# refresh-bio/colord

Measured on AMD Instinct MI355X. Metric: input Gbases/s + archive size vs ref, ONT 50 Gb at 1/2/4/8 MI355X, higher is better.
Workload: dtype u64

## Files before the change

### colord_amd/csrc/common.hpp

```cpp
#pragma once
#ifdef CL_HOST_DEBUG
#define CL_DEV __host__ __device__
#else
#define CL_DEV __device__
#endif
#include <hip/hip_runtime.h>
#include <cstdint>
#include <cstdio>
#include <cstring>
#include <string>
#include <vector>
#include <algorithm>
#include <map>
#include <deque>
#include <mutex>
#include <atomic>
#include <condition_variable>
#include <thread>
#include <chrono>
#include "../../include/colord_hip.h"

#define CL_WAVE 64

struct KernelTime { double ms = 0; uint32_t launches = 0; double bytes = 0, cells = 0; };
// ... 364 lines not shown
	}
	~KernelTimer()
	{
		if (cl_sync_debug())
		{
			fprintf(stderr, "[sync] > %s\n", name);
			const hipError_t e = hipStreamSynchronize(cl_launch_stream(c));
			fprintf(stderr, "[sync] < %s%s%s\n", name, e == hipSuccess ? "" : ": ", e == hipSuccess ? "" : hipGetErrorString(e));
		}
		if (!c->timing) return;
		(void)hipEventRecord(b, cl_launch_stream(c));
		c->pending.push_back({ name, { a, b } });
		c->pending_bytes.push_back(c->next_bytes); c->next_bytes = 0;
		c->pending_cells.push_back(c->next_cells); c->next_cells = 0;
	}
};
#define LAUNCH(ctx, kernel, grid, block, ...) do { KernelTimer _kt((ctx), #kernel); \
	hipLaunchKernelGGL(kernel, dim3(grid), dim3(block), 0, cl_launch_stream(ctx), __VA_ARGS__); } while (0)
#define LAUNCHB_NAMED(ctx, name, bytes, kernel, grid, block, ...) do { (ctx)->next_bytes = (double)(bytes); KernelTimer _kt((ctx), (name)); \
	hipLaunchKernelGGL(kernel, dim3(grid), dim3(block), 0, cl_launch_stream(ctx), __VA_ARGS__); } while (0)
#define LAUNCH_NAMED(ctx, name, kernel, grid, block, ...) LAUNCHB_NAMED(ctx, name, 0.0, kernel, grid, block, __VA_ARGS__)
#define LAUNCHB(ctx, bytes, kernel, grid, block, ...) do { (ctx)->next_bytes = (double)(bytes); LAUNCH(ctx, kernel, grid, block, __VA_ARGS__); } while (0)
#define LAUNCHB_SHM(ctx, bytes, kernel, grid, block, shm, ...) do { (ctx)->next_bytes = (double)(bytes); KernelTimer _kt((ctx), #kernel); \
	hipLaunchKernelGGL(kernel, dim3(grid), dim3(block), (shm), cl_launch_stream(ctx), __VA_ARGS__); } while (0)
enum { CL_ROLE_MAIN = 0, CL_ROLE_QUAL = 1, CL_ROLE_LANE = 2, CL_ROLE_PREP = 3, CL_ROLE_CODER = 4, CL_N_ROLES = 5 };
struct CuMaskCfg { bool any = false; bool on[CL_N_ROLES] = { false, false, false, false, false }; uint32_t lo[CL_N_ROLES] = { 0, 0, 0, 0, 0 }, hi[CL_N_ROLES] = { 0, 0, 0, 0, 0 }; };
inline const CuMaskCfg& cl_cu_mask_cfg()
{
	static const CuMaskCfg cfg = []() {
		CuMaskCfg c;
		const char* e = getenv("COLORD_HIP_CU_MASK");
		if (!e) return c;
		static const char* names[CL_N_ROLES] = { "main", "qual", "lane", "prep", "coder" };
		std::string s(e); size_t p = 0;
		while (p < s.size())
		{
			size_t q = s.find(',', p); if (q == std::string::npos) q = s.size();
			const std::string item = s.substr(p, q - p); p = q + 1;
			const size_t colon = item.find(':'), dash = item.find('-');
			if (colon == std::string::npos || dash == std::string::npos || dash < colon) continue;
			for (int r = 0; r < CL_N_ROLES; ++r) if (item.substr(0, colon) == names[r])
			{
				c.lo[r] = (uint32_t)atoi(item.substr(colon + 1, dash - colon - 1).c_str()); c.hi[r] = (uint32_t)atoi(item.substr(dash + 1).c_str());
				if (c.hi[r] >= c.lo[r] && c.hi[r] < 1024) { c.on[r] = true; c.any = true; }
			}
		}
		return c;
	}();
	return cfg;
}
static inline int cl_role_level(int role, int dflt)
{
	static const struct Cfg { bool on[CL_N_ROLES] = {}; int level[CL_N_ROLES] = {}; Cfg() {
		const char* e = getenv("COLORD_HIP_ROLE_PRIO"); if (!e) return;
		static const char* names[CL_N_ROLES] = { "main", "qual", "lane", "prep", "coder" };
		std::string t(e); size_t p = 0;
		while (p < t.size()) { size_t q = t.find(',', p); if (q == std::string::npos) q = t.size(); const std::string item = t.substr(p, q - p); const size_t c = item.find(':');
			if (c != std::string::npos) for (int r = 0; r < CL_N_ROLES; ++r) if (item.substr(0, c) == names[r]) { on[r] = true; level[r] = atoi(item.c_str() + c + 1); }
			p = q + 1; }
	} } cfg;
	return role >= 0 && role < CL_N_ROLES && cfg.on[role] ? cfg.level[role] : dflt;
}
static inline int cl_level_to_prio(int level)
{
	int least = 0, greatest = 0;
	if (hipDeviceGetStreamPriorityRange(&least, &greatest) != hipSuccess) { (void)hipGetLastError(); return 0; }
	return level > 0 ? greatest : level < 0 ? least : 0;
}
static inline hipError_t cl_stream_create_role(int role, int prio, hipStream_t* s)
{
	const CuMaskCfg& m = cl_cu_mask_cfg();
	if (role >= 0 && role < CL_N_ROLES && m.on[role])
	{
		uint32_t bits[32] = { 0 };
		for (uint32_t b = m.lo[role]; b <= m.hi[role]; ++b) bits[b >> 5] |= 1u << (b & 31);
		return hipExtStreamCreateWithCUMask(s, (m.hi[role] >> 5) + 1, bits);
	}
	return prio ? hipStreamCreateWithPriority(s, hipStreamNonBlocking, prio) : hipStreamCreateWithFlags(s, hipStreamNonBlocking);
}
static inline hipError_t cl_stream_create(cl_ctx* c, hipStream_t* s) { return cl_stream_create_role(c->role, c->prio, s); }
static inline hipError_t cl_side_stream(cl_ctx* c, std::atomic<hipStream_t>& slot)
{
	if (slot.load(std::memory_order_acquire)) return hipSuccess;
	hipStream_t s = nullptr;
	const hipError_t e = cl_stream_create(c, &s);
	if (e == hipSuccess) slot.store(s, std::memory_order_release);
	return e;
}
static inline void cl_timing_begin(cl_ctx*) {}
static inline void cl_timing_collect(cl_ctx* c, bool wait = false)
{
	if (!c->timing) return;
	size_t keep = 0;
	for (size_t i = 0; i < c->pending.size(); ++i)
	{
		auto& p = c->pending[i];
		bool done = true;
		if (wait) (void)hipEventSynchronize(p.second.second);
		else if (hipEventQuery(p.second.second) != hipSuccess) { (void)hipGetLastError(); done = false; }
		if (!done)
		{
			if (keep != i) { c->pending[keep] = std::move(p); c->pending_bytes[keep] = c->pending_bytes[i]; c->pending_cells[keep] = c->pending_cells[i]; }
			++keep;
			continue;
		}
		float ms = 0; (void)hipEventElapsedTime(&ms, p.second.first, p.second.second);
		std::string nm = p.first;
		if (!nm.empty() && nm.front() == '(' && nm.back() == ')') nm = nm.substr(1, nm.size() - 2);
		auto& t = c->times[nm]; t.ms += ms; t.launches += 1; t.bytes += c->pending_bytes[i]; t.cells += c->pending_cells[i];
		c->ev_pool.push_back(p.second.first); c->ev_pool.push_back(p.second.second);
	}
	c->pending.resize(keep); c->pending_bytes.resize(keep); c->pending_cells.resize(keep);
}

__host__ __device__ static inline uint64_t hash_mm(uint64_t x)
{
	x ^= x >> 33; x *= 0xff51afd7ed558ccdULL;
	x ^= x >> 33; x *= 0xc4ceb9fe1a85ec53ULL;
	x ^= x >> 33;
	return x;
}

struct ModTest { uint64_t low_mask, dinv, lim; uint32_t s; };
static inline ModTest make_modtest(uint32_t f)
{
	ModTest m; uint32_t s = 0; uint64_t d = f;
	while ((d & 1) == 0) { d >>= 1; ++s; }
	uint64_t inv = d;
	for (int i = 0; i < 6; ++i) inv *= 2 - d * inv;
	m.s = s; m.low_mask = (s ? ((1ULL << s) - 1) : 0); m.dinv = inv; m.lim = ~0ULL / d;
	return m;
}
__device__ static inline bool mod_is_zero(uint64_t h, const ModTest& m)
{
	return ((h & m.low_mask) == 0) && (((h >> m.s) * m.dinv) <= m.lim);
}

__device__ static inline uint32_t lane_id() { return threadIdx.x & 63; }
__device__ static inline uint64_t lanemask_lt() { return (1ULL << lane_id()) - 1; }

__device__ static inline uint32_t wave_incl_scan(uint32_t v)
{
#pragma unroll
	for (int d = 1; d < 64; d <<= 1) { uint32_t t = __shfl_up(v, d, 64); if ((int)lane_id() >= d) v += t; }
	return v;
}
__device__ static inline uint32_t wave_sum(uint32_t v)
{
#pragma unroll
	for (int d = 32; d > 0; d >>= 1) v += __shfl_xor(v, d, 64);
	return v;
}

__device__ static inline uint32_t block_excl_scan_256(uint32_t v, uint32_t* sh, uint32_t* total)
{
	uint32_t incl = wave_incl_scan(v);
	uint32_t w = threadIdx.x >> 6;
	__syncthreads();
	if (lane_id() == 63) sh[w] = incl;
	__syncthreads();
	uint32_t base = 0, tot = 0;
#pragma unroll
	for (uint32_t i = 0; i < 4; ++i) { uint32_t s = sh[i]; if (i < w) base += s; tot += s; }
	*total = tot;
	return base + incl - v;
}

cl_status dev_exclusive_scan_u32(cl_ctx* ctx, uint32_t* d_data, uint64_t n, uint64_t* h_total);
cl_status dev_exclusive_scan_u64(cl_ctx* ctx, const uint32_t* d_in, uint64_t* d_out, uint64_t n, uint64_t* h_total);
cl_status dev_run_starts_u32(cl_ctx* ctx, const uint32_t* d_keys, uint64_t n, uint32_t shift, uint32_t* d_seg, uint64_t seg_cap, uint64_t* h_n_runs);
cl_status dev_run_starts_u64(cl_ctx* ctx, const uint64_t* d_keys, uint64_t n, uint32_t shift, uint32_t* d_seg, uint64_t seg_cap, uint64_t* h_n_runs);
cl_status dev_sort_pairs(cl_ctx* ctx, uint64_t* d_keys, uint32_t* d_vals, uint64_t n, uint32_t begin_bit, uint32_t end_bit);
cl_status dev_sort_pairs_swap(cl_ctx* ctx, DevBuf<uint64_t>& keys, DevBuf<uint32_t>& vals, uint64_t n, uint32_t begin_bit, uint32_t end_bit);
cl_status dev_sort_keys32_pairs(cl_ctx* ctx, uint32_t* d_keys, uint32_t* d_vals, uint64_t n, uint32_t begin_bit, uint32_t end_bit);
cl_status dev_sort_keys32_pairs_swap(cl_ctx* ctx, DevBuf<uint32_t>& keys, DevBuf<uint32_t>& vals, uint64_t n, uint32_t begin_bit, uint32_t end_bit);

static inline uint32_t grid_for(uint64_t n, uint32_t per_block) { return (uint32_t)((n + per_block - 1) / per_block); }
```

### colord_amd/csrc/dna.hip

```cpp
#include "common.hpp"
#include <functional>
#include "objects.hpp"
#include "rc_dev.hpp"
#include <algorithm>
#include <deque>
#include <thread>
#include <chrono>

namespace {
enum { T_INS = 0, T_DEL, T_MATCH, T_SUBST, T_ANCHOR, T_SKIP, T_ALT_ID, T_MAIN_REF, T_PLAIN, T_START_PLAIN, T_START_ES, T_START_PLAIN_N, T_NONE };
enum { F_READ_TYPE = 0, F_REV_COMP, F_SEEN, F_LEN_BITS, F_LEN_DATA, F_SYMBOLS, F_SYMBOLS_N, F_READ_ID, F_READ_ID_SHORT,
       F_ANCHOR_LEN, F_SKIP_LOCAL, F_SKIP_DISTANT, F_TUPLE_TYPE, N_FAM };
constexpr uint32_t MAX_ALT = 64;

struct FamTab {
	uint32_t n_sym[N_FAM], max_total[N_FAM], adder[N_FAM];
	uint32_t ctx_base[N_FAM + 1];
	uint64_t state_base[N_FAM + 1];
	uint32_t n_ctx[N_FAM];
	int32_t level, T, S;
	uint32_t sym_B;
	uint32_t max_alt;
	uint32_t long_run;
	uint32_t walk_chunk, walk_warm;
};

struct RefStore { const uint64_t* packed; const uint64_t* word_off; const uint32_t* lens; uint32_t n; };
__device__ inline uint32_t ref_at(const RefStore& R, uint32_t id, bool rev, int64_t pos)
{
	if (id >= R.n) return 255;
	const uint32_t len = R.lens[id];
	if (pos < 0 || pos >= (int64_t)len) return 255;
	const uint32_t p = rev ? (len - 1 - (uint32_t)pos) : (uint32_t)pos;
	const uint32_t b = (uint32_t)(R.packed[R.word_off[id] + (p >> 5)] >> (62 - 2 * (p & 31))) & 3u;
	return rev ? 3u - b : b;
}
struct RefCur {
	uint32_t id = 0xffffffffu, len = 0, widx = 0xffffffffu; bool rev = false, ok = false; uint64_t wo = 0, word = 0;
	__device__ inline void set(const RefStore& R, uint32_t nid, bool nrev)
	{
		rev = nrev;
		if (nid == id) return;
		id = nid; widx = 0xffffffffu; ok = nid < R.n;
		if (ok) { len = R.lens[nid]; wo = R.word_off[nid]; }
	}
	__device__ inline uint32_t at(const RefStore& R, int64_t pos)
	{
		if (!ok || pos < 0 || pos >= (int64_t)len) return 255;
		const uint32_t p = rev ? (len - 1 - (uint32_t)pos) : (uint32_t)pos;
		if ((p >> 5) != widx) { widx = p >> 5; word = R.packed[wo + widx]; }
		const uint32_t b = (uint32_t)(word >> (62 - 2 * (p & 31))) & 3u;
		return rev ? 3u - b : b;
	}
};
__device__ inline uint32_t ilog2_(uint64_t x) { return x ? 64u - (uint32_t)__clzll((long long)x) : 0u; }
__device__ inline uint32_t no_bytes_(uint64_t x) { uint32_t r = 1; x >>= 8; for (; x; ++r) x >>= 8; return r; }

template<typename K> struct KeyFmt {
	static __host__ __device__ inline K make(uint32_t gctx, uint32_t payload) { return ((K)gctx << 8) | (K)payload; }
	static __host__ __device__ inline uint32_t ctx(K k) { return (uint32_t)(k >> 8); }
	static __host__ __device__ inline uint32_t payload(K k) { return (uint32_t)k & 0xffu; }
};
__device__ inline uint32_t key_payload(int fam, uint32_t sym, int e1, int e2)
{
	if (fam == F_TUPLE_TYPE)
	{
		const uint32_t x = e1 == 15 ? 0u : e2 == 15 ? (e1 == T_ANCHOR ? 1u : 2u) : e1 == T_ANCHOR ? 3u : e1 == T_DEL ? 4u : 5u;
		return (x << 3) | sym;
	}
	if (fam == F_SYMBOLS) return ((e1 == 15 ? 0u : (uint32_t)e1 + 1u) << 2) | sym;
	return sym;
}
__device__ inline void key_decode(uint32_t fam, uint32_t p, uint32_t& sym, uint32_t& e1, uint32_t& e2)
{
	if (fam == F_TUPLE_TYPE)
	{
		const uint32_t x = p >> 3; sym = p & 7u;
		e1 = x == 0 ? 15u : (x == 1 || x == 3) ? (uint32_t)T_ANCHOR : x == 2 ? (uint32_t)T_SKIP : x == 4 ? (uint32_t)T_DEL : (uint32_t)T_ALT_ID;
		e2 = x == 3 ? (uint32_t)T_MATCH : x == 4 ? (uint32_t)T_SKIP : x == 5 ? (uint32_t)T_MAIN_REF : 15u;
	}
	else if (fam == F_SYMBOLS) { const uint32_t x = p >> 2; sym = p & 3u; e1 = x ? x - 1u : 15u; e2 = 15u; }
	else { sym = p; e1 = e2 = 15u; }
}
__device__ inline uint32_t key_sym_mask(uint32_t fam) { return fam == F_TUPLE_TYPE ? 7u : fam == F_SYMBOLS ? 3u : 0xffu; }

template<typename K>
struct Emitter {
	static constexpr uint32_t SLOTS = 64 / sizeof(K);
	bool write; K* key; uint64_t off; uint32_t count; const FamTab* ft;
	K* stage = nullptr; uint64_t first = 0; bool any = false;
	__device__ inline void put(K k)
	{
		const uint64_t g = off + count;
		if (!stage) { key[g] = k; return; }
		if (!any) { first = g; any = true; }
		stage[g & (SLOTS - 1)] = k;
		if ((g & (SLOTS - 1)) != SLOTS - 1) return;
		const uint64_t base = g & ~(uint64_t)(SLOTS - 1);
		if (first <= base)
		{
			uint4* dst = (uint4*)(key + base); const uint32_t* sw = (const uint32_t*)stage;
#pragma unroll
			for (int q = 0; q < 4; ++q) dst[q] = make_uint4(sw[4 * q], sw[4 * q + 1], sw[4 * q + 2], sw[4 * q + 3]);
		}
		else for (uint64_t x = first; x <= g; ++x) key[x] = stage[x & (SLOTS - 1)];
	}
	__device__ inline void finish()
	{
		if (!stage || !any) return;
		const uint64_t g = off + count, base = g & ~(uint64_t)(SLOTS - 1);
		for (uint64_t x = first > base ? first : base; x < g; ++x) key[x] = stage[x & (SLOTS - 1)];
	}
	__device__ inline void operator()(int fam, uint32_t ctx, uint32_t sym, int e1 = 15, int e2 = 15)
	{
		if (write)
		{
			put(KeyFmt<K>::make(ft->ctx_base[fam] + ctx, key_payload(fam, sym, e1, e2)));
		}
		++count;
	}
};

struct EsReader {
	const uint8_t* p; const uint8_t* e;
	uint64_t w0 = 0, w1 = 0; uint32_t have = 0;
	__device__ inline void refill()
	{
		const uint64_t a = (uint64_t)(size_t)p; const uint32_t sh = (uint32_t)(a & 7);
		const uint64_t* q = (const uint64_t*)(a & ~7ull);
		const uint64_t* lim = (const uint64_t*)(((uint64_t)(size_t)e + 7) & ~7ull);
		const uint64_t x0 = q[0], x1 = q + 1 < lim ? q[1] : 0ull, x2 = q + 2 < lim ? q[2] : 0ull;
		w0 = sh ? (x0 >> (8 * sh)) | (x1 << (64 - 8 * sh)) : x0;
		w1 = sh ? (x1 >> (8 * sh)) | (x2 << (64 - 8 * sh)) : x1;
		have = 16;
	}
	__device__ inline void drop(uint32_t n) { p += n; have -= n; w0 = (w0 >> (8 * n)) | (w1 << (64 - 8 * n)); w1 >>= 8 * n; }
	__device__ inline bool next(uint32_t& type, uint32_t& v1, uint32_t& v2)
	{
		if (p >= e) return false;
		if (have < 5) refill();
		const uint32_t b0 = (uint32_t)(w0 & 0xff), t = b0 >> 4; type = t;
		switch (t)
		{
		case T_INS: case T_SUBST: case T_PLAIN: v1 = b0 & 0xf; drop(1); break;
		case T_ANCHOR: case T_SKIP: v2 = ((b0 & 0xf) << 24) | ((uint32_t)((w0 >> 8) & 0xff) << 16) | ((uint32_t)((w0 >> 16) & 0xff) << 8) | (uint32_t)((w0 >> 24) & 0xff); drop(4); break;
		case T_ALT_ID: case T_START_ES: v2 = b0 & 0xf; v1 = ((uint32_t)((w0 >> 8) & 0xff) << 24) | ((uint32_t)((w0 >> 16) & 0xff) << 16) | ((uint32_t)((w0 >> 24) & 0xff) << 8) | (uint32_t)((w0 >> 32) & 0xff); drop(5); break;
		default: drop(1);
		}
		return true;
	}
};

template<typename K> __device__ inline void emit_read_len(Emitter<K>& em, uint32_t len)
{
	int nb = (int)ilog2_(len);
	em(F_LEN_BITS, 0, (uint32_t)nb);
// ... 190 lines not shown
					rd.p += 8; rd.have -= 8; rd.w0 = rd.w1; rd.w1 = 0;
					t_idx += 8;
					continue;
				}
			}
		}
		if (!rd.next(type, v1, v2)) break;
		++t_idx;
		const uint32_t ref_symbol = !track ? 0u : is_main ? mainc.at(R, ref_pos) : altc.at(R, alt_pos);
		{
			uint32_t cls = delta < -10 ? 1u : delta < -1 ? 2u : delta > 10 ? 3u : delta > 1 ? 4u : 0u;
			uint32_t c = (uint32_t)ctx_tuple | ((uint32_t)(ctx_symbol & 0xf) << s3);
			if (ref_symbol <= 3) c |= (ref_symbol << (s3 + 4)) | (cls << (s3 + 6));
			else c = (1u << (s3 + 9)) + (c | (cls << (s3 + 4)));
			int e1 = 15, e2 = 15;
			if (!first)
				switch (last_flag)
				{
				case T_MATCH: e1 = T_ANCHOR; break;
				case T_DEL: e1 = T_SKIP; break;
				case T_ANCHOR: e1 = T_ANCHOR; e2 = T_MATCH; break;
				case T_SKIP: e1 = T_DEL; e2 = T_SKIP; break;
				case T_MAIN_REF: case T_ALT_ID: e1 = T_ALT_ID; e2 = T_MAIN_REF; break;
				default: break;
				}
			em(F_TUPLE_TYPE, c, type, e1, e2);
			ctx_tuple = ((ctx_tuple << 3) + type) & mask_tuple;
		}
		first = false; last_flag = type;
		switch (type)
		{
		case T_ALT_ID:
		{
			if (!is_main && alt_slot >= 0) alt_pos_of[alt_slot] = (int32_t)alt_pos;
			bool is_new = false; int32_t slot = -1;
			if (n_alt == 0) { emit_read_id(em, v1, cur_read_id); alt_ids[0] = (int32_t)v1; alt_pos_of[0] = 0; n_alt = 1; slot = 0; is_new = true; }
			else
			{
				const uint32_t seen = n_alt;
				for (uint32_t i = 0; i < n_alt; ++i) if (alt_ids[i] == (int32_t)v1) slot = (int32_t)i;
				const int32_t short_id = slot;
				if (slot < 0)
				{
					if (n_alt >= MAX_ALT) { if (err) atomicOr(err, 1u); em.finish(); return; }
					slot = (int32_t)n_alt; alt_ids[n_alt] = (int32_t)v1; alt_pos_of[n_alt] = 0; ++n_alt; is_new = true;
				}
				em(F_SEEN, seen, short_id >= 0 ? 1u : 0u);
				if (short_id < 0) emit_read_id(em, v1, cur_read_id);
				else em(F_READ_ID_SHORT, seen, (uint32_t)short_id);
			}
			if (is_new) alt_rev_of[slot] = (uint8_t)v2;
			rev_comp_flag(v1, v2 != 0);
			alt_id = v1; alt_slot = slot; alt_rev = alt_rev_of[slot] != 0;
			altc.set(R, alt_id, alt_rev);
			alt_pos = 0; is_main = false; delta = 0;
			break;
		}
		case T_ANCHOR:
			emit_anchor_len(em, v2);
			if (is_main) ref_pos += v2; else alt_pos += v2;
			if (track)
			{
				for (int i = ft.S; i > 0; --i)
					ctx_symbol = (ctx_symbol << 2) + (is_main ? mainc.at(R, ref_pos - i) : altc.at(R, alt_pos - i));
				ctx_symbol &= mask_symbol;
				known = (uint32_t)ft.S;
			}
			delta = 0;
			break;
		case T_MATCH:
			ctx_symbol = ((ctx_symbol << 2) + ref_symbol) & mask_symbol; ++known;
			if (is_main) ++ref_pos; else ++alt_pos;
			break;
		case T_INS:
		{
			uint32_t shift = 2, c = 2;
			if (ft.level == 1) { c += (uint32_t)(ctx_symbol & 0xff) << shift; shift += 8; }
			else if (ft.level == 2) { c += (uint32_t)(ctx_symbol & 0x3ff) << shift; shift += 10; }
			else { c += (uint32_t)(ctx_symbol & 0x3ff) << shift; shift += 10; c += (uint32_t)(((ctx_symbol >> 10) & 3) == ((ctx_symbol >> 8) & 3)) << shift; ++shift; }
			const bool guard = ref_symbol > 3;
			c += (guard ? 0u : ref_symbol) << shift; shift += 2;
			c += (uint32_t)(ctx_tuple & 0777) << shift;
			if (guard) c += 1u << ft.sym_B;
			em(F_SYMBOLS, c, v1);
			ctx_symbol = ((ctx_symbol << 2) + v1) & mask_symbol; ++known;
			++delta;
			break;
		}
		case T_DEL:
			if (is_main) ++ref_pos; else ++alt_pos;
			--delta;
			break;
		case T_SUBST:
		{
			const uint32_t rs = ref_symbol & 3;
			const uint32_t sym = (rs == 0) ? (v1 == 0 ? 1u : v1 == 1 ? 2u : 3u) : (rs == 1) ? (v1 == 0 ? 0u : v1 == 1 ? 2u : 3u)
			                   : (rs == 2) ? (v1 == 0 ? 0u : v1 == 1 ? 1u : 3u) : (v1 == 0 ? 0u : v1 == 1 ? 1u : 2u);
			uint32_t shift = 2, c = 1;
			c += (uint32_t)(ctx_symbol & 0x3f) << shift; shift += 6;
			if (ft.level == 3) { c += (uint32_t)(((ctx_symbol >> 6) & 3) == ((ctx_symbol >> 4) & 3)) << shift; ++shift; }
			c += rs << shift; shift += 2;
			c += (uint32_t)(ctx_tuple & 07777) << shift;
			em(F_SYMBOLS, c, sym, (int)rs);
			ctx_symbol = ((ctx_symbol << 2) + sym) & mask_symbol; ++known;
			if (is_main) ++ref_pos; else ++alt_pos;
			break;
		}
		case T_SKIP:
		{
			const int32_t skip_len = (int32_t)v2;
			delta -= skip_len;
			if (!is_main && last_type == T_ALT_ID)
			{
				const int32_t mod = skip_len - (alt_slot >= 0 ? alt_pos_of[alt_slot] : 0);
				if (mod > 0) emit_skip_len(em, (uint32_t)mod, false);
				else { emit_skip_len(em, 0, false); emit_skip_len(em, (uint32_t)(-mod), false); }
			}
			else emit_skip_len(em, (uint32_t)skip_len, last_type != T_ALT_ID && last_type != T_NONE);
			if (is_main) ref_pos += v2; else alt_pos += v2;
			break;
		}
		case T_MAIN_REF:
			is_main = true;
			if (alt_slot >= 0) alt_pos_of[alt_slot] = (int32_t)alt_pos;
			delta = 0;
			break;
		default: break;
		}
		last_type = type;
	}
	em.finish();
	if (!WRITE)
	{
		hdr_counts[r] = em.count; counts[r] = em.count;
		if (t_idx != ntup - 1 && err) atomicOr(err, 2u);
	}
}

__global__ void k_read_flags(const uint8_t* __restrict__ es, const uint64_t* __restrict__ es_off, uint32_t r0, uint32_t r1, uint8_t* __restrict__ flag)
{
	uint32_t r = r0 + blockIdx.x * blockDim.x + threadIdx.x;
	if (r >= r1) return;
	uint32_t t = es[es_off[r]] >> 4;
	flag[r - r0] = t == T_START_PLAIN ? 0 : t == T_START_PLAIN_N ? 1 : 2;
}

__global__ __launch_bounds__(256) void k_fill_sidx(const uint64_t* __restrict__ sym_off, uint64_t s0, uint32_t r0, uint32_t r1, TripLayoutDev lay, uint32_t* __restrict__ sidx)
{
	const uint32_t r = r0 + blockIdx.x * 4 + (threadIdx.x >> 6);
	if (r >= r1) return;
	const uint32_t lane = threadIdx.x & 63;
	const uint64_t a = sym_off[r] - s0, b = sym_off[r + 1] - s0;
	if (a == b) return;
	const uint32_t part = part_of_read(lay, r), pl = lay.rank ? lay.rank[part] : part;
	const uint64_t gb = lay.group_base[pl >> 6], p0 = lay.part_sym_start[part];
	for (uint64_t i = a + lane; i < b; i += 64) sidx[i] = (uint32_t)trip_slot(gb, pl & 63, i - p0);
}
template<typename K>
__global__ __launch_bounds__(256) void k_dna_plain(const FamTab* __restrict__ ftp, const uint8_t* __restrict__ es, const uint64_t* __restrict__ es_off,
                                                  const uint32_t* __restrict__ es_ntup, const uint8_t* __restrict__ read_flag, const uint32_t* __restrict__ hdr_counts,
                                                  const uint64_t* __restrict__ sym_off, uint32_t r0, uint32_t r1, K* __restrict__ key)
{
	const uint32_t r = r0 + blockIdx.x * 4 + (threadIdx.x >> 6);
	if (r >= r1) return;
	const uint32_t fl = read_flag[r - r0];
	if (fl == 2) return;
	const FamTab& ft = *ftp;
	const uint32_t lane = threadIdx.x & 63;
	const uint8_t* b = es + es_off[r] + 1;
	const uint32_t len = es_ntup[r] - 1;
	const uint64_t off = sym_off[r - r0] + hdr_counts[r - r0];
	const uint32_t S2 = 2 * ft.S; const uint32_t mask = (1u << S2) - 1;
	const uint32_t fam = fl == 0 ? F_SYMBOLS : F_SYMBOLS_N;
	const uint32_t cbase = ft.ctx_base[fam];
	for (uint32_t i = lane; i < len; i += 64)
	{
		uint32_t ctx = mask;
		if (fl == 0)
		{
			const uint32_t n = i < (uint32_t)ft.S ? i : (uint32_t)ft.S;
			for (uint32_t t = n; t >= 1; --t) ctx = ((ctx << 2) + (b[i - t] & 3u)) & mask;
			ctx <<= 2;
		}
		else
		{
			const uint32_t n = i < 4 ? i : 4;
			for (uint32_t t = n; t >= 1; --t) ctx = ((ctx << 4) + (b[i - t] & 0xfu)) & mask;
		}
		key[off + i] = KeyFmt<K>::make(cbase + ctx, b[i] & 0xfu);
	}
}


constexpr uint32_t LONG_RUN = 1u << 19;
struct LongRun { uint32_t s, e, fam, gctx; uint64_t step0, group0, epoch0; uint32_t epoch_cap, pad; };
template<int NS> struct EpochRec { uint32_t start, tot; uint32_t st[NS]; uint32_t cnt0[NS]; };
__device__ inline uint32_t find_run(const LongRun* runs, uint32_t n_runs, uint64_t step)
{
	uint32_t lo = 0, hi = n_runs;
	while (hi - lo > 1) { const uint32_t mid = (lo + hi) >> 1; if (runs[mid].step0 <= step) lo = mid; else hi = mid; }
	return lo;
}
template<typename K>
__global__ void k_long_find(const uint32_t* __restrict__ seg_start, uint32_t n_seg, const K* __restrict__ skey, const FamTab* __restrict__ ftp, LongRun* __restrict__ runs , uint32_t cap, uint32_t* __restrict__ n_runs )
{
	const uint32_t sg = blockIdx.x * blockDim.x + threadIdx.x;
	if (sg >= n_seg) return;
	const uint32_t s = seg_start[sg], e = seg_start[sg + 1];
	const FamTab& ft = *ftp;
	if (e - s < ft.long_run) return;
	const uint32_t gctx = KeyFmt<K>::ctx(skey[s]);
	uint32_t fam = 0;
	for (uint32_t f = 1; f < N_FAM; ++f) if (gctx >= ft.ctx_base[f]) fam = f;
	if (ft.n_sym[fam] > 32) return;
	const uint32_t which = ft.n_sym[fam] > 8 ? 1u : 0u;
	const uint32_t i = atomicAdd(n_runs + which, 1u);
	if (i < cap) { LongRun r; r.s = s; r.e = e; r.fam = fam; r.gctx = gctx; r.step0 = r.group0 = r.epoch0 = 0; r.epoch_cap = 0; r.pad = 0; runs[which * cap + i] = r; }
}
template<int NS, typename K>
__global__ __launch_bounds__(256) void k_long_hist(const LongRun* __restrict__ runs, uint32_t n_runs, uint64_t n_groups, const K* __restrict__ skey,
                                                  uint32_t* __restrict__ step_pfx, uint32_t* __restrict__ group_tot)
{
	const uint64_t g = ((uint64_t)blockIdx.x * blockDim.x + threadIdx.x) >> 6; const uint32_t lane = threadIdx.x & 63;
	if (g >= n_groups) return;
	uint32_t lo = 0, hi = n_runs;
	while (hi - lo > 1) { const uint32_t mid = (lo + hi) >> 1; if (runs[mid].group0 <= g) lo = mid; else hi = mid; }
	const LongRun R = runs[lo];
	const uint64_t gl = g - R.group0;
	const uint32_t smask = key_sym_mask(R.fam);
	uint32_t c[NS];
#pragma unroll
	for (int a = 0; a < NS; ++a) c[a] = 0;
	for (uint32_t k = 0; k < 64; ++k)
	{
		const uint64_t j = (uint64_t)R.s + (gl * 64 + k) * 64 + lane;
		const bool valid = j < R.e;
		const uint32_t sym = valid ? (uint32_t)skey[j] & smask : 0xffu;
#pragma unroll
		for (uint32_t a = 0; a < NS; ++a) { const uint32_t n = (uint32_t)__popcll(__ballot(sym == a)); if (lane == k) c[a] = n; }
	}
	const uint64_t n_steps = ((uint64_t)(R.e - R.s) + 63) / 64;
	const uint64_t step = R.step0 + gl * 64 + lane;
#pragma unroll
	for (uint32_t a = 0; a < NS; ++a)
	{
		const uint32_t incl = wave_incl_scan(c[a]);
		if (gl * 64 + lane < n_steps) step_pfx[step * NS + a] = incl - c[a];
		if (lane == 63) group_tot[g * NS + a] = incl;
	}
}
template<int NS>
__global__ __launch_bounds__(64) void k_long_groups(const LongRun* __restrict__ runs, uint32_t n_runs, uint32_t* __restrict__ group_tot )
{
	const uint32_t r = blockIdx.x, lane = threadIdx.x;
	if (r >= n_runs) return;
	const LongRun R = runs[r];
	const uint64_t n_steps = ((uint64_t)(R.e - R.s) + 63) / 64, n_groups = (n_steps + 63) / 64;
	uint32_t carry[NS];
#pragma unroll
	for (int a = 0; a < NS; ++a) carry[a] = 0;
	for (uint64_t g0 = 0; g0 < n_groups; g0 += 64)
	{
		const uint64_t g = g0 + lane; const bool valid = g < n_groups;
#pragma unroll
		for (uint32_t a = 0; a < NS; ++a)
		{
			const uint32_t v = valid ? group_tot[(R.group0 + g) * NS + a] : 0u;
			const uint32_t incl = wave_incl_scan(v);
			if (valid) group_tot[(R.group0 + g) * NS + a] = carry[a] + incl - v;
			carry[a] += __shfl(incl, 63);
		}
	}
}
template<int NS, typename K>
__device__ inline uint32_t long_prefix(const LongRun& R, const K* skey, const uint32_t* step_pfx, const uint32_t* group_pfx, uint32_t x, uint32_t lane)
{
	const uint32_t smask = key_sym_mask(R.fam);
	const uint64_t step = x >> 6; const uint32_t off = x & 63;
	const uint32_t a = lane & (NS - 1);
	uint32_t v = group_pfx[(R.group0 + (step >> 6)) * NS + a] + (step * 64 < (uint64_t)(R.e - R.s) || off ? step_pfx[(R.step0 + step) * NS + a] : 0u);
	if (x == R.e - R.s && off == 0)
	{
		const uint64_t last = step - 1;
		const uint64_t j = (uint64_t)R.s + last * 64 + lane; const uint32_t sym = j < R.e ? (uint32_t)skey[j] & smask : 0xffu;
		uint32_t mine = 0;
#pragma unroll
		for (uint32_t b = 0; b < NS; ++b) { const uint32_t n = (uint32_t)__popcll(__ballot(sym == b)); if (a == b) mine = n; }
		return group_pfx[(R.group0 + (last >> 6)) * NS + a] + step_pfx[(R.step0 + last) * NS + a] + mine;
	}
	if (off)
	{
		const uint64_t j = (uint64_t)R.s + step * 64 + lane; const uint32_t sym = j < R.e ? (uint32_t)skey[j] & smask : 0xffu;
		const uint64_t below = (1ULL << off) - 1;
		uint32_t mine = 0;
#pragma unroll
		for (uint32_t b = 0; b < NS; ++b) { const uint32_t n = (uint32_t)__popcll(__ballot(sym == b) & below); if (a == b) mine = n; }
		v += mine;
	}
	return v;
}
template<int NS, typename K>
__global__ __launch_bounds__(64) void k_long_epochs(const FamTab* __restrict__ ftp, const LongRun* __restrict__ runs, uint32_t n_runs, const K* __restrict__ skey,
                                                   const uint32_t* __restrict__ step_pfx, const uint32_t* __restrict__ group_pfx, uint32_t* __restrict__ state,
                                                   EpochRec<NS>* __restrict__ epochs, uint32_t* __restrict__ n_epochs, uint32_t* __restrict__ group_epoch, uint32_t* __restrict__ err)
{
	const uint32_t r = blockIdx.x, lane = threadIdx.x;
	if (r >= n_runs) return;
	const LongRun R = runs[r];
	const FamTab& ft = *ftp;
	const uint32_t n_sym = ft.n_sym[R.fam], max_total = ft.max_total[R.fam], adder = ft.adder[R.fam];
// ... 101 lines not shown
	{
		if (e - s >= ft.long_run) return;
		uint32_t st[8]; uint32_t tot = sp[n_sym];
#pragma unroll
		for (uint32_t a = 0; a < 8; ++a) st[a] = a < n_sym ? sp[a] : 0u;
		for (uint32_t j0 = s; j0 < e; j0 += 64)
		{
			const uint32_t j = j0 + lane; const bool valid = j < e;
			uint32_t sym = 0xffu, e1 = 15u, e2 = 15u;
			if (valid) key_decode(fam, KeyFmt<K>::payload(skey[j]), sym, e1, e2);
			const uint32_t dst = valid ? sval[j] : 0u;
			uint64_t m[8];
#pragma unroll
			for (uint32_t a = 0; a < 8; ++a) m[a] = __ballot(valid && sym == a);
			const uint32_t cnt = (e - j0) < 64 ? (e - j0) : 64;
			uint32_t start = 0;
			while (start < cnt)
			{
				const uint32_t r = (max_total - tot + adder - 1) / adder;
				const uint32_t now = (cnt - start) < r ? (cnt - start) : r;
				const uint64_t win = (now == 64 ? ~0ULL : ((1ULL << now) - 1)) << start;
				if (lane >= start && lane < start + now)
				{
					const uint64_t before = lt & win;
					uint32_t cum = 0, freq = 0, excl = 0;
#pragma unroll
					for (uint32_t a = 0; a < 8; ++a)
					{
						const uint32_t v = st[a] + adder * (uint32_t)__popcll(m[a] & before);
						const bool ex = a == e1 || a == e2;
						if (ex) excl += v;
						if (a < sym && !ex) cum += v;
						if (a == sym) freq = v;
					}
					trip[dst] = pack_triple(cum, freq, tot + adder * (lane - start) - excl);
				}
#pragma unroll
				for (uint32_t a = 0; a < 8; ++a) st[a] += adder * (uint32_t)__popcll(m[a] & win);
				tot += adder * now;
				while (tot >= max_total)
				{
					tot = 0;
#pragma unroll
					for (uint32_t a = 0; a < 8; ++a) { st[a] = (st[a] + 1) / 2; tot += st[a]; }
				}
				start += now;
			}
		}
		if (lane == 0)
		{
			for (uint32_t a = 0; a < n_sym; ++a) sp[a] = st[a];
			sp[n_sym] = tot;
		}
		return;
	}
	if (n_sym <= 32 && e - s >= ft.long_run) return;
	uint32_t* cnt = s_cnt[w]; uint32_t* pre = s_pre[w];
#pragma unroll
	for (uint32_t t = 0; t < 4; ++t) { uint32_t a = lane * 4 + t; cnt[a] = a < n_sym ? sp[a] : 0u; }
	uint32_t tot = sp[n_sym];
	auto rebuild_prefix = [&]() {
		uint32_t v0 = cnt[lane * 4], v1 = cnt[lane * 4 + 1], v2 = cnt[lane * 4 + 2], v3 = cnt[lane * 4 + 3];
		uint32_t sum = v0 + v1 + v2 + v3;
		uint32_t ex = wave_incl_scan(sum) - sum;
		pre[lane * 4] = ex; pre[lane * 4 + 1] = ex + v0; pre[lane * 4 + 2] = ex + v0 + v1; pre[lane * 4 + 3] = ex + v0 + v1 + v2;
		__builtin_amdgcn_wave_barrier();
	};
	__builtin_amdgcn_wave_barrier();
	rebuild_prefix();
	for (uint32_t j0 = s; j0 < e; j0 += 64)
	{
		const uint32_t j = j0 + lane; const bool valid = j < e;
		const uint32_t sym = valid ? KeyFmt<K>::payload(skey[j]) : 0u;
		const uint32_t dst = valid ? sval[j] : 0u;
		const uint32_t n_here = (e - j0) < 64 ? (e - j0) : 64;
		uint32_t start = 0;
		while (start < n_here)
		{
			const uint32_t r = (max_total - tot + adder - 1) / adder;
			const uint32_t now = (n_here - start) < r ? (n_here - start) : r;
			uint32_t less = 0, eq = 0;
			for (uint32_t l = start; l < start + now; ++l)
			{
				const uint32_t o = __builtin_amdgcn_readlane(sym, l);
				if (l < lane) { less += (o < sym) ? 1u : 0u; eq += (o == sym) ? 1u : 0u; }
			}
			const bool mine = lane >= start && lane < start + now;
			if (mine) trip[dst] = pack_triple(pre[sym] + adder * less, cnt[sym] + adder * eq, tot + adder * (lane - start));
			__builtin_amdgcn_wave_barrier();
			if (mine) atomicAdd(&cnt[sym], adder);
			__builtin_amdgcn_wave_barrier();
			tot += adder * now;
			while (tot >= max_total)
			{
				uint32_t sum = 0;
#pragma unroll
				for (uint32_t t = 0; t < 4; ++t) { uint32_t a = lane * 4 + t; if (a < n_sym) { uint32_t v = (cnt[a] + 1) / 2; cnt[a] = v; sum += v; } }
				tot = wave_sum(sum);
			}
			__builtin_amdgcn_wave_barrier();
			rebuild_prefix();
			start += now;
		}
	}
#pragma unroll
	for (uint32_t t = 0; t < 4; ++t) { uint32_t a = lane * 4 + t; if (a < n_sym) sp[a] = cnt[a]; }
	if (lane == 0) sp[n_sym] = tot;
}

__global__ void k_init_fam_state(const FamTab* __restrict__ ftp, uint32_t fam, uint32_t* __restrict__ state)
{
	const FamTab& ft = *ftp;
	const uint32_t ns = ft.n_sym[fam];
	const uint64_t n = (uint64_t)ft.n_ctx[fam] * (ns + 1);
	for (uint64_t i = (uint64_t)blockIdx.x * blockDim.x + threadIdx.x; i < n; i += (uint64_t)gridDim.x * blockDim.x)
		state[ft.state_base[fam] + i] = (i % (ns + 1)) == ns ? ns : 1u;
}
__global__ void k_gather_bytes2(const uint8_t* __restrict__ src, const uint64_t* __restrict__ src_off, const uint64_t* __restrict__ dst_off,
                                const uint64_t* __restrict__ size, uint8_t* __restrict__ dst)
{
	const uint32_t p = blockIdx.x;
	const uint64_t n = size[p]; const uint8_t* s = src + src_off[p]; uint8_t* d = dst + dst_off[p];
	for (uint64_t i = threadIdx.x; i < n; i += blockDim.x) d[i] = s[i];
}
__global__ void k_last_types(const uint8_t* __restrict__ flag, uint32_t n, uint32_t prev, uint32_t* __restrict__ out)
{
	uint32_t v = prev;
	uint32_t start = n > 4 ? n - 4 : 0;
	for (uint32_t i = start; i < n; ++i) v = ((v << 2) + flag[i]) & 0xff;
	*out = v;
}
}

struct DnaGroupPrep {
	uint32_t p0 = 0, p1 = 0, r0 = 0, r1 = 0; uint64_t s0 = 0, n_syms = 0, n_seg = 0, trip_words = 0;
	std::vector<uint32_t> rank, plen_r;
	DevBuf<uint64_t> d_gbase; DevBuf<uint32_t> d_plen;
	DevBuf<uint32_t> sidx, seg;
	struct LongPrep { uint32_t n_runs = 0; uint64_t steps = 0, groups = 0, eps = 0; DevBuf<LongRun> runs; DevBuf<uint32_t> step_pfx, group_pfx; } lp[2];
	bool long_ready = false;
};
struct DnaWalked {
	const uint8_t* d_es = nullptr; uint32_t n_reads = 0;
	uint32_t prev_types_in = 0, cur_read_id_in = 0, prev_types_out = 0;
	DevBuf<uint8_t> rflag; DevBuf<uint32_t> hdr; DevBuf<uint64_t> sym_off, key; DevBuf<uint32_t> key32; bool narrow = false;
	std::vector<uint64_t> h_sym_off;
	bool presorted = false; std::vector<uint32_t> part_bounds; std::vector<std::unique_ptr<DnaGroupPrep>> groups;
};
struct cl_dna_coder {
	cl_ctx* ctx = nullptr;
	FamTab ft;
	DevBuf<FamTab> d_ft;
	DevBuf<uint32_t> state;
	uint32_t ctx_bits = 0; bool narrow = false;
	uint32_t cur_read_id = 0;
	uint32_t prev_types = 0;
	uint32_t next_read_id = 0, next_prev_types = 0; bool next_valid = false;
	std::unique_ptr<DnaWalked> ahead;
	std::function<cl_status()> before_tail;
	std::deque<std::unique_ptr<struct DnaEvolved>> evolved;
	uint32_t ahead_prev_types = 0, ahead_read_id = 0;
	std::vector<hipStream_t> cstreams; uint32_t next_cstream = 0;
	~cl_dna_coder();
};

extern "C" cl_status cl_dna_coder_create(cl_ctx* ctx, uint32_t max_alt_refs, int32_t level, uint32_t start_read_id, cl_dna_coder** out)
{
	if (!ctx || !out) return cl_fail(ctx, CL_E_INVALID, "cl_dna_coder_create: null argument");
	if (level < 1 || level > 3 || max_alt_refs < 1 || max_alt_refs > MAX_ALT) return cl_fail(ctx, CL_E_INVALID, "cl_dna_coder_create: level 1..3, 1 <= max_alt_refs <= 64");
	HIP_TRY(ctx, hipSetDevice(ctx->device));
	cl_dna_coder* D = new cl_dna_coder(); D->ctx = ctx; D->cur_read_id = start_read_id;
	std::unique_ptr<cl_dna_coder> guard(D);
	FamTab& f = D->ft; memset(&f, 0, sizeof(f));
	f.level = level; f.max_alt = max_alt_refs;
	f.T = level == 3 ? 4 : level == 2 ? 3 : 2;
	f.S = level == 3 ? 8 : level == 2 ? 7 : 5;
	f.sym_B = level == 3 ? 24 : level == 2 ? 23 : 22;
	f.long_run = LONG_RUN;
	if (const char* lr = getenv("COLORD_HIP_LONG_RUN")) f.long_run = (uint32_t)std::max(64, atoi(lr));
	f.walk_chunk = WALK_CHUNK; f.walk_warm = WALK_WARM;
	if (const char* v = getenv("COLORD_HIP_WALK_CHUNK")) f.walk_chunk = (uint32_t)std::min(1 << 20, std::max(32, atoi(v)));
	if (const char* v = getenv("COLORD_HIP_WALK_WARM")) f.walk_warm = (uint32_t)std::max(0, atoi(v));
	f.walk_warm = std::min(f.walk_warm, f.walk_chunk / 2);
	auto set = [&](int i, uint32_t ns, uint32_t mt, uint32_t ad, uint32_t nc) { f.n_sym[i] = ns; f.max_total[i] = mt; f.adder[i] = ad; f.n_ctx[i] = nc; };
	set(F_READ_TYPE, 3, 1u << 15, 1, 256);
	set(F_REV_COMP, 2, 1u << 15, 1, 16);
	set(F_SEEN, 2, 1u << 15, 1, MAX_ALT + 1);
	set(F_LEN_BITS, 32, 1u << 18, 8, 1);
	set(F_LEN_DATA, 256, 1u << 18, 8, 512);
	set(F_SYMBOLS, 4, 1u << 10, 1, 1u << (f.sym_B + 1));
	set(F_SYMBOLS_N, 5, 1u << 10, 1, 1u << 16);
	set(F_READ_ID, 256, 1u << 13, 1, 2048);
	set(F_READ_ID_SHORT, max_alt_refs, 1u << 13, 1, MAX_ALT + 1);
	set(F_ANCHOR_LEN, 24, 1u << 15, 1, 1u << 17);
	set(F_SKIP_LOCAL, 256, 1u << 15, 1, 1u << 14);
	set(F_SKIP_DISTANT, 256, 1u << 15, 1, 256);
	set(F_TUPLE_TYPE, 8, 1u << 15, 1, 1u << (3 * f.T + 10));
	uint64_t cb = 0, sb = 0;
	for (int i = 0; i < N_FAM; ++i) { f.ctx_base[i] = (uint32_t)cb; f.state_base[i] = sb; cb += f.n_ctx[i]; sb += (uint64_t)f.n_ctx[i] * (f.n_sym[i] + 1); }
	f.ctx_base[N_FAM] = (uint32_t)cb; f.state_base[N_FAM] = sb;
	if (cb >= (1ull << 32)) return cl_fail(ctx, CL_E_UNSUPPORTED, "cl_dna_coder_create: context space too large");
	D->ctx_bits = 1; while ((1ull << D->ctx_bits) < cb) ++D->ctx_bits;
	D->narrow = D->ctx_bits + 8 <= 32 && !getenv("COLORD_HIP_DNA_WIDE_KEYS");
	DEV_ALLOC(ctx, D->d_ft, 1);
	HIP_TRY(ctx, hipMemcpyAsync(D->d_ft.p, &f, sizeof(f), hipMemcpyHostToDevice, ctx->stream));
	DEV_ALLOC(ctx, D->state, sb);
	for (uint32_t i = 0; i < N_FAM; ++i) LAUNCH(ctx, k_init_fam_state, 2048, 256, (const FamTab*)D->d_ft.p, i, D->state.p);
	HIP_TRY(ctx, hipGetLastError());
	HIP_TRY(ctx, hipStreamSynchronize(ctx->stream));
	*out = guard.release();
	return CL_OK;
}
extern "C" void cl_dna_coder_free(cl_dna_coder* d) { delete d; }

namespace {
struct SideSync { hipStream_t s = nullptr; ~SideSync() { if (s) (void)hipStreamSynchronize(s); } };
struct PendingGroup {
	DevBuf<triple_t> trip; DevBuf<uint64_t> d_gbase, d_out_off, d_size, d_dst_off; DevBuf<uint32_t> d_plen; DevBuf<uint8_t> tmp;
	std::vector<uint64_t> out_off; std::vector<uint32_t> rank; uint32_t p0 = 0, np = 0;
	hipStream_t stream = nullptr;
	SideSync sync;
};
}
struct DnaEvolved {
	const uint8_t* d_es = nullptr; uint32_t n_reads = 0, prev_types_in = 0, read_id_in = 0, prev_types_out = 0;
	std::vector<uint32_t> part_bounds;
	std::vector<std::unique_ptr<PendingGroup>> groups;
};
cl_dna_coder::~cl_dna_coder() { evolved.clear(); for (hipStream_t s : cstreams) (void)hipStreamDestroy(s); }

namespace {
cl_status dna_walk(cl_ctx* ctx, cl_dna_coder* D, const cl_reads* refs, const uint8_t* d_es, const uint64_t* d_es_off, const uint32_t* d_es_ntuples, uint32_t n_reads,
                   uint32_t prev_types, uint32_t cur_read_id, DnaWalked& W)
{
	const FamTab& f = D->ft;
	RefStore R{ refs->packed.p, refs->word_off.p, refs->lens.p, refs->n_reads };
	W.d_es = d_es; W.n_reads = n_reads; W.prev_types_in = prev_types; W.cur_read_id_in = cur_read_id;
	DevBuf<uint8_t>& rflag = W.rflag; DevBuf<uint32_t>& hdr = W.hdr; DevBuf<uint64_t>& sym_off = W.sym_off; std::vector<uint64_t>& h_sym_off = W.h_sym_off;
	W.narrow = D->narrow;
	DEV_ALLOC(ctx, rflag, (uint64_t)n_reads + 1); DEV_ALLOC(ctx, hdr, (uint64_t)n_reads + 1); DEV_ALLOC(ctx, sym_off, (uint64_t)n_reads + 1);
	DevBuf<uint32_t> err; DEV_ALLOC(ctx, err, 1);
	HIP_TRY(ctx, hipMemsetAsync(err.p, 0, 4, ctx->stream));
	h_sym_off.assign((size_t)n_reads + 1, 0);
	if (n_reads)
	{
		uint64_t total_syms = 0, h_eb[2] = { 0, 0 };
		HIP_TRY(ctx, hipMemcpyAsync(&h_eb[0], d_es_off, 8, hipMemcpyDeviceToHost, ctx->stream));
		HIP_TRY(ctx, hipMemcpyAsync(&h_eb[1], d_es_off + n_reads, 8, hipMemcpyDeviceToHost, ctx->stream));
		HIP_TRY(ctx, hipStreamSynchronize(ctx->stream));
		DevBuf<uint64_t> chunk_off; DEV_ALLOC(ctx, chunk_off, (uint64_t)n_reads + 1);
		DevBuf<WalkCk> cks; uint64_t n_chunks = 0;
		{
			DevBuf<uint32_t> counts; DEV_ALLOC(ctx, counts, n_reads);
			LAUNCH(ctx, k_read_flags, grid_for(n_reads, 256), 256, d_es, d_es_off, 0u, n_reads, rflag.p);
			LAUNCH(ctx, k_walk_chunks, grid_for(n_reads, 256), 256, d_es_ntuples, (const uint8_t*)rflag.p, n_reads, f.walk_chunk, counts.p);
			CL_TRY(dev_exclusive_scan_u64(ctx, counts.p, chunk_off.p, n_reads, &n_chunks));
			if (n_chunks >= (1ull << 32)) return cl_fail(ctx, CL_E_UNSUPPORTED, "cl_dna_encode: too many tuples in one call");
			DEV_ALLOC(ctx, cks, n_chunks);
			LAUNCHB_NAMED(ctx, "k_dna_walk<false>", (double)(h_eb[1] - h_eb[0]) + 8.0 * n_reads + (double)n_chunks * sizeof(WalkCk), (k_dna_walk<false, uint32_t>), grid_for(n_reads, WALK_LPW), 64,
				(const FamTab*)D->d_ft.p, R, d_es, d_es_off, d_es_ntuples, (const uint8_t*)rflag.p, n_reads,
				prev_types, cur_read_id, (const uint64_t*)chunk_off.p, cks.p, (uint32_t)n_chunks, counts.p, hdr.p, (const uint64_t*)nullptr, (uint32_t*)nullptr, err.p, 0u);
			HIP_TRY(ctx, hipGetLastError());
			CL_TRY(dev_exclusive_scan_u64(ctx, counts.p, sym_off.p, n_reads, &total_syms));
		}
		HIP_TRY(ctx, hipMemcpy(h_sym_off.data(), sym_off.p, ((uint64_t)n_reads + 1) * 8, hipMemcpyDeviceToHost));
		uint32_t herr0 = 0;
		HIP_TRY(ctx, hipMemcpy(&herr0, err.p, 4, hipMemcpyDeviceToHost));
		if (herr0 & 2) return cl_fail(ctx, CL_E_INVALID, "cl_dna_encode: the tuple count of a read does not match its stream");
		if (herr0) return cl_fail(ctx, CL_E_UNSUPPORTED, "cl_dna_encode: a read uses more than 64 alternative references");
		if (W.narrow)
		{
			DEV_ALLOC(ctx, W.key32, total_syms);
			LAUNCHB_NAMED(ctx, "k_dna_walk<true>", total_syms * 5.0, (k_dna_walk<true, uint32_t>), grid_for(n_chunks, WALK_LPW), 64,
				(const FamTab*)D->d_ft.p, R, d_es, d_es_off, d_es_ntuples, (const uint8_t*)rflag.p, n_reads,
				prev_types, cur_read_id, (const uint64_t*)chunk_off.p, cks.p, (uint32_t)n_chunks, (uint32_t*)nullptr, (uint32_t*)nullptr, (const uint64_t*)sym_off.p, W.key32.p, err.p, 1u);
			LAUNCH_NAMED(ctx, "k_dna_plain", (k_dna_plain<uint32_t>), grid_for(n_reads, 4), 256, (const FamTab*)D->d_ft.p, d_es, d_es_off, d_es_ntuples, (const uint8_t*)rflag.p, (const uint32_t*)hdr.p,
				(const uint64_t*)sym_off.p, 0u, n_reads, W.key32.p);
		}
		else
		{
			DEV_ALLOC(ctx, W.key, total_syms);
			LAUNCHB_NAMED(ctx, "k_dna_walk<true>", total_syms * 9.0, (k_dna_walk<true, uint64_t>), grid_for(n_chunks, WALK_LPW), 64,
				(const FamTab*)D->d_ft.p, R, d_es, d_es_off, d_es_ntuples, (const uint8_t*)rflag.p, n_reads,
				prev_types, cur_read_id, (const uint64_t*)chunk_off.p, cks.p, (uint32_t)n_chunks, (uint32_t*)nullptr, (uint32_t*)nullptr, (const uint64_t*)sym_off.p, W.key.p, err.p, 1u);
			LAUNCH_NAMED(ctx, "k_dna_plain", (k_dna_plain<uint64_t>), grid_for(n_reads, 4), 256, (const FamTab*)D->d_ft.p, d_es, d_es_off, d_es_ntuples, (const uint8_t*)rflag.p, (const uint32_t*)hdr.p,
				(const uint64_t*)sym_off.p, 0u, n_reads, W.key.p);
		}
		HIP_TRY(ctx, hipGetLastError());
	}
	{
		DevBuf<uint32_t> lt; DEV_ALLOC(ctx, lt, 1);
		LAUNCH(ctx, k_last_types, 1, 1, (const uint8_t*)rflag.p, n_reads, prev_types, lt.p);
		HIP_TRY(ctx, hipGetLastError());
		HIP_TRY(ctx, hipMemcpyAsync(&W.prev_types_out, lt.p, 4, hipMemcpyDeviceToHost, ctx->stream));
		HIP_TRY(ctx, hipStreamSynchronize(ctx->stream));
	}
	return CL_OK;
}
}

namespace {
template<typename K>
cl_status dna_long_prepare(cl_ctx* ctx, cl_dna_coder* D, const K* gkey, uint64_t n_syms, DnaGroupPrep& G)
{
	const FamTab& f = D->ft;
	const uint32_t RUN_CAP = (uint32_t)std::max<uint64_t>(4096, n_syms / f.long_run + 2);
	DevBuf<LongRun> runs; DEV_ALLOC(ctx, runs, 2 * RUN_CAP);
	DevBuf<uint32_t> n_runs; DEV_ALLOC(ctx, n_runs, 2);
	HIP_TRY(ctx, hipMemsetAsync(n_runs.p, 0, 8, ctx->stream));
	LAUNCH_NAMED(ctx, "k_long_find", (k_long_find<K>), grid_for(G.n_seg, 256), 256, (const uint32_t*)G.seg.p, (uint32_t)G.n_seg, gkey, (const FamTab*)D->d_ft.p, runs.p, RUN_CAP, n_runs.p);
	uint32_t nlr2[2] = { 0, 0 };
	HIP_TRY(ctx, hipMemcpyAsync(nlr2, n_runs.p, 8, hipMemcpyDeviceToHost, ctx->stream));
	HIP_TRY(ctx, hipStreamSynchronize(ctx->stream));
	if (nlr2[0] > RUN_CAP || nlr2[1] > RUN_CAP) return cl_fail(ctx, CL_E_UNSUPPORTED, "cl_dna_encode: more than 4096 long context runs in one group");
	for (int which = 0; which < 2; ++which)
	{
		DnaGroupPrep::LongPrep& L = G.lp[which];
		const uint32_t nlr = nlr2[which], NS = which ? 32 : 8;
		L.n_runs = nlr; L.steps = L.groups = L.eps = 0;
		if (!nlr) continue;
		std::vector<LongRun> h(nlr);
		HIP_TRY(ctx, hipMemcpy(h.data(), runs.p + (uint64_t)which * RUN_CAP, nlr * sizeof(LongRun), hipMemcpyDeviceToHost));
		std::sort(h.begin(), h.end(), [](const LongRun& a, const LongRun& b) { return a.s < b.s; });
		for (auto& r : h)
		{
			const uint64_t Ln = r.e - r.s, ns = (Ln + 63) / 64, ngp = (ns + 63) / 64;
			const uint64_t half = f.max_total[r.fam] / 2 / f.adder[r.fam];
			r.step0 = L.steps; r.group0 = L.groups; r.epoch0 = L.eps; r.epoch_cap = (uint32_t)(Ln / (half > 80 ? half - 40 : 1) + 8);
			L.steps += ns; L.groups += ngp; L.eps += r.epoch_cap;
		}
		DEV_ALLOC(ctx, L.runs, nlr);
		HIP_TRY(ctx, hipMemcpyAsync(L.runs.p, h.data(), nlr * sizeof(LongRun), hipMemcpyHostToDevice, ctx->stream));
		DEV_ALLOC(ctx, L.step_pfx, (L.steps + 1) * NS); DEV_ALLOC(ctx, L.group_pfx, (L.groups + 1) * NS);
		const LongRun* cr = L.runs.p;
		if (which == 0)
		{
			LAUNCHB_NAMED(ctx, "k_long_hist<8>", L.steps * 64.0 * sizeof(K), (k_long_hist<8, K>), grid_for(L.groups * 64, 256), 256, cr, nlr, L.groups, gkey, L.step_pfx.p, L.group_pfx.p);
			LAUNCH(ctx, (k_long_groups<8>), nlr, 64, cr, nlr, L.group_pfx.p);
		}
		else
		{
			LAUNCHB_NAMED(ctx, "k_long_hist<32>", L.steps * 64.0 * sizeof(K), (k_long_hist<32, K>), grid_for(L.groups * 64, 256), 256, cr, nlr, L.groups, gkey, L.step_pfx.p, L.group_pfx.p);
			LAUNCH(ctx, (k_long_groups<32>), nlr, 64, cr, nlr, L.group_pfx.p);
		}
		HIP_TRY(ctx, hipGetLastError());
		HIP_TRY(ctx, hipStreamSynchronize(ctx->stream));
	}
	G.long_ready = true;
	return CL_OK;
}
}

namespace {
cl_status dna_group_prepare(cl_ctx* ctx, cl_dna_coder* D, DnaWalked& W, uint32_t p0, const uint32_t* h_part_bounds, uint32_t n_parts, DnaGroupPrep& G)
{
	const std::vector<uint64_t>& h_sym_off = W.h_sym_off;
	const uint64_t GROUP_SYMS = 5ull << 28;
	uint32_t p1 = p0; const uint32_t r0 = h_part_bounds[p0];
	while (p1 < n_parts)
	{
		const uint64_t pl = h_sym_off[h_part_bounds[p1 + 1]] - h_sym_off[h_part_bounds[p1]];
		if (pl >= (1ull << 31) - 64) return cl_fail(ctx, CL_E_UNSUPPORTED, "cl_dna_encode: one part has >= 2^31 symbols");
		if (p1 > p0 && h_sym_off[h_part_bounds[p1 + 1]] - h_sym_off[r0] >= GROUP_SYMS) break;
		++p1;
	}
	const uint32_t r1 = h_part_bounds[p1], nr = r1 - r0, np = p1 - p0, ng = (np + 63) / 64;
	const uint64_t s0 = h_sym_off[r0], n_syms = h_sym_off[r1] - s0;
	G.p0 = p0; G.p1 = p1; G.r0 = r0; G.r1 = r1; G.s0 = s0; G.n_syms = n_syms;
	std::vector<uint64_t> sym_start(np + 1);
	std::vector<uint32_t> plen(np), pfirst(np + 1);
	for (uint32_t p = 0; p <= np; ++p) { pfirst[p] = h_part_bounds[p0 + p]; sym_start[p] = h_sym_off[pfirst[p]] - s0; }
	for (uint32_t p = 0; p < np; ++p) plen[p] = (uint32_t)(sym_start[p + 1] - sym_start[p]);
	std::vector<uint32_t> order(np); std::vector<uint32_t>& rank = G.rank; std::vector<uint32_t>& plen_r = G.plen_r;
	rank.resize(np); plen_r.resize(np);
	for (uint32_t p = 0; p < np; ++p) order[p] = p;
	std::stable_sort(order.begin(), order.end(), [&](uint32_t a, uint32_t b) { return plen[a] > plen[b]; });
	for (uint32_t i = 0; i < np; ++i) { rank[order[i]] = i; plen_r[i] = plen[order[i]]; }
	std::vector<uint64_t> gbase(ng + 1, 0);
	for (uint32_t g = 0; g < ng; ++g) gbase[g + 1] = gbase[g] + trip_group_words(plen_r[g * 64]);
	if (gbase[ng] >= (1ull << 32)) return cl_fail(ctx, CL_E_UNSUPPORTED, "cl_dna_encode: group too large for 32-bit triple indices");
	G.trip_words = gbase[ng];
	DevBuf<uint64_t> d_sym_start; DevBuf<uint32_t> d_pfirst, d_rank;
	DEV_ALLOC(ctx, d_rank, np);
	HIP_TRY(ctx, hipMemcpyAsync(d_rank.p, rank.data(), np * 4, hipMemcpyHostToDevice, ctx->stream));
	DEV_ALLOC(ctx, d_sym_start, np + 1); DEV_ALLOC(ctx, G.d_gbase, ng + 1); DEV_ALLOC(ctx, G.d_plen, np); DEV_ALLOC(ctx, d_pfirst, np + 1);
	HIP_TRY(ctx, hipMemcpyAsync(d_sym_start.p, sym_start.data(), (np + 1) * 8, hipMemcpyHostToDevice, ctx->stream));
	HIP_TRY(ctx, hipMemcpyAsync(G.d_gbase.p, gbase.data(), (ng + 1) * 8, hipMemcpyHostToDevice, ctx->stream));
	HIP_TRY(ctx, hipMemcpyAsync(G.d_plen.p, plen_r.data(), np * 4, hipMemcpyHostToDevice, ctx->stream));
	HIP_TRY(ctx, hipMemcpyAsync(d_pfirst.p, pfirst.data(), (np + 1) * 4, hipMemcpyHostToDevice, ctx->stream));
	TripLayoutDev lay{ d_pfirst.p, d_sym_start.p, G.d_gbase.p, np, d_rank.p };
	if (n_syms)
	{
		DEV_ALLOC(ctx, G.sidx, n_syms);
		LAUNCHB(ctx, n_syms * 4.0, k_fill_sidx, grid_for(nr, 4), 256, (const uint64_t*)W.sym_off.p, s0, r0, r1, lay, G.sidx.p);
		HIP_TRY(ctx, hipGetLastError());
		const uint32_t cbits = D->ctx_bits;
		const uint64_t seg_cap = std::min<uint64_t>(n_syms, D->ft.ctx_base[N_FAM]) + 1;
		DEV_ALLOC(ctx, G.seg, seg_cap);
		if (W.narrow)
		{
			if (s0 == 0 && W.key32.n == n_syms) CL_TRY(dev_sort_keys32_pairs_swap(ctx, W.key32, G.sidx, n_syms, 8, 8 + cbits));
			else CL_TRY(dev_sort_keys32_pairs(ctx, W.key32.p + s0, G.sidx.p, n_syms, 8, 8 + cbits));
			CL_TRY(dev_run_starts_u32(ctx, W.key32.p + s0, n_syms, 8, G.seg.p, seg_cap, &G.n_seg));
			CL_TRY(dna_long_prepare<uint32_t>(ctx, D, W.key32.p + s0, n_syms, G));
		}
		else
		{
			if (s0 == 0 && W.key.n == n_syms) CL_TRY(dev_sort_pairs_swap(ctx, W.key, G.sidx, n_syms, 8, 8 + cbits));
			else CL_TRY(dev_sort_pairs(ctx, W.key.p + s0, G.sidx.p, n_syms, 8, 8 + cbits));
			CL_TRY(dev_run_starts_u64(ctx, W.key.p + s0, n_syms, 8, G.seg.p, seg_cap, &G.n_seg));
			CL_TRY(dna_long_prepare<uint64_t>(ctx, D, W.key.p + s0, n_syms, G));
		}
	}
	HIP_TRY(ctx, hipStreamSynchronize(ctx->stream));
	return CL_OK;
}
}

cl_status cl_dna_prepare_batch(cl_ctx* ctx, cl_dna_coder* D, const cl_reads* refs, const uint8_t* d_es, const uint64_t* d_es_off, const uint32_t* d_es_ntuples, uint32_t n_reads,
                               uint32_t prev_types, uint32_t read_id, const uint32_t* h_part_bounds, uint32_t n_parts, DnaWalked** out, uint32_t* prev_types_out)
{
	if (!ctx || !D || !refs || !d_es || !d_es_off || !d_es_ntuples || !n_reads || !out) return CL_E_INVALID;
	HIP_TRY(ctx, hipSetDevice(ctx->device));
	auto W = std::make_unique<DnaWalked>();
	CL_TRY(dna_walk(ctx, D, refs, d_es, d_es_off, d_es_ntuples, n_reads, prev_types, read_id, *W));
	if (h_part_bounds && n_parts && h_part_bounds[0] == 0 && h_part_bounds[n_parts] == n_reads)
	{
		W->part_bounds.assign(h_part_bounds, h_part_bounds + n_parts + 1);
		for (uint32_t p0 = 0; p0 < n_parts; )
		{
			auto G = std::make_unique<DnaGroupPrep>();
			CL_TRY(dna_group_prepare(ctx, D, *W, p0, h_part_bounds, n_parts, *G));
			p0 = G->p1;
			W->groups.push_back(std::move(G));
		}
		W->presorted = true;
	}
	if (prev_types_out) *prev_types_out = W->prev_types_out;
	*out = W.release();
	return CL_OK;
}
namespace {
__global__ void k_batch_types(const uint8_t* __restrict__ es, const uint64_t* __restrict__ es_off, uint32_t n_reads, uint64_t es_bytes, uint32_t prev, unsigned long long* __restrict__ out)
{
	uint32_t v = prev; bool ok = true;
	const uint32_t start = n_reads > 4 ? n_reads - 4 : 0;
	for (uint32_t r = start; r < n_reads; ++r)
	{
		const uint64_t a = es_off[r], b = es_off[r + 1];
		if (a >= b || b > es_bytes) { ok = false; break; }
		const uint32_t t = es[a] >> 4;
		v = ((v << 2) + (t == T_START_PLAIN ? 0u : t == T_START_PLAIN_N ? 1u : 2u)) & 0xff;
	}
	*out = ok ? (unsigned long long)v : ~0ull;
}
}
cl_status cl_dna_batch_types(cl_ctx* ctx, const uint8_t* d_es, const uint64_t* d_es_off, uint32_t n_reads, uint64_t es_bytes, uint32_t prev_types, uint32_t* out)
{
	if (!ctx || !d_es || !d_es_off || !out) return CL_E_INVALID;
	HIP_TRY(ctx, hipSetDevice(ctx->device));
	uint64_t* hs = nullptr; uint64_t* ds = nullptr;
	HIP_TRY(ctx, cl_slot(ctx, 1, &hs, &ds));
	LAUNCH(ctx, k_batch_types, 1, 1, d_es, d_es_off, n_reads, es_bytes, prev_types, (unsigned long long*)ds);
	HIP_TRY(ctx, hipGetLastError());
	HIP_TRY(ctx, hipStreamSynchronize(ctx->stream));
	const uint64_t v = *(volatile uint64_t*)hs;
	if (v == ~0ull) return cl_fail(ctx, CL_E_INVALID, "cl_dna_batch_types: a tuple stream offset of the last reads lies outside the stream");
	*out = (uint32_t)v;
	return CL_OK;
}
void cl_dna_walked_free(DnaWalked* W) { delete W; }
void cl_dna_set_ahead(cl_dna_coder* D, DnaWalked* W) { if (D) D->ahead.reset(W); else delete W; }
void cl_dna_coder_state(const cl_dna_coder* D, uint32_t* prev_types, uint32_t* read_id) { if (prev_types) *prev_types = D->prev_types; if (read_id) *read_id = D->cur_read_id; }

cl_status cl_dna_walk_ahead(cl_ctx* ctx, cl_dna_coder* D, const cl_reads* refs, const uint8_t* d_es, const uint64_t* d_es_off, const uint32_t* d_es_ntuples, uint32_t n_reads)
{
	if (!ctx || !D || !refs || !d_es || !d_es_off || !d_es_ntuples || !n_reads) return CL_E_INVALID;
	if (!D->next_valid) return cl_fail(ctx, CL_E_INVALID, "cl_dna_walk_ahead: only while a batch is being coded");
	auto W = std::make_unique<DnaWalked>();
	CL_TRY(dna_walk(ctx, D, refs, d_es, d_es_off, d_es_ntuples, n_reads, D->next_prev_types, D->next_read_id, *W));
	D->ahead = std::move(W);
	return CL_OK;
}
void cl_dna_set_before_tail(cl_dna_coder* D, std::function<cl_status()> fn) { if (D) D->before_tail = std::move(fn); }

namespace {
cl_status dna_evolve_batch(cl_ctx* ctx, cl_dna_coder* D, const cl_reads* refs, const uint8_t* d_es, const uint64_t* d_es_off, const uint32_t* d_es_ntuples, uint32_t n_reads,
                           const uint32_t* h_part_bounds, uint32_t n_parts, std::unique_ptr<DnaWalked> Wp, uint32_t prev_types, uint32_t read_id, DnaEvolved& E)
{
	const uint64_t* inv_tab = nullptr;
	CL_TRY(cl_inv_table(ctx, &inv_tab));
	if (Wp && Wp->presorted && (Wp->part_bounds.size() != (size_t)n_parts + 1 || memcmp(Wp->part_bounds.data(), h_part_bounds, ((size_t)n_parts + 1) * 4) != 0)) Wp.reset();
	if (!Wp) { Wp = std::make_unique<DnaWalked>(); CL_TRY(dna_walk(ctx, D, refs, d_es, d_es_off, d_es_ntuples, n_reads, prev_types, read_id, *Wp)); }
	DnaWalked& W = *Wp;
	DevBuf<uint32_t> err; DEV_ALLOC(ctx, err, 1);
	HIP_TRY(ctx, hipMemsetAsync(err.p, 0, 4, ctx->stream));
	E.d_es = d_es; E.n_reads = n_reads; E.prev_types_in = prev_types; E.read_id_in = read_id; E.prev_types_out = W.prev_types_out;
	E.part_bounds.assign(h_part_bounds, h_part_bounds + n_parts + 1);
	uint32_t p0 = 0; size_t gi = 0;
	while (p0 < n_parts)
	{
		std::unique_ptr<DnaGroupPrep> GP;
		if (W.presorted) { if (gi >= W.groups.size() || !W.groups[gi] || W.groups[gi]->p0 != p0) return cl_fail(ctx, CL_E_INVALID, "cl_dna_encode: prepared groups do not match"); GP = std::move(W.groups[gi++]); }
		else { GP = std::make_unique<DnaGroupPrep>(); CL_TRY(dna_group_prepare(ctx, D, W, p0, h_part_bounds, n_parts, *GP)); }
		const uint32_t p1 = GP->p1, np = p1 - p0, ng = (np + 63) / 64;
		const uint64_t s0 = GP->s0, n_syms = GP->n_syms;
		const std::vector<uint32_t>& rank = GP->rank; const std::vector<uint32_t>& plen_r = GP->plen_r;
		auto G = std::make_unique<PendingGroup>(); G->p0 = p0; G->np = np; G->rank = rank;
		G->d_gbase = std::move(GP->d_gbase); G->d_plen = std::move(GP->d_plen);
		DevBuf<uint64_t>& d_gbase = G->d_gbase; DevBuf<uint32_t>& d_plen = G->d_plen; DevBuf<triple_t>& trip = G->trip;
		DEV_ALLOC(ctx, trip, GP->trip_words);
		if (n_syms)
		{
			DevBuf<uint32_t>& sidx = GP->sidx; DevBuf<uint32_t>& seg = GP->seg; const uint64_t n_seg = GP->n_seg;
			auto models = [&](auto* gkey) -> cl_status {
				typedef std::remove_cv_t<std::remove_pointer_t<decltype(gkey)>> K;
				LAUNCHB_NAMED(ctx, "k_dna_evolve", n_syms * (12.0 + sizeof(K)), (k_dna_evolve<K>), grid_for(n_seg, 4), 256, (const FamTab*)D->d_ft.p, (const K*)gkey, (const uint32_t*)sidx.p, (const uint32_t*)seg.p,
					(uint32_t)n_seg, D->state.p, trip.p);
				HIP_TRY(ctx, hipGetLastError());
				for (int which = 0; which < 2; ++which)
				{
					DnaGroupPrep::LongPrep& L = GP->lp[which];
					const uint32_t nlr = L.n_runs, NS = which ? 32 : 8;
					if (!nlr) continue;
					DevBuf<uint32_t> d_ne, group_epoch, epochs;
					DEV_ALLOC(ctx, d_ne, nlr); DEV_ALLOC(ctx, group_epoch, L.groups + 1); DEV_ALLOC(ctx, epochs, (L.eps + 1) * (2 + 2 * NS));
					const LongRun* cr = L.runs.p; const uint64_t steps = L.steps;
					if (which == 0)
					{
						LAUNCH_NAMED(ctx, "k_long_epochs<8>", (k_long_epochs<8, K>), nlr, 64, (const FamTab*)D->d_ft.p, cr, nlr, (const K*)gkey, (const uint32_t*)L.step_pfx.p, (const uint32_t*)L.group_pfx.p,
							D->state.p, (EpochRec<8>*)epochs.p, d_ne.p, group_epoch.p, err.p);
						LAUNCHB_NAMED(ctx, "k_long_apply<8>", steps * 64 * (12.0 + sizeof(K)), (k_long_apply<8, K>), grid_for(steps * 64, 256), 256, cr, nlr, steps, (const K*)gkey, (const uint32_t*)sidx.p,
							(const uint32_t*)L.step_pfx.p, (const uint32_t*)L.group_pfx.p, (const EpochRec<8>*)epochs.p, (const uint32_t*)d_ne.p, (const uint32_t*)group_epoch.p, (const FamTab*)D->d_ft.p, trip.p);
					}
					else
					{
						LAUNCH_NAMED(ctx, "k_long_epochs<32>", (k_long_epochs<32, K>), nlr, 64, (const FamTab*)D->d_ft.p, cr, nlr, (const K*)gkey, (const uint32_t*)L.step_pfx.p, (const uint32_t*)L.group_pfx.p,
							D->state.p, (EpochRec<32>*)epochs.p, d_ne.p, group_epoch.p, err.p);
						LAUNCHB_NAMED(ctx, "k_long_apply<32>", steps * 64 * (12.0 + sizeof(K)), (k_long_apply<32, K>), grid_for(steps * 64, 256), 256, cr, nlr, steps, (const K*)gkey, (const uint32_t*)sidx.p,
							(const uint32_t*)L.step_pfx.p, (const uint32_t*)L.group_pfx.p, (const EpochRec<32>*)epochs.p, (const uint32_t*)d_ne.p, (const uint32_t*)group_epoch.p, (const FamTab*)D->d_ft.p, trip.p);
					}
					HIP_TRY(ctx, hipGetLastError());
					HIP_TRY(ctx, hipStreamSynchronize(ctx->stream));
				}
				return CL_OK;
			};
			if (W.narrow) CL_TRY(models((const uint32_t*)(W.key32.p + s0))); else CL_TRY(models((const uint64_t*)(W.key.p + s0)));
			HIP_TRY(ctx, hipStreamSynchronize(ctx->stream));
		}
		uint32_t herr = 0;
		HIP_TRY(ctx, hipMemcpy(&herr, err.p, 4, hipMemcpyDeviceToHost));
		if (herr & 8) return cl_fail(ctx, CL_E_UNSUPPORTED, "cl_dna_encode: epoch table of a long context run too small");
		if (herr) return cl_fail(ctx, CL_E_UNSUPPORTED, "cl_dna_encode: a read uses more than 64 alternative references");
		if (D->cstreams.size() < 4) { hipStream_t ns = nullptr; HIP_TRY(ctx, cl_stream_create_role(CL_ROLE_CODER, cl_level_to_prio(cl_role_level(CL_ROLE_CODER, 0)), &ns)); D->cstreams.push_back(ns); }
		G->stream = D->cstreams[D->next_cstream++ % D->cstreams.size()];
		G->out_off.resize(np + 1);
		G->out_off[0] = 0;
		for (uint32_t p = 0; p < np; ++p) { uint64_t sy = plen_r[p]; G->out_off[p + 1] = G->out_off[p] + ((sy * 18 + 7) / 8 + sy / 16 + 64 + 7) / 8 * 8; }
		DEV_ALLOC(ctx, G->tmp, G->out_off[np]);
		DEV_ALLOC(ctx, G->d_out_off, np + 1); DEV_ALLOC(ctx, G->d_size, np); DEV_ALLOC(ctx, G->d_dst_off, np);
		HIP_TRY(ctx, hipStreamSynchronize(ctx->stream));
// ... 98 lines not shown
```

### colord_amd/csrc/qual.hip

```cpp
#include "common.hpp"
#include <functional>
#include <deque>
#include <thread>
#include <chrono>
#include "objects.hpp"
#include "rc_dev.hpp"
#include <algorithm>

namespace {

enum { QM_ORIGINAL = 0, QM_QUINARY_AVG, QM_QUAD_AVG, QM_BINARY_AVG, QM_QUINARY_THR, QM_QUAD_THR, QM_BINARY_THR, QM_AVERAGE, QM_NONE };

struct QualCfg {
	int32_t mode, level;
	uint32_t bits_per_sym, n_ctx_sym, ctx_bits;
	uint32_t base_bits;
	uint32_t n_sym, sym_bits;
	uint32_t n_bins, navg;
	uint32_t max_total, adder;
	uint32_t n_ctx;
	uint32_t is_avg, is_thr;
	uint32_t hist_radix, n_hist;
	uint32_t dense_bits;
	uint8_t map_fwd[96], quant[96];
};

__host__ __device__ inline uint32_t qual_hist_radix(const QualCfg& c) { return c.mode == QM_ORIGINAL ? 1u << c.bits_per_sym : c.n_sym + 1; }
__host__ __device__ inline uint32_t qual_hist_add(uint32_t hist, uint32_t place, uint32_t field) { return hist + place * field; }
__host__ __device__ inline uint32_t qual_ctx_id(const QualCfg& c, uint32_t hist, uint32_t bctx, uint32_t fl)
{
	return hist + c.n_hist * (bctx | (fl << c.base_bits));
}

}

struct QualGroupPrep {
	uint32_t p0 = 0, p1 = 0, np = 0, ng = 0; uint64_t n_base = 0, n_syms = 0, n_byte = 0, trip_words = 0;
	std::vector<uint32_t> rank, plen_r;
	DevBuf<uint64_t> d_gbase; DevBuf<uint32_t> d_plen;
	DevBuf<uint32_t> key, sidx, bkey, bsidx, bss, bse;
};
struct QualPrepared {
	const cl_reads* R = nullptr; const uint8_t* d_quals = nullptr; std::vector<uint32_t> part_bounds;
	std::vector<std::unique_ptr<QualGroupPrep>> groups;
};
struct cl_qual_coder {
	cl_ctx* ctx = nullptr;
	QualCfg cfg;
	DevBuf<QualCfg> d_cfg;
	DevBuf<uint32_t> state;
	DevBuf<uint32_t> bstate;
	uint64_t symbols_coded = 0;
	std::unique_ptr<QualPrepared> ahead;
	std::deque<std::unique_ptr<struct QualEvolved>> evolved;
	std::function<cl_status()> before_tail;
	std::vector<hipStream_t> cstreams; uint32_t next_cstream = 0;
	~cl_qual_coder();
};
struct QualPending {
	DevBuf<triple_t> trip; DevBuf<uint64_t> d_gbase, d_out_off, d_size, d_dst_off; DevBuf<uint32_t> d_plen; DevBuf<uint8_t> tmp;
	std::vector<uint32_t> rank; uint32_t p0 = 0, np = 0; uint64_t n_syms = 0;
	hipStream_t stream = nullptr;
	~QualPending() { if (stream) (void)hipStreamSynchronize(stream); }
};
struct QualEvolved {
	const cl_reads* R = nullptr; const uint8_t* d_quals = nullptr; std::vector<uint32_t> part_bounds;
	std::vector<std::unique_ptr<QualPending>> groups;
};
cl_qual_coder::~cl_qual_coder() { evolved.clear(); for (hipStream_t s : cstreams) (void)hipStreamDestroy(s); }

namespace {
constexpr uint32_t BYTE_CTX = 5 * 128 + 256;

__device__ inline uint32_t arena_base(const uint64_t* __restrict__ packed, uint64_t wb, uint32_t p)
{
	return (uint32_t)(packed[wb + (p >> 5)] >> (62 - 2 * (p & 31))) & 3u;
}

__global__ __launch_bounds__(256) void k_qual_symbols(const QualCfg* __restrict__ cfgp, const uint64_t* __restrict__ packed,
                                                     const uint64_t* __restrict__ word_off, const uint8_t* __restrict__ quals,
                                                     const uint64_t* __restrict__ qoff, const uint8_t* __restrict__ flags,
                                                     uint32_t r0, uint32_t r1, uint64_t q0, TripLayoutDev lay,
                                                     uint32_t* __restrict__ key, uint32_t* __restrict__ sidx_out,
                                                     uint32_t* __restrict__ bkey, uint32_t* __restrict__ bsidx, uint32_t* __restrict__ bad)
{
	__shared__ QualCfg cfg;
	for (uint32_t i = threadIdx.x; i < sizeof(QualCfg) / 4; i += blockDim.x) ((uint32_t*)&cfg)[i] = ((const uint32_t*)cfgp)[i];
	__syncthreads();
	const uint32_t r = r0 + blockIdx.x * 4 + (threadIdx.x >> 6);
	if (r >= r1) return;
	const uint32_t lane = threadIdx.x & 63;
	const uint64_t qb = qoff[r]; const uint32_t len = (uint32_t)(qoff[r + 1] - qb);
	const uint64_t wb = word_off[r];
	const uint32_t navg = cfg.navg;
	const bool per_base = !(cfg.mode == QM_AVERAGE || cfg.mode == QM_NONE);
	const uint64_t s_read = (per_base ? (qb - q0) : 0) + (uint64_t)(r - r0) * navg;
	const uint64_t k_read = qb - q0;
	const uint32_t part = part_of_read(lay, r);
	bool out_of_range = false;

	if (navg)
	{
		uint32_t sum[5] = { 0, 0, 0, 0, 0 }, cnt[5] = { 0, 0, 0, 0, 0 };
		for (uint32_t i = lane; i < len; i += 64)
		{
			uint32_t q = quals[qb + i] - 33u;
			out_of_range |= q > 95u;
			uint32_t b = cfg.mode == QM_AVERAGE ? 0u : cfg.map_fwd[q > 95u ? 0u : q];
#pragma unroll
			for (uint32_t t = 0; t < 5; ++t) if (b == t) { sum[t] += q; cnt[t] += 1; }
		}
#pragma unroll
		for (uint32_t t = 0; t < 5; ++t) { sum[t] = wave_sum(sum[t]); cnt[t] = wave_sum(cnt[t]); }
		if (lane == 0)
		{
			const uint64_t bo = (uint64_t)(r - r0) * navg;
			if (cfg.mode == QM_AVERAGE)
			{
				double avg = (double)sum[0] / (double)len;
				uint32_t a = (uint32_t)(avg * 256), a1 = a >> 8, a2 = a & 0xff;
				bkey[bo] = (0u << 8) | a1; bsidx[bo] = trip_index(lay, part, s_read);
				bkey[bo + 1] = ((640u + a1) << 8) | a2; bsidx[bo + 1] = trip_index(lay, part, s_read + 1);
			}
			else
			{
				uint32_t ctx_p = 0;
				for (uint32_t t = 0; t < cfg.n_bins; ++t)
				{
					double avg = cnt[t] ? (double)sum[t] / (double)cnt[t] : 0.0;
					uint32_t a = (uint32_t)(avg * 256), a1 = a >> 8, a2 = a & 0xff;
					bkey[bo + 2 * t] = ((t * 128u + ctx_p) << 8) | a1; bsidx[bo + 2 * t] = trip_index(lay, part, s_read + 2 * t);
					bkey[bo + 2 * t + 1] = ((640u + a1) << 8) | a2; bsidx[bo + 2 * t + 1] = trip_index(lay, part, s_read + 2 * t + 1);
					ctx_p = (uint32_t)avg;
				}
			}
		}
	}
	if (cfg.mode == QM_AVERAGE || cfg.mode == QM_NONE) { if (__ballot(out_of_range) && lane == 0) atomicOr(bad, 1u); return; }

	const uint32_t radix = cfg.hist_radix, missing = radix - 1;
	for (uint32_t i = lane; i < len; i += 64)
	{
		uint32_t qv = quals[qb + i] - 33u;
		if (qv > 95u) { out_of_range = true; qv = 0; }
		uint32_t sym = cfg.map_fwd[qv];
		uint32_t hist = 0, place = 1;
		for (uint32_t t = 1; t <= cfg.n_ctx_sym; ++t, place *= radix)
		{
			uint32_t v = missing;
			if (i >= t)
			{
				const uint32_t qp = quals[qb + i - t] - 33u;
				uint32_t s = cfg.map_fwd[qp > 95u ? 0u : qp];
				v = cfg.mode == QM_ORIGINAL ? (cfg.quant[s] & missing) : s;
			}
			hist = qual_hist_add(hist, place, v);
		}
		uint32_t b0 = arena_base(packed, wb, i);
		uint32_t bm1 = i > 0 ? arena_base(packed, wb, i - 1) : 0;
		uint32_t bm2 = i > 1 ? arena_base(packed, wb, i - 2) : 0;
		uint32_t bp1 = i + 1 < len ? arena_base(packed, wb, i + 1) : 0;
		uint32_t bctx;
		if (cfg.is_avg) bctx = (bm2 << 6) | (bm1 << 4) | (b0 << 2) | bp1;
		else if (cfg.is_thr) bctx = b0 | (bm1 << 2) | (bm2 << 4) | (bp1 << 6);
		else if (cfg.level == 3) bctx = b0 | (bm1 << 2) | (bm2 << 4) | (bp1 << 6);
		else bctx = b0 | (bm1 << 2) | ((uint32_t)(i > 1 && bm2 == bm1) << 4) | (bp1 << 5);
		uint32_t fl = 0;
		if (cfg.level > 1 && flags) { uint8_t c = flags[qb + i]; fl = (c == 'M' ? 1u : 0u) | (c == 'A' ? 2u : 0u); }
		key[k_read + i] = (qual_ctx_id(cfg, hist, bctx, fl) << cfg.sym_bits) | sym;
		sidx_out[k_read + i] = trip_index(lay, part, s_read + navg + i);
	}
	if (__ballot(out_of_range) && lane == 0) atomicOr(bad, 1u);
}

__global__ void k_seg_bounds(const uint32_t* __restrict__ skey, uint64_t n, uint32_t shift, uint32_t* __restrict__ seg_start, uint32_t* __restrict__ seg_end)
{
	uint64_t j = (uint64_t)blockIdx.x * blockDim.x + threadIdx.x;
	if (j >= n) return;
	uint32_t c = skey[j] >> shift;
	if (j == 0 || (skey[j - 1] >> shift) != c) seg_start[c] = (uint32_t)j;
	if (j + 1 == n || (skey[j + 1] >> shift) != c) seg_end[c] = (uint32_t)j + 1;
}

__device__ inline uint32_t wave_ctx_lower_bound(const uint32_t* __restrict__ skey, uint32_t lo, uint32_t n, uint32_t shift, uint32_t c, uint32_t lane)
{
	uint32_t hi = n;
	while (hi > lo)
	{
		const uint32_t step = (hi - lo) / 64 + 1;
		const uint64_t p = (uint64_t)lo + (uint64_t)(lane + 1) * step - 1;
		const bool ge = p < hi ? (skey[p] >> shift) >= c : true;
		const uint32_t f = (uint32_t)__builtin_ctzll(__ballot(ge));
		const uint64_t nhi = (uint64_t)lo + (uint64_t)(f + 1) * step - 1;
		lo += f * step;
		if (nhi < hi) hi = (uint32_t)nhi;
	}
	return lo;
}

template<uint32_t A>
__global__ __launch_bounds__(256) void k_evolve_small(const uint32_t* __restrict__ skey, const uint32_t* __restrict__ sval, uint32_t n,
                                                     uint32_t n_ctx, uint32_t sym_bits, uint32_t max_total, uint32_t adder,
                                                     uint32_t* __restrict__ state, triple_t* __restrict__ trip)
{
	const uint32_t c = blockIdx.x * 4 + (threadIdx.x >> 6);
	if (c >= n_ctx) return;
	const uint32_t lane = threadIdx.x & 63;
	const uint32_t s = wave_ctx_lower_bound(skey, 0, n, sym_bits, c, lane);
	if (s >= n || (skey[s] >> sym_bits) != c) return;
	const uint32_t e = wave_ctx_lower_bound(skey, s + 1, n, sym_bits, c + 1, lane);
	const uint64_t lt = (1ULL << lane) - 1;
	uint32_t st[A]; uint32_t tot;
#pragma unroll
	for (uint32_t a = 0; a < A; ++a) st[a] = state[(uint64_t)c * (A + 1) + a];
	tot = state[(uint64_t)c * (A + 1) + A];
	const uint32_t smask = (1u << sym_bits) - 1;
	uint32_t nkey = s + lane < e ? skey[s + lane] : 0u, nval = s + lane < e ? sval[s + lane] : 0u;
	for (uint32_t j0 = s; j0 < e; j0 += 64)
	{
		const uint32_t j = j0 + lane;
		const bool valid = j < e;
		const uint32_t sym = valid ? (nkey & smask) : 0xffu;
		const uint32_t dst = valid ? nval : 0u;
		{ const uint32_t jn = j + 64; const bool vn = jn < e; nkey = vn ? skey[jn] : 0u; nval = vn ? sval[jn] : 0u; }
		uint64_t m[A];
#pragma unroll
		for (uint32_t a = 0; a < A; ++a) m[a] = __ballot(valid && sym == a);
		const uint32_t cnt = (e - j0) < 64 ? (e - j0) : 64;
		uint32_t start = 0;
		while (start < cnt)
		{
			uint32_t r = (max_total - tot + adder - 1) / adder;
			uint32_t now = (cnt - start) < r ? (cnt - start) : r;
			uint64_t win = (now == 64 ? ~0ULL : ((1ULL << now) - 1)) << start;
			if (lane >= start && lane < start + now)
			{
				uint64_t before = lt & win;
				uint32_t cum = 0, freq = 0;
#pragma unroll
				for (uint32_t a = 0; a < A; ++a)
				{
					uint32_t v = st[a] + adder * (uint32_t)__popcll(m[a] & before);
					if (a < sym) cum += v;
					if (a == sym) freq = v;
				}
				trip[dst] = pack_triple(cum, freq, tot + adder * (lane - start));
			}
#pragma unroll
			for (uint32_t a = 0; a < A; ++a) st[a] += adder * (uint32_t)__popcll(m[a] & win);
			tot += adder * now;
			while (tot >= max_total)
			{
				tot = 0;
#pragma unroll
				for (uint32_t a = 0; a < A; ++a) { st[a] = (st[a] + 1) / 2; tot += st[a]; }
			}
			start += now;
		}
	}
	if (lane == 0)
	{
#pragma unroll
		for (uint32_t a = 0; a < A; ++a) state[(uint64_t)c * (A + 1) + a] = st[a];
		state[(uint64_t)c * (A + 1) + A] = tot;
	}
}

__global__ __launch_bounds__(256) void k_evolve_large(const uint32_t* __restrict__ skey, const uint32_t* __restrict__ sval,
                                                     const uint32_t* __restrict__ seg_start, const uint32_t* __restrict__ seg_end, uint32_t n,
                                                     uint32_t n_ctx, uint32_t n_sym, uint32_t sym_bits, uint32_t max_total, uint32_t adder,
                                                     uint32_t* __restrict__ state, triple_t* __restrict__ trip)
{
	__shared__ uint32_t s_cnt[4][256];
	__shared__ uint32_t s_pre[4][256];
	const uint32_t w = threadIdx.x >> 6;
	const uint32_t c = blockIdx.x * 4 + w;
	if (c >= n_ctx) return;
	const uint32_t lane = threadIdx.x & 63;
	uint32_t s, e;
	if (seg_start) { s = seg_start[c]; e = seg_end[c]; }
	else
	{
		s = wave_ctx_lower_bound(skey, 0, n, sym_bits, c, lane);
		e = s < n && (skey[s] >> sym_bits) == c ? wave_ctx_lower_bound(skey, s + 1, n, sym_bits, c + 1, lane) : s;
	}
	if (e <= s) return;
	uint32_t* sp = state + (uint64_t)c * (n_sym + 1);
	uint32_t* cnt = s_cnt[w]; uint32_t* pre = s_pre[w];
#pragma unroll
	for (uint32_t t = 0; t < 4; ++t) { uint32_t a = lane * 4 + t; cnt[a] = a < n_sym ? sp[a] : 0u; }
	uint32_t tot = sp[n_sym];
	auto rebuild_prefix = [&]() {
		uint32_t v0 = cnt[lane * 4], v1 = cnt[lane * 4 + 1], v2 = cnt[lane * 4 + 2], v3 = cnt[lane * 4 + 3];
		uint32_t sum = v0 + v1 + v2 + v3;
		uint32_t ex = wave_incl_scan(sum) - sum;
		pre[lane * 4] = ex; pre[lane * 4 + 1] = ex + v0; pre[lane * 4 + 2] = ex + v0 + v1; pre[lane * 4 + 3] = ex + v0 + v1 + v2;
		__builtin_amdgcn_wave_barrier();
	};
	__builtin_amdgcn_wave_barrier();
	rebuild_prefix();
	const uint32_t smask = (1u << sym_bits) - 1;
	for (uint32_t j0 = s; j0 < e; j0 += 64)
	{
		const uint32_t j = j0 + lane;
		const bool valid = j < e;
		const uint32_t sym = valid ? (skey[j] & smask) : 0u;
		const uint32_t dst = valid ? sval[j] : 0u;
		const uint32_t n_here = (e - j0) < 64 ? (e - j0) : 64;
		uint32_t start = 0;
		while (start < n_here)
		{
			const uint32_t r = (max_total - tot + adder - 1) / adder;
			const uint32_t now = (n_here - start) < r ? (n_here - start) : r;
			uint32_t less = 0, eq = 0;
			for (uint32_t l = start; l < start + now; ++l)
			{
				const uint32_t o = __builtin_amdgcn_readlane(sym, l);
				if (l < lane) { less += (o < sym) ? 1u : 0u; eq += (o == sym) ? 1u : 0u; }
			}
			const bool mine = lane >= start && lane < start + now;
			if (mine) trip[dst] = pack_triple(pre[sym] + adder * less, cnt[sym] + adder * eq, tot + adder * (lane - start));
			__builtin_amdgcn_wave_barrier();
			if (mine) atomicAdd(&cnt[sym], adder);
			__builtin_amdgcn_wave_barrier();
			tot += adder * now;
			while (tot >= max_total)
			{
				uint32_t sum = 0;
#pragma unroll
				for (uint32_t t = 0; t < 4; ++t) { uint32_t a = lane * 4 + t; if (a < n_sym) { uint32_t v = (cnt[a] + 1) / 2; cnt[a] = v; sum += v; } }
				tot = wave_sum(sum);
			}
			__builtin_amdgcn_wave_barrier();
			rebuild_prefix();
			start += now;
		}
	}
#pragma unroll
	for (uint32_t t = 0; t < 4; ++t) { uint32_t a = lane * 4 + t; if (a < n_sym) sp[a] = cnt[a]; }
	if (lane == 0) sp[n_sym] = tot;
}

__global__ void k_gather_u64(const uint64_t* __restrict__ src, const uint32_t* __restrict__ idx, uint64_t n, uint64_t* __restrict__ dst)
{ uint64_t i = (uint64_t)blockIdx.x * blockDim.x + threadIdx.x; if (i < n) dst[i] = src[idx[i]]; }
__global__ void k_fill_u32(uint32_t* v, uint64_t n, uint32_t x) { uint64_t i = (uint64_t)blockIdx.x * blockDim.x + threadIdx.x; if (i < n) v[i] = x; }
__global__ void k_init_state(uint32_t* st, uint64_t n_ctx, uint32_t n_sym)
{
	uint64_t i = (uint64_t)blockIdx.x * blockDim.x + threadIdx.x;
	if (i >= n_ctx * (n_sym + 1)) return;
	st[i] = (i % (n_sym + 1)) == n_sym ? n_sym : 1u;
}
__global__ void k_gather_bytes(const uint8_t* __restrict__ src, const uint64_t* __restrict__ src_off, const uint64_t* __restrict__ dst_off,
                               const uint64_t* __restrict__ size, uint8_t* __restrict__ dst)
{
	const uint32_t p = blockIdx.x;
	const uint64_t n = size[p]; const uint8_t* s = src + src_off[p]; uint8_t* d = dst + dst_off[p];
	for (uint64_t i = threadIdx.x; i < n; i += blockDim.x) d[i] = s[i];
}

void fill_range(uint8_t* a, int lo, int hi, uint8_t v) { for (int i = lo; i < hi; ++i) a[i] = v; }
}

extern "C" cl_status cl_qual_coder_create(cl_ctx* ctx, const cl_qual_params* prm, cl_qual_coder** out)
{
	if (!ctx || !prm || !out) return cl_fail(ctx, CL_E_INVALID, "cl_qual_coder_create: null argument");
	if (prm->mode < 0 || prm->mode > QM_NONE || prm->source < 0 || prm->source > 2 || prm->level < 1 || prm->level > 3)
		return cl_fail(ctx, CL_E_INVALID, "cl_qual_coder_create: mode 0..8, source 0..2, level 1..3");
	HIP_TRY(ctx, hipSetDevice(ctx->device));
	cl_qual_coder* Q = new cl_qual_coder(); Q->ctx = ctx;
	std::unique_ptr<cl_qual_coder> guard(Q);
	QualCfg& c = Q->cfg; memset(&c, 0, sizeof(c));
	c.mode = prm->mode; c.level = prm->level;
	c.max_total = 1u << 18; c.adder = 8;
	auto bins = [&](uint32_t n) -> cl_status {
		if (prm->n_fwd != n - 1) return cl_fail(ctx, CL_E_INVALID, "cl_qual_coder_create: need " + std::to_string(n - 1) + " thresholds");
		for (uint32_t i = 0; i + 1 < n - 1; ++i) if (prm->fwd[i] > prm->fwd[i + 1]) return cl_fail(ctx, CL_E_INVALID, "thresholds must ascend");
		if (prm->fwd[n - 2] > 96) return cl_fail(ctx, CL_E_INVALID, "threshold > 96");
		fill_range(c.map_fwd, 0, (int)prm->fwd[0], 0);
		for (uint32_t b = 1; b + 1 < n; ++b) fill_range(c.map_fwd, (int)prm->fwd[b - 1], (int)prm->fwd[b], (uint8_t)b);
		fill_range(c.map_fwd, (int)prm->fwd[n - 2], 96, (uint8_t)(n - 1));
		c.n_bins = n; c.n_sym = n;
		return CL_OK;
	};
	switch (prm->mode)
	{
	case QM_ORIGINAL:
	{
		for (int i = 0; i < 96; ++i) c.map_fwd[i] = (uint8_t)i;
		static const int ont3[] = { 0, 1, 2, 4, 7, 11, 16, 22, 29, 37, 46, 56, 67, 79, 90, 96 };
		static const int ont12[] = { 0, 1, 2, 5, 10, 15, 20, 25, 35, 50, 70, 96 };
		static const int pb3[] = { 0, 1, 10, 20, 30, 39, 45, 51, 57, 63, 69, 75, 81, 87, 93, 94 };
		static const int pb12[] = { 0, 1, 15, 29, 41, 53, 63, 72, 80, 87, 93, 94 };
		const int* t; int n;
		if (prm->source == 0) { if (prm->level == 3) { t = ont3; n = 15; } else { t = ont12; n = 11; } }
		else { if (prm->level == 3) { t = pb3; n = 15; } else { t = pb12; n = 11; } }
		for (int b = 0; b < n; ++b) fill_range(c.quant, t[b], t[b + 1], (uint8_t)b);
		if (prm->source == 2) { for (int i = 0; i < 93; ++i) c.quant[i] += 1; c.quant[93] = 0; }
		c.bits_per_sym = 4; c.n_ctx_sym = 2; c.n_sym = 96; c.max_total = 1u << 20; c.adder = 32;
		c.base_bits = prm->level == 3 ? 8 : 7;
		break;
	}
	case QM_QUINARY_AVG: CL_TRY(bins(5)); c.bits_per_sym = 3; c.n_ctx_sym = 3; c.is_avg = 1; c.navg = 10; c.base_bits = 8; break;
	case QM_QUAD_AVG: CL_TRY(bins(4)); c.bits_per_sym = 3; c.n_ctx_sym = 3; c.is_avg = 1; c.navg = 8; c.base_bits = 8; break;
	case QM_BINARY_AVG: CL_TRY(bins(2)); c.bits_per_sym = 2; c.n_ctx_sym = 6; c.is_avg = 1; c.navg = 4; c.base_bits = 8; break;
	case QM_QUINARY_THR: CL_TRY(bins(5)); c.bits_per_sym = 3; c.n_ctx_sym = 3; c.is_thr = 1; c.base_bits = 8; break;
	case QM_QUAD_THR: CL_TRY(bins(4)); c.bits_per_sym = 3; c.n_ctx_sym = 3; c.is_thr = 1; c.base_bits = 8; break;
	case QM_BINARY_THR: CL_TRY(bins(2)); c.bits_per_sym = 2; c.n_ctx_sym = 6; c.is_thr = 1; c.base_bits = 8; break;
	case QM_AVERAGE: c.navg = 2; c.n_sym = 2; break;
	case QM_NONE: c.n_sym = 2; break;
	}
	c.ctx_bits = c.bits_per_sym * c.n_ctx_sym;
	c.sym_bits = 1; while ((1u << c.sym_bits) < c.n_sym) ++c.sym_bits;
	c.hist_radix = qual_hist_radix(c); c.n_hist = 1;
	for (uint32_t t = 0; t < c.n_ctx_sym; ++t) c.n_hist *= c.hist_radix;
	const uint64_t n_ctx64 = (uint64_t)c.n_hist << (c.base_bits + (c.level > 1 ? 2 : 0));
	if (n_ctx64 > (1ull << 30)) return cl_fail(ctx, CL_E_UNSUPPORTED, "cl_qual_coder_create: context does not fit 32-bit keys");
	c.n_ctx = (c.mode == QM_AVERAGE || c.mode == QM_NONE) ? 1u : (uint32_t)n_ctx64;
	c.dense_bits = 0; while ((1ull << c.dense_bits) < c.n_ctx) ++c.dense_bits;
	if (c.dense_bits + c.sym_bits > 32 || (c.n_ctx > 1 && qual_ctx_id(c, c.n_hist - 1, (1u << c.base_bits) - 1, c.level > 1 ? 3u : 0u) != c.n_ctx - 1))
		return cl_fail(ctx, CL_E_UNSUPPORTED, "cl_qual_coder_create: context ids do not fit the bits the sort is asked for");
	DEV_ALLOC(ctx, Q->d_cfg, 1);
	HIP_TRY(ctx, hipMemcpyAsync(Q->d_cfg.p, &c, sizeof(c), hipMemcpyHostToDevice, ctx->stream));
	DEV_ALLOC(ctx, Q->state, (uint64_t)c.n_ctx * (c.n_sym + 1));
	LAUNCH(ctx, k_init_state, grid_for((uint64_t)c.n_ctx * (c.n_sym + 1), 256), 256, Q->state.p, (uint64_t)c.n_ctx, c.n_sym);
	DEV_ALLOC(ctx, Q->bstate, (uint64_t)BYTE_CTX * 257);
	LAUNCH(ctx, k_init_state, grid_for((uint64_t)BYTE_CTX * 257, 256), 256, Q->bstate.p, (uint64_t)BYTE_CTX, 256u);
	HIP_TRY(ctx, hipGetLastError());
	HIP_TRY(ctx, hipStreamSynchronize(ctx->stream));
	*out = guard.release();
	return CL_OK;
}
extern "C" cl_ctx* cl_qual_coder_ctx(const cl_qual_coder* q) { return q ? q->ctx : nullptr; }
extern "C" void cl_qual_coder_free(cl_qual_coder* q) { delete q; }

namespace {
cl_status qual_prepare(cl_ctx* ctx, cl_qual_coder* Q, const cl_reads* R, const uint8_t* d_quals, const uint64_t* d_qual_off,
                       const uint8_t* d_flags, const uint32_t* h_part_bounds, uint32_t n_parts, QualPrepared& P)
{
	const QualCfg& c = Q->cfg;
	P.R = R; P.d_quals = d_quals; P.part_bounds.assign(h_part_bounds, h_part_bounds + n_parts + 1);
	std::vector<uint64_t> qo(n_parts + 1);
	{
		DevBuf<uint32_t> d_pb; DEV_ALLOC(ctx, d_pb, (uint64_t)n_parts + 1);
		DevBuf<uint64_t> d_qo; DEV_ALLOC(ctx, d_qo, (uint64_t)n_parts + 1);
		HIP_TRY(ctx, hipMemcpyAsync(d_pb.p, h_part_bounds, ((uint64_t)n_parts + 1) * 4, hipMemcpyHostToDevice, ctx->stream));
		LAUNCH(ctx, k_gather_u64, grid_for((uint64_t)n_parts + 1, 256), 256, d_qual_off, (const uint32_t*)d_pb.p, (uint64_t)n_parts + 1, d_qo.p);
		HIP_TRY(ctx, hipMemcpyAsync(qo.data(), d_qo.p, ((uint64_t)n_parts + 1) * 8, hipMemcpyDeviceToHost, ctx->stream));
		HIP_TRY(ctx, hipStreamSynchronize(ctx->stream));
	}
	DevBuf<uint32_t> bad; DEV_ALLOC(ctx, bad, 1);
	HIP_TRY(ctx, hipMemsetAsync(bad.p, 0, 4, ctx->stream));
	auto refuse_bad = [&]() -> cl_status {
		uint32_t h_bad = 0;
		HIP_TRY(ctx, hipMemcpyAsync(&h_bad, bad.p, 4, hipMemcpyDeviceToHost, ctx->stream));
		HIP_TRY(ctx, hipStreamSynchronize(ctx->stream));
		if (h_bad) return cl_fail(ctx, CL_E_INVALID, "cl_qual_encode: quality byte outside '!'..'~'+1 (Phred+33 values 0..95)");
		return CL_OK;
	};
	const uint64_t GROUP_SYMS = (1ull << 31) - (1ull << 24);
	uint32_t p0 = 0;
	while (p0 < n_parts)
	{
		auto Gp = std::make_unique<QualGroupPrep>(); QualGroupPrep& G = *Gp;
		uint32_t p1 = p0 + 1;
		const bool per_base = !(c.mode == QM_AVERAGE);
		auto syms_of = [&](uint32_t a, uint32_t b) { return (per_base ? (qo[b] - qo[a]) : 0) + (uint64_t)(h_part_bounds[b] - h_part_bounds[a]) * c.navg; };
		while (p1 < n_parts && syms_of(p0, p1 + 1) <= GROUP_SYMS) ++p1;
		const uint32_t r0 = h_part_bounds[p0], r1 = h_part_bounds[p1];
		const uint64_t n_base = qo[p1] - qo[p0], n_syms = syms_of(p0, p1), n_byte = (uint64_t)(r1 - r0) * c.navg;
		if (n_syms >= (1ull << 32)) return cl_fail(ctx, CL_E_UNSUPPORTED, "cl_qual_encode: a single part has >= 2^32 symbols");
		const uint32_t np = p1 - p0;
		const uint32_t ng = (np + 63) / 64;
		G.p0 = p0; G.p1 = p1; G.np = np; G.ng = ng; G.n_base = per_base ? n_base : 0; G.n_syms = n_syms; G.n_byte = n_byte;
		std::vector<uint64_t> sym_start(np + 1), gbase(ng + 1);
		std::vector<uint32_t> plen(np), pfirst(np + 1);
		sym_start[0] = 0;
		for (uint32_t p = 0; p < np; ++p)
		{
			uint64_t sl = syms_of(p0 + p, p0 + p + 1);
			if (sl >= (1ull << 31)) return cl_fail(ctx, CL_E_UNSUPPORTED, "cl_qual_encode: a part has >= 2^31 symbols");
			plen[p] = (uint32_t)sl; sym_start[p + 1] = sym_start[p] + sl; pfirst[p] = h_part_bounds[p0 + p];
		}
		pfirst[np] = h_part_bounds[p1];
		std::vector<uint32_t> order(np); std::vector<uint32_t>& rank = G.rank; std::vector<uint32_t>& plen_r = G.plen_r;
		rank.resize(np); plen_r.resize(np);
		for (uint32_t p = 0; p < np; ++p) order[p] = p;
		std::stable_sort(order.begin(), order.end(), [&](uint32_t a, uint32_t b) { return plen[a] > plen[b]; });
		for (uint32_t i = 0; i < np; ++i) { rank[order[i]] = i; plen_r[i] = plen[order[i]]; }
		gbase[0] = 0;
		for (uint32_t g = 0; g < ng; ++g) gbase[g + 1] = gbase[g] + trip_group_words(plen_r[g * 64]);
		if (gbase[ng] >= (1ull << 32)) return cl_fail(ctx, CL_E_UNSUPPORTED, "cl_qual_encode: group too large for 32-bit triple indices");
		G.trip_words = gbase[ng];
		DevBuf<uint64_t> d_sym_start; DevBuf<uint32_t> d_pfirst, d_rank;
		DEV_ALLOC(ctx, d_sym_start, np + 1); DEV_ALLOC(ctx, G.d_gbase, ng + 1); DEV_ALLOC(ctx, G.d_plen, np); DEV_ALLOC(ctx, d_pfirst, np + 1); DEV_ALLOC(ctx, d_rank, np);
		HIP_TRY(ctx, hipMemcpyAsync(d_rank.p, rank.data(), np * 4, hipMemcpyHostToDevice, ctx->stream));
		HIP_TRY(ctx, hipMemcpyAsync(d_sym_start.p, sym_start.data(), (np + 1) * 8, hipMemcpyHostToDevice, ctx->stream));
		HIP_TRY(ctx, hipMemcpyAsync(G.d_gbase.p, gbase.data(), (ng + 1) * 8, hipMemcpyHostToDevice, ctx->stream));
		HIP_TRY(ctx, hipMemcpyAsync(G.d_plen.p, plen_r.data(), np * 4, hipMemcpyHostToDevice, ctx->stream));
		HIP_TRY(ctx, hipMemcpyAsync(d_pfirst.p, pfirst.data(), (np + 1) * 4, hipMemcpyHostToDevice, ctx->stream));
		TripLayoutDev lay{ d_pfirst.p, d_sym_start.p, G.d_gbase.p, np, d_rank.p };
		DevBuf<uint32_t>& key = G.key; DevBuf<uint32_t>& sidx = G.sidx; DevBuf<uint32_t>& bkey = G.bkey; DevBuf<uint32_t>& bsidx = G.bsidx;
		DEV_ALLOC(ctx, key, per_base ? n_base : 0); DEV_ALLOC(ctx, sidx, per_base ? n_base : 0);
		DEV_ALLOC(ctx, bkey, n_byte); DEV_ALLOC(ctx, bsidx, n_byte);
		if (r1 > r0)
			LAUNCHB(ctx, n_base * (1.0 + 0.25 + 8.0) + n_byte * 8.0, k_qual_symbols, grid_for(r1 - r0, 4), 256, (const QualCfg*)Q->d_cfg.p, (const uint64_t*)R->packed.p, (const uint64_t*)R->word_off.p,
				d_quals, d_qual_off, d_flags, r0, r1, qo[p0], lay, key.p, sidx.p, bkey.p, bsidx.p, bad.p);
		HIP_TRY(ctx, hipGetLastError());
		if (per_base && n_base) CL_TRY(dev_sort_keys32_pairs(ctx, key.p, sidx.p, n_base, c.sym_bits, c.sym_bits + c.dense_bits));
		if (n_byte)
		{
			CL_TRY(dev_sort_keys32_pairs(ctx, bkey.p, bsidx.p, n_byte, 8, 8 + 10));
			DEV_ALLOC(ctx, G.bss, BYTE_CTX); DEV_ALLOC(ctx, G.bse, BYTE_CTX);
			HIP_TRY(ctx, hipMemsetAsync(G.bss.p, 0, BYTE_CTX * 4, ctx->stream));
			HIP_TRY(ctx, hipMemsetAsync(G.bse.p, 0, BYTE_CTX * 4, ctx->stream));
			LAUNCH(ctx, k_seg_bounds, grid_for(n_byte, 256), 256, (const uint32_t*)bkey.p, n_byte, 8u, G.bss.p, G.bse.p);
			HIP_TRY(ctx, hipGetLastError());
		}
		CL_TRY(refuse_bad());
		P.groups.push_back(std::move(Gp));
		p0 = p1;
	}
	return CL_OK;
}
}
cl_status cl_qual_prepare_batch(cl_ctx* ctx, cl_qual_coder* Q, const cl_reads* R, const uint8_t* d_quals, const uint64_t* d_qual_off,
                                const uint8_t* d_flags, const uint32_t* h_part_bounds, uint32_t n_parts, QualPrepared** out)
{
	if (!ctx || !Q || !R || !d_qual_off || !h_part_bounds || !n_parts || !out || Q->cfg.mode == QM_NONE) return CL_E_INVALID;
	HIP_TRY(ctx, hipSetDevice(ctx->device));
	for (uint32_t p = 0; p < n_parts; ++p) if (h_part_bounds[p] > h_part_bounds[p + 1]) return CL_E_INVALID;
	if (h_part_bounds[n_parts] > R->n_reads) return CL_E_INVALID;
	auto P = std::make_unique<QualPrepared>();
	CL_TRY(qual_prepare(ctx, Q, R, d_quals, d_qual_off, d_flags, h_part_bounds, n_parts, *P));
	*out = P.release();
	return CL_OK;
}
void cl_qual_prepared_free(QualPrepared* P) { delete P; }
void cl_qual_set_ahead(cl_qual_coder* Q, QualPrepared* P) { if (Q) Q->ahead.reset(P); else delete P; }

namespace {
cl_status qual_evolve_batch(cl_ctx* ctx, cl_qual_coder* Q, const cl_reads* R, const uint8_t* d_quals, const uint64_t* d_qual_off, const uint8_t* d_flags,
                            const uint32_t* h_part_bounds, uint32_t n_parts, std::unique_ptr<QualPrepared> Pp, QualEvolved& E)
{
	const QualCfg& c = Q->cfg;
	if (Pp && !(Pp->R == R && Pp->d_quals == d_quals && Pp->part_bounds.size() == (size_t)n_parts + 1 && memcmp(Pp->part_bounds.data(), h_part_bounds, ((size_t)n_parts + 1) * 4) == 0)) Pp.reset();
	if (!Pp) { Pp = std::make_unique<QualPrepared>(); CL_TRY(qual_prepare(ctx, Q, R, d_quals, d_qual_off, d_flags, h_part_bounds, n_parts, *Pp)); }
	E.R = R; E.d_quals = d_quals; E.part_bounds.assign(h_part_bounds, h_part_bounds + n_parts + 1);
	const uint32_t bits_max = c.max_total == (1u << 20) ? 20 : 18;
	const uint64_t* inv_tab = nullptr;
	CL_TRY(cl_inv_table(ctx, &inv_tab));
	for (auto& Gp : Pp->groups)
	{
		QualGroupPrep& G = *Gp;
		const uint32_t np = G.np, ng = G.ng;
		const uint64_t n_base = G.n_base, n_syms = G.n_syms, n_byte = G.n_byte;
		auto Pn = std::make_unique<QualPending>(); QualPending& PG = *Pn;
		PG.p0 = G.p0; PG.np = np; PG.rank = G.rank; PG.n_syms = n_syms;
		PG.d_gbase = std::move(G.d_gbase); PG.d_plen = std::move(G.d_plen);
		DevBuf<triple_t>& trip = PG.trip; DEV_ALLOC(ctx, trip, G.trip_words);
		if (n_base)
		{
			const uint32_t g = grid_for(c.n_ctx, 4);
			switch (c.n_sym)
			{
			case 2: LAUNCHB(ctx, n_base * 16.0, (k_evolve_small<2>), g, 256, (const uint32_t*)G.key.p, (const uint32_t*)G.sidx.p, (uint32_t)n_base, c.n_ctx, c.sym_bits, c.max_total, c.adder, Q->state.p, trip.p); break;
			case 4: LAUNCHB(ctx, n_base * 16.0, (k_evolve_small<4>), g, 256, (const uint32_t*)G.key.p, (const uint32_t*)G.sidx.p, (uint32_t)n_base, c.n_ctx, c.sym_bits, c.max_total, c.adder, Q->state.p, trip.p); break;
			case 5: LAUNCHB(ctx, n_base * 16.0, (k_evolve_small<5>), g, 256, (const uint32_t*)G.key.p, (const uint32_t*)G.sidx.p, (uint32_t)n_base, c.n_ctx, c.sym_bits, c.max_total, c.adder, Q->state.p, trip.p); break;
			default: LAUNCHB(ctx, n_base * 16.0, k_evolve_large, g, 256, (const uint32_t*)G.key.p, (const uint32_t*)G.sidx.p, (const uint32_t*)nullptr, (const uint32_t*)nullptr, (uint32_t)n_base, c.n_ctx, c.n_sym, c.sym_bits, c.max_total, c.adder, Q->state.p, trip.p); break;
			}
			HIP_TRY(ctx, hipGetLastError());
		}
		if (n_byte)
		{
			LAUNCH(ctx, k_evolve_large, grid_for(BYTE_CTX, 4), 256, (const uint32_t*)G.bkey.p, (const uint32_t*)G.bsidx.p, (const uint32_t*)G.bss.p, (const uint32_t*)G.bse.p, (uint32_t)n_byte,
				BYTE_CTX, 256u, 8u, 1u << 18, 8u, Q->bstate.p, trip.p);
			HIP_TRY(ctx, hipGetLastError());
		}
		std::vector<uint64_t> out_off(np + 1);
		out_off[0] = 0;
		for (uint32_t p = 0; p < np; ++p)
		{
			uint64_t s = G.plen_r[p];
			out_off[p + 1] = out_off[p] + ((s * bits_max + 7) / 8 + s / 16 + 64 + 7) / 8 * 8;
		}
		DEV_ALLOC(ctx, PG.tmp, out_off[np]);
		DEV_ALLOC(ctx, PG.d_out_off, np + 1); DEV_ALLOC(ctx, PG.d_size, np); DEV_ALLOC(ctx, PG.d_dst_off, np);
		HIP_TRY(ctx, hipMemcpyAsync(PG.d_out_off.p, out_off.data(), (np + 1) * 8, hipMemcpyHostToDevice, ctx->stream));
		HIP_TRY(ctx, hipStreamSynchronize(ctx->stream));
		G.key.release(); G.sidx.release(); G.bkey.release(); G.bsidx.release();
		if (Q->cstreams.size() < 4) { hipStream_t ns = nullptr; HIP_TRY(ctx, cl_stream_create_role(CL_ROLE_CODER, cl_level_to_prio(cl_role_level(CL_ROLE_CODER, 0)), &ns)); Q->cstreams.push_back(ns); }
		PG.stream = Q->cstreams[Q->next_cstream++ % Q->cstreams.size()];
		{
			LaunchOn on(ctx, PG.stream);
			LAUNCH_RANGE_CODE(ctx, n_syms * 8.0, ng, (const triple_t*)trip.p, (const uint64_t*)PG.d_gbase.p, (const uint32_t*)PG.d_plen.p, np, PG.tmp.p, (const uint64_t*)PG.d_out_off.p, PG.d_size.p, inv_tab);
			hipError_t e2 = hipGetLastError();
			HIP_TRY(ctx, e2);
		}
		E.groups.push_back(std::move(Pn));
	}
	return CL_OK;
}
}
cl_status cl_qual_evolve_ahead(cl_ctx* ctx, cl_qual_coder* Q, const cl_reads* R, const uint8_t* d_quals, const uint64_t* d_qual_off, const uint32_t* h_part_bounds, uint32_t n_parts, QualPrepared* P)
{
	std::unique_ptr<QualPrepared> Pp(P);
	if (!ctx || !Q || !R || !h_part_bounds || !n_parts || Q->evolved.size() >= 4 || Q->cfg.mode == QM_NONE) return CL_E_INVALID;
	auto E = std::make_unique<QualEvolved>();
	CL_TRY(qual_evolve_batch(ctx, Q, R, d_quals, d_qual_off, nullptr, h_part_bounds, n_parts, std::move(Pp), *E));
	Q->evolved.push_back(std::move(E));
	return CL_OK;
}
void cl_qual_set_before_tail(cl_qual_coder* Q, std::function<cl_status()> fn) { if (Q) Q->before_tail = std::move(fn); }

extern "C" cl_status cl_qual_encode(cl_ctx* ctx, cl_qual_coder* Q, const cl_reads* R, const uint8_t* d_quals, const uint64_t* d_qual_off,
                                    const uint8_t* d_flags, const uint32_t* h_part_bounds, uint32_t n_parts,
                                    uint8_t* d_out, uint64_t cap, uint64_t* h_part_sizes, uint64_t* n_out)
{
	if (!ctx || !Q || !R || !d_qual_off || !h_part_bounds || !h_part_sizes || !n_out) return cl_fail(ctx, CL_E_INVALID, "cl_qual_encode: null argument");
	HIP_TRY(ctx, hipSetDevice(ctx->device));
	const QualCfg& c = Q->cfg;
	for (uint32_t p = 0; p < n_parts; ++p) if (h_part_bounds[p] > h_part_bounds[p + 1]) return cl_fail(ctx, CL_E_INVALID, "cl_qual_encode: part bounds must ascend");
	if (n_parts && h_part_bounds[n_parts] > R->n_reads) return cl_fail(ctx, CL_E_INVALID, "cl_qual_encode: part bound beyond the arena");
	*n_out = 0;
	std::unique_ptr<QualPrepared> Pp = std::move(Q->ahead);
	std::unique_ptr<QualEvolved> Ep;
	if (!Q->evolved.empty()) { Ep = std::move(Q->evolved.front()); Q->evolved.pop_front(); }
	if (!n_parts) return Ep ? cl_fail(ctx, CL_E_INVALID, "cl_qual_encode: the batch evolved ahead is not the one encoded next") : CL_OK;
	if (c.mode == QM_NONE)
	{
		if (cap < 8ull * n_parts) { *n_out = 8ull * n_parts; return cl_fail(ctx, CL_E_CAPACITY, "cl_qual_encode: output capacity"); }
		HIP_TRY(ctx, hipMemsetAsync(d_out, 0, 8ull * n_parts, ctx->stream));
		HIP_TRY(ctx, hipStreamSynchronize(ctx->stream));
		for (uint32_t p = 0; p < n_parts; ++p) h_part_sizes[p] = 8;
		*n_out = 8ull * n_parts;
		return CL_OK;
	}
	if (Ep)
	{
		if (!(Ep->R == R && Ep->d_quals == d_quals && Ep->part_bounds.size() == (size_t)n_parts + 1 && memcmp(Ep->part_bounds.data(), h_part_bounds, ((size_t)n_parts + 1) * 4) == 0))
			return cl_fail(ctx, CL_E_INVALID, "cl_qual_encode: the batch evolved ahead is not the one encoded next");
	}
	else { Ep = std::make_unique<QualEvolved>(); CL_TRY(qual_evolve_batch(ctx, Q, R, d_quals, d_qual_off, d_flags, h_part_bounds, n_parts, std::move(Pp), *Ep)); }
	if (Q->before_tail)
		for (;;)
		{
			const cl_status hs = Q->before_tail();
			if (hs == CL_OK) break;
			if (hs != CL_HOOK_RETRY) return hs;
			bool running = false;
			for (auto& g : Ep->groups) if (hipStreamQuery(g->stream) == hipErrorNotReady) running = true;
			(void)hipGetLastError();
			if (!running) break;
			std::this_thread::sleep_for(std::chrono::milliseconds(1));
		}
	uint64_t written = 0;
	for (auto& Pn : Ep->groups)
	{
		QualPending& PG = *Pn;
		const uint32_t p0 = PG.p0, np = PG.np;
		HIP_TRY(ctx, hipStreamSynchronize(PG.stream));
		std::vector<uint64_t> size_r(np);
// ... 22 lines not shown
```

### colord_amd/csrc/rc_dev.hpp

```cpp
#pragma once
#include "common.hpp"
#include <type_traits>

typedef uint64_t triple_t;
__device__ inline triple_t pack_triple(uint32_t cum, uint32_t freq, uint32_t tot)
{
	return ((uint64_t)cum << 42) | ((uint64_t)freq << 21) | tot;
}
constexpr uint32_t INV_TABLE_SIZE = 1u << 21;
static __global__ void k_fill_inv_table(uint64_t* __restrict__ tab)
{
	const uint32_t i = blockIdx.x * blockDim.x + threadIdx.x;
	if (i < INV_TABLE_SIZE) tab[i] = i ? ~0ULL / (uint64_t)i : ~0ULL;
}
static inline cl_status cl_inv_table(cl_ctx* ctx, const uint64_t** out)
{
	if (!ctx->inv_tab)
	{
		HIP_TRY(ctx, hipMalloc((void**)&ctx->inv_tab, (uint64_t)INV_TABLE_SIZE * 8));
		hipLaunchKernelGGL(k_fill_inv_table, dim3(INV_TABLE_SIZE / 256), dim3(256), 0, ctx->stream, ctx->inv_tab);
		HIP_TRY(ctx, hipGetLastError());
		HIP_TRY(ctx, hipStreamSynchronize(ctx->stream));
	}
	*out = ctx->inv_tab;
	return CL_OK;
}

#ifndef CL_TRIP_RUN
#define CL_TRIP_RUN 1
#endif
constexpr uint32_t TRIP_RUN = CL_TRIP_RUN;
__host__ __device__ inline uint64_t trip_slot(uint64_t group_base, uint32_t place, uint64_t pos) { return group_base + (pos / TRIP_RUN) * (64ull * TRIP_RUN) + (uint64_t)place * TRIP_RUN + pos % TRIP_RUN; }
__host__ __device__ inline uint64_t trip_group_words(uint64_t longest_part) { return (longest_part + TRIP_RUN - 1) / TRIP_RUN * TRIP_RUN * 64; }
struct TripLayoutDev {
	const uint32_t* part_first_read;
	const uint64_t* part_sym_start;
	const uint64_t* group_base;
	uint32_t np;
	const uint32_t* rank = nullptr;
};
__device__ inline uint32_t part_of_read(const TripLayoutDev& L, uint32_t r)
{
	uint32_t lo = 0, hi = L.np;
	while (hi - lo > 1) { uint32_t mid = (lo + hi) >> 1; if (L.part_first_read[mid] <= r) lo = mid; else hi = mid; }
	return lo;
}
__device__ inline uint32_t trip_index(const TripLayoutDev& L, uint32_t part, uint64_t stream_pos)
{
	const uint32_t pl = L.rank ? L.rank[part] : part;
	return (uint32_t)trip_slot(L.group_base[pl >> 6], pl & 63, stream_pos - L.part_sym_start[part]);
}

struct __attribute__((packed)) unaligned_u64 { uint64_t v; };
__device__ inline void store_be64(uint8_t* p, uint64_t v) { ((unaligned_u64*)p)->v = __builtin_bswap64(v); }

constexpr uint32_t RING = 256, RING_UNIT = 128, RING_STRIDE = 8 + RING + 8 + 4;
typedef uint64_t __attribute__((may_alias, aligned(1))) u64_any;
typedef uint32_t __attribute__((may_alias, aligned(1))) u32_any;
__device__ inline void lds_store_be64(uint8_t* p, uint64_t v) { *(u64_any*)p = __builtin_bswap64(v); }

static __global__ __launch_bounds__(64) void k_range_code(const triple_t* __restrict__ trip, const uint64_t* __restrict__ group_base,
                                                         const uint32_t* __restrict__ part_len, uint32_t n_parts,
                                                         uint8_t* __restrict__ out, const uint64_t* __restrict__ part_out_off, uint64_t* __restrict__ part_size,
                                                         const uint64_t* __restrict__ inv_tab)
{
	__builtin_amdgcn_s_setprio(3);
	const uint32_t p = blockIdx.x * 64 + threadIdx.x;
	const bool live = p < n_parts;
	const uint64_t MASK = 0xff00000000000000ULL;
	uint64_t low = 0, range = MASK;
	const uint64_t out_off = live ? part_out_off[p] : 0;
	uint8_t* outp = out + out_off;
	const uint64_t cap = live ? part_out_off[p + 1] - part_out_off[p] : 0;
	uint32_t n_out = 0; bool overflow = cap < 8 || cap > 0xfffffff0ull;
	__shared__ __attribute__((aligned(16))) uint8_t s_ring[64 * RING_STRIDE];
	uint8_t* const ring = s_ring + threadIdx.x * RING_STRIDE + 8;
	const uint32_t room = overflow ? 0u : (uint32_t)cap;
	uint32_t flushed = 0;
	auto drain = [&]()
	{
		static_assert(RING_UNIT - 1 + 8 * 8 + 8 <= RING, "a round's bytes must fit behind an incomplete unit");
		uint64_t m;
		while ((m = __ballot(n_out - flushed >= RING_UNIT)) != 0)
		{
			const int L = __builtin_ctzll(m);
			const uint32_t fl = __builtin_amdgcn_readlane(flushed, L), rm = __builtin_amdgcn_readlane(room, L);
			const uint64_t o = ((uint64_t)(uint32_t)__builtin_amdgcn_readlane((uint32_t)(out_off >> 32), L) << 32) | (uint32_t)__builtin_amdgcn_readlane((uint32_t)out_off, L);
			if (fl + RING_UNIT <= rm && threadIdx.x < RING_UNIT / 4)
			{
				const uint32_t w = *(const u32_any*)(s_ring + L * RING_STRIDE + 8 + (fl & (RING - 1)) + threadIdx.x * 4);
				*(u32_any*)(out + o + fl + threadIdx.x * 4) = w;
			}
			if ((int)threadIdx.x == L) flushed += RING_UNIT;
		}
	};
	const uint32_t len = live ? part_len[p] : 0;
	uint32_t lmax = len;
#pragma unroll
	for (int d = 32; d > 0; d >>= 1) { uint32_t t = __shfl_xor(lmax, d, 64); lmax = t > lmax ? t : lmax; }
	if (lmax == 0) { if (live) { if (!overflow) store_be64(outp, 0); part_size[p] = overflow ? ~0ULL : 8; } return; }
	const triple_t* src = trip + group_base[blockIdx.x] + threadIdx.x * TRIP_RUN;
	auto at = [](uint32_t q) -> uint64_t { return (uint64_t)(q / TRIP_RUN) * (64 * TRIP_RUN) + q % TRIP_RUN; };
	constexpr uint32_t U = 8;
	static_assert(U % TRIP_RUN == 0, "a round of the coder takes whole runs of a lane's triples");
	triple_t A[U], B[U], C[U]; uint64_t iA[U], iB[U], iC[U];
	const uint64_t NEUTRAL_X = (1ULL << 21) | 1ULL, NEUTRAL_Y = ~0ULL;
	const uint32_t last = lmax - 1;
#pragma unroll
	for (uint32_t u = 0; u < U; ++u) { A[u] = src[at(u < last ? u : last)]; B[u] = src[at(U + u < last ? U + u : last)]; }
#pragma unroll
	for (uint32_t u = 0; u < U; ++u) iA[u] = inv_tab[A[u] & 0x1fffff];
	auto round = [&](auto all_active, uint32_t pos, const triple_t (&cur)[U], const uint64_t (&icur)[U], const triple_t (&nxt)[U], uint64_t (&inxt)[U], triple_t (&far)[U])
	{
		{
			const uint32_t q0 = pos + 2 * U;
			if (TRIP_RUN == U && q0 + U - 1 <= last)
			{
				const ulonglong2* v = (const ulonglong2*)(src + at(q0));
#pragma unroll
				for (uint32_t u = 0; u < U; u += 2) { const ulonglong2 w = v[u / 2]; far[u] = w.x; far[u + 1] = w.y; }
			}
			else
			{
#pragma unroll
				for (uint32_t u = 0; u < U; ++u) { const uint32_t q = q0 + u; far[u] = src[at(q < last ? q : last)]; }
			}
		}
#pragma unroll
		for (uint32_t u = 0; u < U; ++u) inxt[u] = inv_tab[nxt[u] & 0x1fffff];
#pragma unroll
		for (uint32_t u = 0; u < U; ++u)
		{
			const bool act = decltype(all_active)::value || pos + u < len;
			const uint64_t tx = act ? cur[u] : NEUTRAL_X, inv = act ? icur[u] : NEUTRAL_Y;
			const uint32_t tot = (uint32_t)(tx & 0x1fffff), freq = (uint32_t)((tx >> 21) & 0x1fffff), cum = (uint32_t)(tx >> 42);
			uint64_t q = __umul64hi(range, inv);
			const uint32_t r = (uint32_t)range - (uint32_t)q * tot;
			q += (uint32_t)(r >= tot);
			low += q * cum;
			range = q * freq;
			const uint64_t low0 = low;
			uint32_t nb = 0;
			uint32_t rh = (uint32_t)(range >> 32), rl = (uint32_t)range, lh = (uint32_t)(low >> 32), ll = (uint32_t)low;
			asm volatile("" : "+v"(rh), "+v"(rl), "+v"(lh), "+v"(ll));
			auto step = [&]()
			{
				const bool need = rh < 0x00010000u;
				const uint32_t sh = lh + rh + (uint32_t)(rl > ~ll);
				const bool straddle = (lh ^ sh) > 0x00ffffffu;
				const uint32_t fh = straddle ? (~lh & 0x0000ffffu) : rh, fl = straddle ? ~ll : rl;
				rh = need ? __builtin_amdgcn_alignbit(fh, fl, 24) : rh; rl = need ? fl << 8 : rl;
				lh = need ? __builtin_amdgcn_alignbit(lh, ll, 24) : lh; ll = need ? ll << 8 : ll;
				nb += need ? 1u : 0u;
			};
			step();
			if (__any(rh < 0x00010000u))
			{
#pragma unroll 1
				for (uint32_t it = 1; it < 8; ++it) { step(); if (!__any(rh < 0x00010000u)) break; }
			}
			range = ((uint64_t)rh << 32) | rl; low = ((uint64_t)lh << 32) | ll;
			if (nb) { const uint32_t rp = n_out & (RING - 1); lds_store_be64(ring + rp, low0); if (rp > RING - 8) lds_store_be64(ring + rp - RING, low0); }
			n_out += nb;
		}
		drain();
	};
	uint32_t lmin = live ? len : 0u;
#pragma unroll
	for (int d = 32; d > 0; d >>= 1) { uint32_t t = __shfl_xor(lmin, d, 64); lmin = t < lmin ? t : lmin; }
	const std::true_type ALL{}; const std::false_type SOME{};
	uint32_t pos = 0;
	for (; pos + 3 * U <= lmin; pos += 3 * U)
	{
		round(ALL, pos, A, iA, B, iB, C);
		round(ALL, pos + U, B, iB, C, iC, A);
		round(ALL, pos + 2 * U, C, iC, A, iA, B);
	}
	for (; pos < lmax; pos += 3 * U)
	{
		round(SOME, pos, A, iA, B, iB, C);
		if (pos + U >= lmax) break;
		round(SOME, pos + U, B, iB, C, iC, A);
		if (pos + 2 * U >= lmax) break;
		round(SOME, pos + 2 * U, C, iC, A, iA, B);
	}
	{
		{ const uint32_t rp = n_out & (RING - 1); lds_store_be64(ring + rp, low); if (rp > RING - 8) lds_store_be64(ring + rp - RING, low); }
		n_out += 8;
		if (!live || n_out > room || (uint32_t)(range >> 32) < 0x00010000u) overflow = true;
		drain();
		const uint32_t rem = overflow ? 0u : n_out - flushed;
		for (int L = 0; L < 64; ++L)
		{
			const uint32_t n = __builtin_amdgcn_readlane(rem, L), fl = __builtin_amdgcn_readlane(flushed, L);
			if (n == 0) continue;
			const uint64_t o = ((uint64_t)(uint32_t)__builtin_amdgcn_readlane((uint32_t)(out_off >> 32), L) << 32) | (uint32_t)__builtin_amdgcn_readlane((uint32_t)out_off, L);
			for (uint32_t b = threadIdx.x; b < n; b += 64) out[o + fl + b] = s_ring[L * RING_STRIDE + 8 + ((fl + b) & (RING - 1))];
		}
		if (live) part_size[p] = overflow ? ~0ULL : n_out;
	}
}

#define LAUNCH_RANGE_CODE(ctx, bytes, ng, ...) LAUNCHB_NAMED(ctx, "k_range_code", bytes, k_range_code, ng, 64, __VA_ARGS__)
```

### colord_amd/csrc/sort.hip

```cpp
#include "common.hpp"
#include <string>

namespace {
constexpr uint32_t ST = 256;
constexpr uint32_t SI = 16;
constexpr uint32_t STILE = ST * SI;

template<typename K, uint32_t DB, uint32_t G>
__global__ __launch_bounds__(ST) void k_sort_hist(const K* __restrict__ keys, uint64_t n, uint32_t shift, uint32_t dmask,
                                                  uint32_t* __restrict__ hist, uint32_t nb)
{
	constexpr uint32_t ND = 1u << DB;
	constexpr uint32_t ROW = G > 1 ? ND + 1 : ND;
	__shared__ uint32_t h[G * ROW];
	for (uint32_t i = threadIdx.x; i < G * ROW; i += ST) h[i] = 0;
	__syncthreads();
	const uint32_t tile0 = blockIdx.x * G;
	for (uint32_t g = 0; g < G && tile0 + g < nb; ++g)
	{
		const uint64_t base = (uint64_t)(tile0 + g) * STILE;
#pragma unroll
		for (uint32_t i = 0; i < SI; ++i)
		{
			uint64_t idx = base + (uint64_t)i * ST + threadIdx.x;
			if (idx < n) atomicAdd(&h[g * ROW + ((uint32_t)(keys[idx] >> shift) & dmask)], 1u);
		}
	}
	__syncthreads();
	for (uint32_t i = threadIdx.x; i < G * ND; i += ST)
	{
		const uint32_t g = i % G, d = i / G;
		if (tile0 + g < nb) hist[(uint64_t)d * nb + tile0 + g] = h[g * ROW + d];
	}
}

template<typename K, bool HAS_V, uint32_t DB>
__global__ __launch_bounds__(ST) void k_sort_scatter(const K* __restrict__ kin, const uint32_t* __restrict__ vin,
                                                     K* __restrict__ kout, uint32_t* __restrict__ vout,
                                                     uint64_t n, uint32_t shift, uint32_t dmask, const uint32_t* __restrict__ offs, uint32_t nb)
{
	constexpr uint32_t ND = 1u << DB, PER = ND / ST;
	__shared__ uint32_t wh[4][ND];
	__shared__ uint32_t lstart[ND + 1];
	__shared__ uint32_t gdelta[ND];
	__shared__ uint32_t wtot[4];
	__shared__ K skey[STILE];
	__shared__ uint32_t sval[HAS_V ? STILE : 1];
	const uint32_t w = threadIdx.x >> 6, lane = threadIdx.x & 63;
	for (uint32_t i = threadIdx.x; i < 4 * ND; i += ST) (&wh[0][0])[i] = 0;
	__syncthreads();

	const uint64_t tbase = (uint64_t)blockIdx.x * STILE, wbase = tbase + (uint64_t)w * (64 * SI);
	K key[SI]; uint32_t rank[SI]; uint32_t val[HAS_V ? SI : 1];
	const uint64_t lt = (1ULL << lane) - 1;
	uint32_t goff[PER];
#pragma unroll
	for (uint32_t k = 0; k < PER; ++k) goff[k] = offs[(uint64_t)(threadIdx.x * PER + k) * nb + blockIdx.x];
#pragma unroll
	for (uint32_t r = 0; r < SI; ++r)
	{
		uint64_t idx = wbase + (uint64_t)r * 64 + lane;
		key[r] = idx < n ? kin[idx] : (K)0;
		if (HAS_V) val[r] = idx < n ? vin[idx] : 0u;
	}
#pragma unroll
	for (uint32_t r = 0; r < SI; ++r)
	{
		uint64_t idx = wbase + (uint64_t)r * 64 + lane;
		bool valid = idx < n;
		uint32_t d = (uint32_t)(key[r] >> shift) & dmask;
		uint64_t peers = __ballot(valid);
#pragma unroll
		for (uint32_t b = 0; b < DB; ++b)
		{
			bool bit = (d >> b) & 1u;
			uint64_t m = __ballot(valid && bit);
			peers &= bit ? m : ~m;
		}
		uint32_t prior = valid ? wh[w][d] : 0u;
		rank[r] = prior + (uint32_t)__popcll(peers & lt);
		__builtin_amdgcn_wave_barrier();
		if (valid && (peers & lt) == 0) wh[w][d] = prior + (uint32_t)__popcll(peers);
		__builtin_amdgcn_wave_barrier();
	}
	__syncthreads();
	{
		uint32_t c[PER][4], tot[PER], mine = 0;
#pragma unroll
		for (uint32_t k = 0; k < PER; ++k)
		{
			const uint32_t d = threadIdx.x * PER + k;
			c[k][0] = wh[0][d]; c[k][1] = wh[1][d]; c[k][2] = wh[2][d]; c[k][3] = wh[3][d];
			tot[k] = c[k][0] + c[k][1] + c[k][2] + c[k][3]; mine += tot[k];
		}
		uint32_t incl = mine;
#pragma unroll
		for (uint32_t o = 1; o < 64; o <<= 1) { const uint32_t t = __shfl_up(incl, o, 64); if (lane >= o) incl += t; }
		if (lane == 63) wtot[w] = incl;
		__syncthreads();
		uint32_t ls = incl - mine;
		for (uint32_t i = 0; i < w; ++i) ls += wtot[i];
#pragma unroll
		for (uint32_t k = 0; k < PER; ++k)
		{
			const uint32_t d = threadIdx.x * PER + k;
			lstart[d] = ls;
			if (d == ND - 1) lstart[ND] = ls + tot[k];
			gdelta[d] = goff[k] - ls;
			wh[0][d] = ls; wh[1][d] = ls + c[k][0]; wh[2][d] = ls + c[k][0] + c[k][1]; wh[3][d] = ls + c[k][0] + c[k][1] + c[k][2];
			ls += tot[k];
		}
	}
	__syncthreads();
#pragma unroll
	for (uint32_t r = 0; r < SI; ++r)
	{
		uint64_t idx = wbase + (uint64_t)r * 64 + lane;
		if (idx < n)
		{
			uint32_t d = (uint32_t)(key[r] >> shift) & dmask;
			uint32_t lp = wh[w][d] + rank[r];
			skey[lp] = key[r];
			if (HAS_V) sval[lp] = val[r];
		}
	}
	__syncthreads();
	const uint32_t tile_n = lstart[ND];
	for (uint32_t j = threadIdx.x; j < tile_n; j += ST)
	{
		const K k = skey[j];
		const uint32_t pos = gdelta[(uint32_t)(k >> shift) & dmask] + j;
		kout[pos] = k;
		if (HAS_V) vout[pos] = sval[j];
	}
}

template<typename K, uint32_t DB>
cl_status sort_pass(cl_ctx* ctx, const K* kin, const uint32_t* vin, K* kout, uint32_t* vout, uint64_t n, uint32_t shift, uint32_t dmask, uint32_t* hist, uint32_t nb)
{
	static const std::string kt = sizeof(K) == 8 ? "unsigned long" : "unsigned int", db = std::to_string(DB) + "u";
	constexpr uint32_t G = DB == 8 ? 16 : 4; const bool grouped = nb >= 4096;
	static const std::string n_hist1 = "k_sort_hist<" + kt + ", " + db + ", 1u>", n_histg = "k_sort_hist<" + kt + ", " + db + ", " + std::to_string(G) + "u>", n_sv = "k_sort_scatter<" + kt + ", true, " + db + ">", n_sk = "k_sort_scatter<" + kt + ", false, " + db + ">";
	if (grouped) LAUNCHB_NAMED(ctx, n_histg.c_str(), n * sizeof(K), (k_sort_hist<K, DB, G>), (nb + G - 1) / G, ST, kin, n, shift, dmask, hist, nb);
	else LAUNCHB_NAMED(ctx, n_hist1.c_str(), n * sizeof(K), (k_sort_hist<K, DB, 1>), nb, ST, kin, n, shift, dmask, hist, nb);
	HIP_TRY(ctx, hipGetLastError());
	CL_TRY(dev_exclusive_scan_u32(ctx, hist, (uint64_t)(1u << DB) * nb, nullptr));
	if (vin) LAUNCHB_NAMED(ctx, n_sv.c_str(), n * (2 * sizeof(K) + 8), (k_sort_scatter<K, true, DB>), nb, ST, kin, vin, kout, vout, n, shift, dmask, (const uint32_t*)hist, nb);
	else LAUNCHB_NAMED(ctx, n_sk.c_str(), n * 2 * sizeof(K), (k_sort_scatter<K, false, DB>), nb, ST, kin, (const uint32_t*)nullptr, kout, (uint32_t*)nullptr, n, shift, dmask, (const uint32_t*)hist, nb);
	HIP_TRY(ctx, hipGetLastError());
	return CL_OK;
}

template<typename K>
cl_status sort_impl(cl_ctx* ctx, K* d_keys, uint32_t* d_vals, uint64_t n, uint32_t begin_bit, uint32_t end_bit, DevBuf<K>* swap_k = nullptr, DevBuf<uint32_t>* swap_v = nullptr)
{
	if (n <= 1 || end_bit <= begin_bit) return CL_OK;
	if (n >= (1ULL << 32)) return cl_fail(ctx, CL_E_UNSUPPORTED, "radix sort: n must be < 2^32 per call");
	const uint32_t nb = grid_for(n, STILE);
	const uint32_t bits = end_bit - begin_bit;
	const uint32_t n_pass_real = (bits + 7) / 8 == (bits + 9) / 10 ? (bits + 7) / 8 : (bits + 9) / 10;
	const uint32_t db_hi = (bits + n_pass_real - 1) / n_pass_real;
	const bool third = (n_pass_real & 1) && n_pass_real > 1 && n * (sizeof(K) + (d_vals ? 4 : 0)) <= (2ull << 30);
	const uint32_t n_pass = third ? n_pass_real : (n_pass_real + 1) & ~1u;
	DevBuf<K> ktmp, ktmp2; DEV_ALLOC(ctx, ktmp, n);
	DevBuf<uint32_t> vtmp, vtmp2; if (d_vals) DEV_ALLOC(ctx, vtmp, n);
	if (n_pass & 1) { DEV_ALLOC(ctx, ktmp2, n); if (d_vals) DEV_ALLOC(ctx, vtmp2, n); }
	DevBuf<uint32_t> hist; DEV_ALLOC(ctx, hist, (uint64_t)(1u << std::max(8u, db_hi)) * nb);
	K* kin = d_keys; uint32_t* vin = d_vals;
	uint32_t pass = 0;
	for (uint32_t shift = begin_bit; shift < end_bit; ++pass)
	{
		K* kout; uint32_t* vout;
		if (n_pass & 1) { kout = pass == 0 ? ktmp2.p : (pass & 1) ? ktmp.p : d_keys; vout = pass == 0 ? vtmp2.p : (pass & 1) ? vtmp.p : d_vals; }
		else { kout = (pass & 1) ? d_keys : ktmp.p; vout = (pass & 1) ? d_vals : vtmp.p; }
		const uint32_t left = end_bit - shift, passes_left = n_pass_real - pass;
		const uint32_t db = std::max(8u, (left + passes_left - 1) / passes_left);
		const uint32_t use = std::min(db, 10u);
		const uint32_t dmask = (1u << std::min(use, left)) - 1;
		if (use == 10) CL_TRY((sort_pass<K, 10>(ctx, kin, vin, kout, vout, n, shift, dmask, hist.p, nb)));
		else if (use == 9) CL_TRY((sort_pass<K, 9>(ctx, kin, vin, kout, vout, n, shift, dmask, hist.p, nb)));
		else CL_TRY((sort_pass<K, 8>(ctx, kin, vin, kout, vout, n, shift, dmask, hist.p, nb)));
		shift += use;
		kin = kout; vin = vout;
	}
	if (kin != d_keys && swap_k && kin == ktmp.p && (!d_vals || (swap_v && vin == vtmp.p)))
	{
		std::swap(*swap_k, ktmp);
		if (d_vals) std::swap(*swap_v, vtmp);
	}
	else if (kin != d_keys)
	{
		HIP_TRY(ctx, hipMemcpyAsync(d_keys, kin, n * sizeof(K), hipMemcpyDeviceToDevice, cl_launch_stream(ctx)));
		if (d_vals) HIP_TRY(ctx, hipMemcpyAsync(d_vals, vin, n * 4, hipMemcpyDeviceToDevice, cl_launch_stream(ctx)));
	}
	HIP_TRY(ctx, hipStreamSynchronize(cl_launch_stream(ctx)));
	return CL_OK;
}
}

cl_status dev_sort_pairs(cl_ctx* ctx, uint64_t* d_keys, uint32_t* d_vals, uint64_t n, uint32_t begin_bit, uint32_t end_bit)
{
	return sort_impl<uint64_t>(ctx, d_keys, d_vals, n, begin_bit, end_bit);
}
cl_status dev_sort_pairs_swap(cl_ctx* ctx, DevBuf<uint64_t>& keys, DevBuf<uint32_t>& vals, uint64_t n, uint32_t begin_bit, uint32_t end_bit)
{
	if (keys.n != n || vals.n != n) return sort_impl<uint64_t>(ctx, keys.p, vals.p, n, begin_bit, end_bit);
	return sort_impl<uint64_t>(ctx, keys.p, vals.p, n, begin_bit, end_bit, &keys, &vals);
}
cl_status dev_sort_keys32_pairs(cl_ctx* ctx, uint32_t* d_keys, uint32_t* d_vals, uint64_t n, uint32_t begin_bit, uint32_t end_bit)
{
	return sort_impl<uint32_t>(ctx, d_keys, d_vals, n, begin_bit, end_bit);
}
cl_status dev_sort_keys32_pairs_swap(cl_ctx* ctx, DevBuf<uint32_t>& keys, DevBuf<uint32_t>& vals, uint64_t n, uint32_t begin_bit, uint32_t end_bit)
{
	if (keys.n != n || vals.n != n) return sort_impl<uint32_t>(ctx, keys.p, vals.p, n, begin_bit, end_bit);
	return sort_impl<uint32_t>(ctx, keys.p, vals.p, n, begin_bit, end_bit, &keys, &vals);
}
```

Baseline: 2.905.

## Fuse slot-index and qual key generation into first radix sort pass

Adds generic source objects so the first radix-sort pass computes its (key, value) pairs on the fly instead of reading them from buffers that a separate kernel filled. For DNA, the trip-slot index is derived inside the histogram and scatter kernels using wave-cooperative binary searches over partition starts, which removes k_fill_sidx and its write and read of the sidx array. For quality, key and slot computation is factored out so it can run inside the sort's first pass. This trades a pass of memory traffic for extra searches and per-element compute, and the histogram kernel may have to recompute the keys as well.

```diff
diff --git a/colord_amd/csrc/common.hpp b/colord_amd/csrc/common.hpp
--- a/colord_amd/csrc/common.hpp
+++ b/colord_amd/csrc/common.hpp
@@ -540,6 +540,28 @@
 	return v;
 }
 
+template<typename T>
+__device__ static inline uint32_t last_le(const T* __restrict__ a, uint32_t lo, uint32_t hi, T x)
+{
+	while (hi - lo > 1) { const uint32_t mid = lo + ((hi - lo) >> 1); if (a[mid] <= x) lo = mid; else hi = mid; }
+	return lo;
+}
+template<typename T>
+__device__ static inline uint32_t wave_last_le(const T* __restrict__ a, uint32_t lo, uint32_t hi, T x)
+{
+	while (hi - lo > 1)
+	{
+		const uint32_t step = (hi - lo - 1) / 64 + 1;
+		const uint64_t p = (uint64_t)lo + (uint64_t)(lane_id() + 1) * step;
+		const bool gt = p < hi ? a[p] > x : true;
+		const uint32_t f = (uint32_t)__builtin_ctzll(__ballot(gt));
+		const uint64_t nhi = (uint64_t)lo + (uint64_t)(f + 1) * step;
+		lo += f * step;
+		if (nhi < hi) hi = (uint32_t)nhi;
+	}
+	return lo;
+}
+
 __device__ static inline uint32_t block_excl_scan_256(uint32_t v, uint32_t* sh, uint32_t* total)
 {
 	uint32_t incl = wave_incl_scan(v);
diff --git a/colord_amd/csrc/dna.hip b/colord_amd/csrc/dna.hip
--- a/colord_amd/csrc/dna.hip
+++ b/colord_amd/csrc/dna.hip
@@ -2,6 +2,7 @@
 #include <functional>
 #include "objects.hpp"
 #include "rc_dev.hpp"
+#include "sort_dev.hpp"
 #include <algorithm>
 #include <deque>
 #include <thread>
@@ -498,10 +499,45 @@
 	const uint32_t lane = threadIdx.x & 63;
 	const uint64_t a = sym_off[r] - s0, b = sym_off[r + 1] - s0;
 	if (a == b) return;
-	const uint32_t part = part_of_read(lay, r), pl = lay.rank ? lay.rank[part] : part;
-	const uint64_t gb = lay.group_base[pl >> 6], p0 = lay.part_sym_start[part];
-	for (uint64_t i = a + lane; i < b; i += 64) sidx[i] = (uint32_t)trip_slot(gb, pl & 63, i - p0);
-}
+	const TripPart tp = trip_part(lay, part_of_read(lay, r));
+	for (uint64_t i = a + lane; i < b; i += 64) sidx[i] = trip_index(tp, i);
+}
+template<typename K>
+struct SlotSource {
+	const K* __restrict__ kin; TripLayoutDev lay;
+	struct Cursor {
+		uint32_t p_lo, p_hi;
+		uint32_t a, len; TripPart tp;
+	};
+	template<bool PAIRS> __device__ Cursor begin(uint64_t first, uint64_t end) const
+	{
+		Cursor c; c.p_lo = c.p_hi = 0; c.a = 0; c.len = 0; c.tp = TripPart{ 0, 0, 0 };
+		if (!PAIRS || first >= end) return c;
+		const uint64_t* __restrict__ ps = lay.part_sym_start;
+		const uint32_t lo = wave_last_le(ps, 0u, lay.np, first);
+		const uint32_t j = lo + 1 + lane_id() < lay.np ? lo + 1 + lane_id() : lay.np;
+		const uint64_t m = __ballot(ps[j] > end - 1);
+		const uint32_t hi = m ? lo + (uint32_t)__builtin_ctzll(m) : wave_last_le(ps, lo + 64, lay.np, end - 1);
+		c.p_lo = __builtin_amdgcn_readfirstlane(lo); c.p_hi = __builtin_amdgcn_readfirstlane(hi);
+		return c;
+	}
+	__device__ K key(Cursor&, uint64_t idx) const { return kin[idx]; }
+	template<bool HAS_V> __device__ void pair(Cursor& c, uint64_t idx, K& k, uint32_t& v) const
+	{
+		k = kin[idx];
+		if ((uint32_t)idx - c.a >= c.len)
+		{
+			const uint32_t p = last_le(lay.part_sym_start, c.p_lo, c.p_hi + 1, idx);
+			c.a = (uint32_t)lay.part_sym_start[p]; c.len = (uint32_t)(lay.part_sym_start[p + 1] - lay.part_sym_start[p]);
+			c.tp = trip_part(lay, p);
+		}
+		v = trip_index(c.tp, idx);
+	}
+	static const char* suffix() { return "SlotSource"; }
+	static constexpr bool KEYS_ONLY = false;
+	double hist_bytes() const { return sizeof(K); }
+	double pair_bytes(bool) const { return sizeof(K); }
+};
 template<typename K>
 __global__ __launch_bounds__(256) void k_dna_plain(const FamTab* __restrict__ ftp, const uint8_t* __restrict__ es, const uint64_t* __restrict__ es_off,
                                                   const uint32_t* __restrict__ es_ntup, const uint8_t* __restrict__ read_flag, const uint32_t* __restrict__ hdr_counts,
@@ -909,6 +945,7 @@
 	FamTab ft;
 	DevBuf<FamTab> d_ft;
 	DevBuf<uint32_t> state;
+	bool slot_unfused = false;
 	uint32_t ctx_bits = 0; bool narrow = false;
 	uint32_t cur_read_id = 0;
 	uint32_t prev_types = 0;
@@ -958,6 +995,7 @@
 	f.ctx_base[N_FAM] = (uint32_t)cb; f.state_base[N_FAM] = sb;
 	if (cb >= (1ull << 32)) return cl_fail(ctx, CL_E_UNSUPPORTED, "cl_dna_coder_create: context space too large");
 	D->ctx_bits = 1; while ((1ull << D->ctx_bits) < cb) ++D->ctx_bits;
+	D->slot_unfused = getenv("COLORD_HIP_DNA_SLOT_UNFUSED") != nullptr;
 	D->narrow = D->ctx_bits + 8 <= 32 && !getenv("COLORD_HIP_DNA_WIDE_KEYS");
 	DEV_ALLOC(ctx, D->d_ft, 1);
 	HIP_TRY(ctx, hipMemcpyAsync(D->d_ft.p, &f, sizeof(f), hipMemcpyHostToDevice, ctx->stream));
@@ -1149,21 +1187,28 @@
 	if (n_syms)
 	{
 		DEV_ALLOC(ctx, G.sidx, n_syms);
-		LAUNCHB(ctx, n_syms * 4.0, k_fill_sidx, grid_for(nr, 4), 256, (const uint64_t*)W.sym_off.p, s0, r0, r1, lay, G.sidx.p);
+		const bool fused = !D->slot_unfused;
+		if (!fused) LAUNCHB(ctx, n_syms * 4.0, k_fill_sidx, grid_for(nr, 4), 256, (const uint64_t*)W.sym_off.p, s0, r0, r1, lay, G.sidx.p);
 		HIP_TRY(ctx, hipGetLastError());
 		const uint32_t cbits = D->ctx_bits;
 		const uint64_t seg_cap = std::min<uint64_t>(n_syms, D->ft.ctx_base[N_FAM]) + 1;
 		DEV_ALLOC(ctx, G.seg, seg_cap);
 		if (W.narrow)
 		{
-			if (s0 == 0 && W.key32.n == n_syms) CL_TRY(dev_sort_keys32_pairs_swap(ctx, W.key32, G.sidx, n_syms, 8, 8 + cbits));
+			const bool whole = s0 == 0 && W.key32.n == n_syms;
+			const SlotSource<uint32_t> src{ W.key32.p + s0, lay };
+			if (fused) CL_TRY((sort_impl<uint32_t, SlotSource<uint32_t>>(ctx, W.key32.p + s0, G.sidx.p, n_syms, 8, 8 + cbits, whole ? &W.key32 : nullptr, whole ? &G.sidx : nullptr, &src)));
+			else if (whole) CL_TRY(dev_sort_keys32_pairs_swap(ctx, W.key32, G.sidx, n_syms, 8, 8 + cbits));
 			else CL_TRY(dev_sort_keys32_pairs(ctx, W.key32.p + s0, G.sidx.p, n_syms, 8, 8 + cbits));
 			CL_TRY(dev_run_starts_u32(ctx, W.key32.p + s0, n_syms, 8, G.seg.p, seg_cap, &G.n_seg));
 			CL_TRY(dna_long_prepare<uint32_t>(ctx, D, W.key32.p + s0, n_syms, G));
 		}
 		else
 		{
-			if (s0 == 0 && W.key.n == n_syms) CL_TRY(dev_sort_pairs_swap(ctx, W.key, G.sidx, n_syms, 8, 8 + cbits));
+			const bool whole = s0 == 0 && W.key.n == n_syms;
+			const SlotSource<uint64_t> src{ W.key.p + s0, lay };
+			if (fused) CL_TRY((sort_impl<uint64_t, SlotSource<uint64_t>>(ctx, W.key.p + s0, G.sidx.p, n_syms, 8, 8 + cbits, whole ? &W.key : nullptr, whole ? &G.sidx : nullptr, &src)));
+			else if (whole) CL_TRY(dev_sort_pairs_swap(ctx, W.key, G.sidx, n_syms, 8, 8 + cbits));
 			else CL_TRY(dev_sort_pairs(ctx, W.key.p + s0, G.sidx.p, n_syms, 8, 8 + cbits));
 			CL_TRY(dev_run_starts_u64(ctx, W.key.p + s0, n_syms, 8, G.seg.p, seg_cap, &G.n_seg));
 			CL_TRY(dna_long_prepare<uint64_t>(ctx, D, W.key.p + s0, n_syms, G));
diff --git a/colord_amd/csrc/qual.hip b/colord_amd/csrc/qual.hip
--- a/colord_amd/csrc/qual.hip
+++ b/colord_amd/csrc/qual.hip
@@ -5,6 +5,7 @@
 #include <chrono>
 #include "objects.hpp"
 #include "rc_dev.hpp"
+#include "sort_dev.hpp"
 #include <algorithm>
 
 namespace {
@@ -54,6 +55,7 @@
 	std::unique_ptr<QualPrepared> ahead;
 	std::deque<std::unique_ptr<struct QualEvolved>> evolved;
 	std::function<cl_status()> before_tail;
+	bool unfused = false;
 	std::vector<hipStream_t> cstreams; uint32_t next_cstream = 0;
 	~cl_qual_coder();
 };
@@ -77,6 +79,89 @@
 	return (uint32_t)(packed[wb + (p >> 5)] >> (62 - 2 * (p & 31))) & 3u;
 }
 
+
+__device__ inline uint32_t qual_key_at(const QualCfg& cfg, const uint64_t* __restrict__ packed, const uint8_t* __restrict__ quals, const uint8_t* __restrict__ flags,
+                                       uint64_t qb, uint64_t wb, uint32_t len, uint32_t i, bool& out_of_range)
+{
+	const uint8_t* q = quals + qb + i;
+	uint32_t w0, w1 = 0;
+	if (i >= 3) w0 = *(const u32_any*)(q - 3);
+	else { w0 = (uint32_t)q[0] << 24; if (i >= 1) w0 |= (uint32_t)q[-1] << 16; if (i >= 2) w0 |= (uint32_t)q[-2] << 8; }
+	if (cfg.n_ctx_sym > 3)
+	{
+		if (i >= 7) w1 = *(const u32_any*)(q - 7);
+		else for (uint32_t t = 4; t <= i; ++t) w1 |= (uint32_t)q[-(int32_t)t] << (24 - 8 * (t - 4));
+	}
+	auto back = [&](uint32_t t) { return ((t < 4 ? w0 >> (24 - 8 * t) : w1 >> (24 - 8 * (t - 4))) & 0xffu) - 33u; };
+	uint32_t qv = back(0);
+	if (qv > 95u) { out_of_range = true; qv = 0; }
+	const uint32_t sym = cfg.map_fwd[qv];
+	const uint32_t radix = cfg.hist_radix, missing = radix - 1;
+	uint32_t hist = 0, place = 1;
+	for (uint32_t t = 1; t <= cfg.n_ctx_sym; ++t, place *= radix)
+	{
+		uint32_t v = missing;
+		if (i >= t)
+		{
+			const uint32_t qp = back(t);
+			uint32_t s = cfg.map_fwd[qp > 95u ? 0u : qp];
+			v = cfg.mode == QM_ORIGINAL ? (cfg.quant[s] & missing) : s;
+		}
+		hist = qual_hist_add(hist, place, v);
+	}
+	const uint32_t lo = i > 2 ? i - 2 : 0, hi = i + 1 < len ? i + 1 : len - 1;
+	const uint64_t wa = packed[wb + (lo >> 5)], wz = (hi >> 5) != (lo >> 5) ? packed[wb + (hi >> 5)] : wa;
+	auto base = [&](uint32_t p) { return (uint32_t)(((p >> 5) == (lo >> 5) ? wa : wz) >> (62 - 2 * (p & 31))) & 3u; };
+	uint32_t b0 = base(i);
+	uint32_t bm1 = i > 0 ? base(i - 1) : 0;
+	uint32_t bm2 = i > 1 ? base(i - 2) : 0;
+	uint32_t bp1 = i + 1 < len ? base(i + 1) : 0;
+	uint32_t bctx;
+	if (cfg.is_avg) bctx = (bm2 << 6) | (bm1 << 4) | (b0 << 2) | bp1;
+	else if (cfg.is_thr) bctx = b0 | (bm1 << 2) | (bm2 << 4) | (bp1 << 6);
+	else if (cfg.level == 3) bctx = b0 | (bm1 << 2) | (bm2 << 4) | (bp1 << 6);
+	else bctx = b0 | (bm1 << 2) | ((uint32_t)(i > 1 && bm2 == bm1) << 4) | (bp1 << 5);
+	uint32_t fl = 0;
+	if (cfg.level > 1 && flags) { uint8_t c = flags[qb + i]; fl = (c == 'M' ? 1u : 0u) | (c == 'A' ? 2u : 0u); }
+	return (qual_ctx_id(cfg, hist, bctx, fl) << cfg.sym_bits) | sym;
+}
+
+__device__ inline void qual_read_bytes(const QualCfg& cfg, const uint8_t* __restrict__ quals, uint64_t qb, uint32_t len, uint32_t lane, const TripLayoutDev& lay,
+                                       uint32_t part, uint64_t s_read, uint64_t bo, uint32_t* __restrict__ bkey, uint32_t* __restrict__ bsidx, bool& out_of_range)
+{
+	uint32_t sum[5] = { 0, 0, 0, 0, 0 }, cnt[5] = { 0, 0, 0, 0, 0 };
+	for (uint32_t i = lane; i < len; i += 64)
+	{
+		uint32_t q = quals[qb + i] - 33u;
+		out_of_range |= q > 95u;
+		uint32_t b = cfg.mode == QM_AVERAGE ? 0u : cfg.map_fwd[q > 95u ? 0u : q];
+#pragma unroll
+		for (uint32_t t = 0; t < 5; ++t) if (b == t) { sum[t] += q; cnt[t] += 1; }
+	}
+#pragma unroll
+	for (uint32_t t = 0; t < 5; ++t) { sum[t] = wave_sum(sum[t]); cnt[t] = wave_sum(cnt[t]); }
+	if (lane != 0) return;
+	if (cfg.mode == QM_AVERAGE)
+	{
+		double avg = (double)sum[0] / (double)len;
+		uint32_t a = (uint32_t)(avg * 256), a1 = a >> 8, a2 = a & 0xff;
+		bkey[bo] = (0u << 8) | a1; bsidx[bo] = trip_index(lay, part, s_read);
+		bkey[bo + 1] = ((640u + a1) << 8) | a2; bsidx[bo + 1] = trip_index(lay, part, s_read + 1);
+	}
+	else
+	{
+		uint32_t ctx_p = 0;
+		for (uint32_t t = 0; t < cfg.n_bins; ++t)
+		{
+			double avg = cnt[t] ? (double)sum[t] / (double)cnt[t] : 0.0;
+			uint32_t a = (uint32_t)(avg * 256), a1 = a >> 8, a2 = a & 0xff;
+			bkey[bo + 2 * t] = ((t * 128u + ctx_p) << 8) | a1; bsidx[bo + 2 * t] = trip_index(lay, part, s_read + 2 * t);
+			bkey[bo + 2 * t + 1] = ((640u + a1) << 8) | a2; bsidx[bo + 2 * t + 1] = trip_index(lay, part, s_read + 2 * t + 1);
+			ctx_p = (uint32_t)avg;
+		}
+	}
+}
+
 __global__ __launch_bounds__(256) void k_qual_symbols(const QualCfg* __restrict__ cfgp, const uint64_t* __restrict__ packed,
                                                      const uint64_t* __restrict__ word_off, const uint8_t* __restrict__ quals,
                                                      const uint64_t* __restrict__ qoff, const uint8_t* __restrict__ flags,
@@ -99,79 +184,81 @@
 	const uint32_t part = part_of_read(lay, r);
 	bool out_of_range = false;
 
-	if (navg)
-	{
-		uint32_t sum[5] = { 0, 0, 0, 0, 0 }, cnt[5] = { 0, 0, 0, 0, 0 };
-		for (uint32_t i = lane; i < len; i += 64)
-		{
-			uint32_t q = quals[qb + i] - 33u;
-			out_of_range |= q > 95u;
-			uint32_t b = cfg.mode == QM_AVERAGE ? 0u : cfg.map_fwd[q > 95u ? 0u : q];
-#pragma unroll
-			for (uint32_t t = 0; t < 5; ++t) if (b == t) { sum[t] += q; cnt[t] += 1; }
-		}
-#pragma unroll
-		for (uint32_t t = 0; t < 5; ++t) { sum[t] = wave_sum(sum[t]); cnt[t] = wave_sum(cnt[t]); }
-		if (lane == 0)
-		{
-			const uint64_t bo = (uint64_t)(r - r0) * navg;
-			if (cfg.mode == QM_AVERAGE)
+	if (navg) qual_read_bytes(cfg, quals, qb, len, lane, lay, part, s_read, (uint64_t)(r - r0) * navg, bkey, bsidx, out_of_range);
+	if (!per_base) { if (__ballot(out_of_range) && lane == 0) atomicOr(bad, 1u); return; }
+	if (!key) return;
+
+	const TripPart tp = trip_part(lay, part);
+	for (uint32_t i = lane; i < len; i += 64)
+	{
+		key[k_read + i] = qual_key_at(cfg, packed, quals, flags, qb, wb, len, i, out_of_range);
+		sidx_out[k_read + i] = trip_index(tp, s_read + navg + i);
+	}
+	if (__ballot(out_of_range) && lane == 0) atomicOr(bad, 1u);
+}
+
+struct QualSource {
+	QualCfg cfg;
+	const uint64_t* __restrict__ packed; const uint64_t* __restrict__ word_off; const uint8_t* __restrict__ quals; const uint64_t* __restrict__ qoff; const uint8_t* __restrict__ flags;
+	uint32_t r0, r1; uint64_t q0; TripLayoutDev lay; uint32_t* bad;
+	struct Cursor {
+		uint32_t r_lo, r_hi, p_lo, p_hi;
+		uint32_t kb, len; uint64_t wb;
+		TripPart tp; uint64_t s0;
+	};
+	template<bool PAIRS> __device__ Cursor begin(uint64_t first, uint64_t end) const
+	{
+		Cursor c; c.r_lo = c.r_hi = r0; c.p_lo = c.p_hi = 0; c.kb = 0; c.len = 0; c.wb = 0; c.tp = TripPart{ 0, 0, 0 }; c.s0 = 0;
+		if (first >= end) return c;
+		const uint32_t lo = wave_last_le(qoff, r0, r1, q0 + first);
+		const uint64_t xl = q0 + end - 1;
+		const uint32_t j = lo + 1 + lane_id() < r1 ? lo + 1 + lane_id() : r1;
+		const uint64_t m = __ballot(qoff[j] > xl);
+		const uint32_t hi = m ? lo + (uint32_t)__builtin_ctzll(m) : wave_last_le(qoff, lo + 64, r1, xl);
+		c.r_lo = __builtin_amdgcn_readfirstlane(lo); c.r_hi = __builtin_amdgcn_readfirstlane(hi);
+		if (PAIRS)
+		{
+			const uint32_t plo = wave_last_le(lay.part_first_read, 0u, lay.np, lo);
+			const uint32_t phi = hi == lo ? plo : wave_last_le(lay.part_first_read, plo, lay.np, hi);
+			c.p_lo = __builtin_amdgcn_readfirstlane(plo); c.p_hi = __builtin_amdgcn_readfirstlane(phi);
+		}
+		return c;
+	}
+	template<bool PAIRS> __device__ uint32_t locate(Cursor& c, uint32_t k) const
+	{
+		if (k - c.kb >= c.len)
+		{
+			const uint32_t r = last_le(qoff, c.r_lo, c.r_hi + 1, q0 + k);
+			const uint64_t qb = qoff[r];
+			c.kb = (uint32_t)(qb - q0); c.len = (uint32_t)(qoff[r + 1] - qb); c.wb = word_off[r];
+			if (PAIRS)
 			{
-				double avg = (double)sum[0] / (double)len;
-				uint32_t a = (uint32_t)(avg * 256), a1 = a >> 8, a2 = a & 0xff;
-				bkey[bo] = (0u << 8) | a1; bsidx[bo] = trip_index(lay, part, s_read);
-				bkey[bo + 1] = ((640u + a1) << 8) | a2; bsidx[bo + 1] = trip_index(lay, part, s_read + 1);
+				c.tp = trip_part(lay, last_le(lay.part_first_read, c.p_lo, c.p_hi + 1, r));
+				c.s0 = (qb - q0) + (uint64_t)(r - r0) * cfg.navg + cfg.navg;
 			}
-			else
-			{
-				uint32_t ctx_p = 0;
-				for (uint32_t t = 0; t < cfg.n_bins; ++t)
-				{
-					double avg = cnt[t] ? (double)sum[t] / (double)cnt[t] : 0.0;
-					uint32_t a = (uint32_t)(avg * 256), a1 = a >> 8, a2 = a & 0xff;
-					bkey[bo + 2 * t] = ((t * 128u + ctx_p) << 8) | a1; bsidx[bo + 2 * t] = trip_index(lay, part, s_read + 2 * t);
-					bkey[bo + 2 * t + 1] = ((640u + a1) << 8) | a2; bsidx[bo + 2 * t + 1] = trip_index(lay, part, s_read + 2 * t + 1);
-					ctx_p = (uint32_t)avg;
-				}
-			}
-		}
-	}
-	if (cfg.mode == QM_AVERAGE || cfg.mode == QM_NONE) { if (__ballot(out_of_range) && lane == 0) atomicOr(bad, 1u); return; }
-
-	const uint32_t radix = cfg.hist_radix, missing = radix - 1;
-	for (uint32_t i = lane; i < len; i += 64)
-	{
-		uint32_t qv = quals[qb + i] - 33u;
-		if (qv > 95u) { out_of_range = true; qv = 0; }
-		uint32_t sym = cfg.map_fwd[qv];
-		uint32_t hist = 0, place = 1;
-		for (uint32_t t = 1; t <= cfg.n_ctx_sym; ++t, place *= radix)
-		{
-			uint32_t v = missing;
-			if (i >= t)
-			{
-				const uint32_t qp = quals[qb + i - t] - 33u;
-				uint32_t s = cfg.map_fwd[qp > 95u ? 0u : qp];
-				v = cfg.mode == QM_ORIGINAL ? (cfg.quant[s] & missing) : s;
-			}
-			hist = qual_hist_add(hist, place, v);
-		}
-		uint32_t b0 = arena_base(packed, wb, i);
-		uint32_t bm1 = i > 0 ? arena_base(packed, wb, i - 1) : 0;
-		uint32_t bm2 = i > 1 ? arena_base(packed, wb, i - 2) : 0;
-		uint32_t bp1 = i + 1 < len ? arena_base(packed, wb, i + 1) : 0;
-		uint32_t bctx;
-		if (cfg.is_avg) bctx = (bm2 << 6) | (bm1 << 4) | (b0 << 2) | bp1;
-		else if (cfg.is_thr) bctx = b0 | (bm1 << 2) | (bm2 << 4) | (bp1 << 6);
-		else if (cfg.level == 3) bctx = b0 | (bm1 << 2) | (bm2 << 4) | (bp1 << 6);
-		else bctx = b0 | (bm1 << 2) | ((uint32_t)(i > 1 && bm2 == bm1) << 4) | (bp1 << 5);
-		uint32_t fl = 0;
-		if (cfg.level > 1 && flags) { uint8_t c = flags[qb + i]; fl = (c == 'M' ? 1u : 0u) | (c == 'A' ? 2u : 0u); }
-		key[k_read + i] = (qual_ctx_id(cfg, hist, bctx, fl) << cfg.sym_bits) | sym;
-		sidx_out[k_read + i] = trip_index(lay, part, s_read + navg + i);
-	}
-	if (__ballot(out_of_range) && lane == 0) atomicOr(bad, 1u);
-}
+		}
+		return k - c.kb;
+	}
+	__device__ uint32_t key(Cursor& c, uint64_t idx) const
+	{
+		const uint32_t i = locate<false>(c, (uint32_t)idx);
+		bool out_of_range = false;
+		const uint32_t k = qual_key_at(cfg, packed, quals, flags, q0 + c.kb, c.wb, c.len, i, out_of_range);
+		if (out_of_range) atomicOr(bad, 1u);
+		return k;
+	}
+	template<bool HAS_V> __device__ void pair(Cursor& c, uint64_t idx, uint32_t& k, uint32_t& v) const
+	{
+		const uint32_t i = locate<true>(c, (uint32_t)idx);
+		bool out_of_range = false;
+		k = qual_key_at(cfg, packed, quals, flags, q0 + c.kb, c.wb, c.len, i, out_of_range);
+		v = trip_index(c.tp, c.s0 + i);
+	}
+	static const char* suffix() { return "QualSource"; }
+	static constexpr bool KEYS_ONLY = false;
+	double hist_bytes() const { return 1.0 + 0.25 + (cfg.level > 1 && flags ? 1.0 : 0.0); }
+	double pair_bytes(bool) const { return hist_bytes(); }
+};
 
 __global__ void k_seg_bounds(const uint32_t* __restrict__ skey, uint64_t n, uint32_t shift, uint32_t* __restrict__ seg_start, uint32_t* __restrict__ seg_end)
 {
@@ -370,6 +457,7 @@
 	cl_qual_coder* Q = new cl_qual_coder(); Q->ctx = ctx;
 	std::unique_ptr<cl_qual_coder> guard(Q);
 	QualCfg& c = Q->cfg; memset(&c, 0, sizeof(c));
+	Q->unfused = getenv("COLORD_HIP_QUAL_UNFUSED") != nullptr;
 	c.mode = prm->mode; c.level = prm->level;
 	c.max_total = 1u << 18; c.adder = 8;
 	auto bins = [&](uint32_t n) -> cl_status {
@@ -502,11 +590,20 @@
 		DevBuf<uint32_t>& key = G.key; DevBuf<uint32_t>& sidx = G.sidx; DevBuf<uint32_t>& bkey = G.bkey; DevBuf<uint32_t>& bsidx = G.bsidx;
 		DEV_ALLOC(ctx, key, per_base ? n_base : 0); DEV_ALLOC(ctx, sidx, per_base ? n_base : 0);
 		DEV_ALLOC(ctx, bkey, n_byte); DEV_ALLOC(ctx, bsidx, n_byte);
-		if (r1 > r0)
-			LAUNCHB(ctx, n_base * (1.0 + 0.25 + 8.0) + n_byte * 8.0, k_qual_symbols, grid_for(r1 - r0, 4), 256, (const QualCfg*)Q->d_cfg.p, (const uint64_t*)R->packed.p, (const uint64_t*)R->word_off.p,
-				d_quals, d_qual_off, d_flags, r0, r1, qo[p0], lay, key.p, sidx.p, bkey.p, bsidx.p, bad.p);
+		const bool fused = per_base && !Q->unfused;
+		if (r1 > r0 && (!fused || n_byte))
+			LAUNCHB(ctx, n_base * (1.0 + (fused ? 0.0 : 0.25 + 8.0)) + n_byte * 8.0, k_qual_symbols, grid_for(r1 - r0, 4), 256, (const QualCfg*)Q->d_cfg.p, (const uint64_t*)R->packed.p, (const uint64_t*)R->word_off.p,
+				d_quals, d_qual_off, d_flags, r0, r1, qo[p0], lay, fused ? (uint32_t*)nullptr : key.p, fused ? (uint32_t*)nullptr : sidx.p, bkey.p, bsidx.p, bad.p);
 		HIP_TRY(ctx, hipGetLastError());
-		if (per_base && n_base) CL_TRY(dev_sort_keys32_pairs(ctx, key.p, sidx.p, n_base, c.sym_bits, c.sym_bits + c.dense_bits));
+		if (per_base && n_base)
+		{
+			if (fused)
+			{
+				const QualSource src{ c, (const uint64_t*)R->packed.p, (const uint64_t*)R->word_off.p, d_quals, d_qual_off, d_flags, r0, r1, qo[p0], lay, bad.p };
+				CL_TRY((sort_impl<uint32_t, QualSource>(ctx, key.p, sidx.p, n_base, c.sym_bits, c.sym_bits + c.dense_bits, nullptr, nullptr, &src)));
+			}
+			else CL_TRY(dev_sort_keys32_pairs(ctx, key.p, sidx.p, n_base, c.sym_bits, c.sym_bits + c.dense_bits));
+		}
 		if (n_byte)
 		{
 			CL_TRY(dev_sort_keys32_pairs(ctx, bkey.p, bsidx.p, n_byte, 8, 8 + 10));
diff --git a/colord_amd/csrc/rc_dev.hpp b/colord_amd/csrc/rc_dev.hpp
--- a/colord_amd/csrc/rc_dev.hpp
+++ b/colord_amd/csrc/rc_dev.hpp
@@ -45,11 +45,14 @@
 	while (hi - lo > 1) { uint32_t mid = (lo + hi) >> 1; if (L.part_first_read[mid] <= r) lo = mid; else hi = mid; }
 	return lo;
 }
-__device__ inline uint32_t trip_index(const TripLayoutDev& L, uint32_t part, uint64_t stream_pos)
+struct TripPart { uint64_t group_base, sym_start; uint32_t place; };
+__device__ inline TripPart trip_part(const TripLayoutDev& L, uint32_t part)
 {
 	const uint32_t pl = L.rank ? L.rank[part] : part;
-	return (uint32_t)trip_slot(L.group_base[pl >> 6], pl & 63, stream_pos - L.part_sym_start[part]);
-}
+	return TripPart{ L.group_base[pl >> 6], L.part_sym_start[part], pl & 63 };
+}
+__device__ inline uint32_t trip_index(const TripPart& P, uint64_t stream_pos) { return (uint32_t)trip_slot(P.group_base, P.place, stream_pos - P.sym_start); }
+__device__ inline uint32_t trip_index(const TripLayoutDev& L, uint32_t part, uint64_t stream_pos) { return trip_index(trip_part(L, part), stream_pos); }
 
 struct __attribute__((packed)) unaligned_u64 { uint64_t v; };
 __device__ inline void store_be64(uint8_t* p, uint64_t v) { ((unaligned_u64*)p)->v = __builtin_bswap64(v); }
diff --git a/colord_amd/csrc/sort.hip b/colord_amd/csrc/sort.hip
--- a/colord_amd/csrc/sort.hip
+++ b/colord_amd/csrc/sort.hip
@@ -1,202 +1,12 @@
-#include "common.hpp"
-#include <string>
-
-namespace {
-constexpr uint32_t ST = 256;
-constexpr uint32_t SI = 16;
-constexpr uint32_t STILE = ST * SI;
-
-template<typename K, uint32_t DB, uint32_t G>
-__global__ __launch_bounds__(ST) void k_sort_hist(const K* __restrict__ keys, uint64_t n, uint32_t shift, uint32_t dmask,
-                                                  uint32_t* __restrict__ hist, uint32_t nb)
-{
-	constexpr uint32_t ND = 1u << DB;
-	constexpr uint32_t ROW = G > 1 ? ND + 1 : ND;
-	__shared__ uint32_t h[G * ROW];
-	for (uint32_t i = threadIdx.x; i < G * ROW; i += ST) h[i] = 0;
-	__syncthreads();
-	const uint32_t tile0 = blockIdx.x * G;
-	for (uint32_t g = 0; g < G && tile0 + g < nb; ++g)
-	{
-		const uint64_t base = (uint64_t)(tile0 + g) * STILE;
-#pragma unroll
-		for (uint32_t i = 0; i < SI; ++i)
-		{
-			uint64_t idx = base + (uint64_t)i * ST + threadIdx.x;
-			if (idx < n) atomicAdd(&h[g * ROW + ((uint32_t)(keys[idx] >> shift) & dmask)], 1u);
-		}
-	}
-	__syncthreads();
-	for (uint32_t i = threadIdx.x; i < G * ND; i += ST)
-	{
-		const uint32_t g = i % G, d = i / G;
-		if (tile0 + g < nb) hist[(uint64_t)d * nb + tile0 + g] = h[g * ROW + d];
-	}
-}
-
-template<typename K, bool HAS_V, uint32_t DB>
-__global__ __launch_bounds__(ST) void k_sort_scatter(const K* __restrict__ kin, const uint32_t* __restrict__ vin,
-                                                     K* __restrict__ kout, uint32_t* __restrict__ vout,
-                                                     uint64_t n, uint32_t shift, uint32_t dmask, const uint32_t* __restrict__ offs, uint32_t nb)
-{
-	constexpr uint32_t ND = 1u << DB, PER = ND / ST;
-	__shared__ uint32_t wh[4][ND];
-	__shared__ uint32_t lstart[ND + 1];
-	__shared__ uint32_t gdelta[ND];
-	__shared__ uint32_t wtot[4];
-	__shared__ K skey[STILE];
-	__shared__ uint32_t sval[HAS_V ? STILE : 1];
-	const uint32_t w = threadIdx.x >> 6, lane = threadIdx.x & 63;
-	for (uint32_t i = threadIdx.x; i < 4 * ND; i += ST) (&wh[0][0])[i] = 0;
-	__syncthreads();
-
-	const uint64_t tbase = (uint64_t)blockIdx.x * STILE, wbase = tbase + (uint64_t)w * (64 * SI);
-	K key[SI]; uint32_t rank[SI]; uint32_t val[HAS_V ? SI : 1];
-	const uint64_t lt = (1ULL << lane) - 1;
-	uint32_t goff[PER];
-#pragma unroll
-	for (uint32_t k = 0; k < PER; ++k) goff[k] = offs[(uint64_t)(threadIdx.x * PER + k) * nb + blockIdx.x];
-#pragma unroll
-	for (uint32_t r = 0; r < SI; ++r)
-	{
-		uint64_t idx = wbase + (uint64_t)r * 64 + lane;
-		key[r] = idx < n ? kin[idx] : (K)0;
-		if (HAS_V) val[r] = idx < n ? vin[idx] : 0u;
-	}
-#pragma unroll
-	for (uint32_t r = 0; r < SI; ++r)
-	{
-		uint64_t idx = wbase + (uint64_t)r * 64 + lane;
-		bool valid = idx < n;
-		uint32_t d = (uint32_t)(key[r] >> shift) & dmask;
-		uint64_t peers = __ballot(valid);
-#pragma unroll
-		for (uint32_t b = 0; b < DB; ++b)
-		{
-			bool bit = (d >> b) & 1u;
-			uint64_t m = __ballot(valid && bit);
-			peers &= bit ? m : ~m;
-		}
-		uint32_t prior = valid ? wh[w][d] : 0u;
-		rank[r] = prior + (uint32_t)__popcll(peers & lt);
-		__builtin_amdgcn_wave_barrier();
-		if (valid && (peers & lt) == 0) wh[w][d] = prior + (uint32_t)__popcll(peers);
-		__builtin_amdgcn_wave_barrier();
-	}
-	__syncthreads();
-	{
-		uint32_t c[PER][4], tot[PER], mine = 0;
-#pragma unroll
-		for (uint32_t k = 0; k < PER; ++k)
-		{
-			const uint32_t d = threadIdx.x * PER + k;
-			c[k][0] = wh[0][d]; c[k][1] = wh[1][d]; c[k][2] = wh[2][d]; c[k][3] = wh[3][d];
-			tot[k] = c[k][0] + c[k][1] + c[k][2] + c[k][3]; mine += tot[k];
-		}
-		uint32_t incl = mine;
-#pragma unroll
-		for (uint32_t o = 1; o < 64; o <<= 1) { const uint32_t t = __shfl_up(incl, o, 64); if (lane >= o) incl += t; }
-		if (lane == 63) wtot[w] = incl;
-		__syncthreads();
-		uint32_t ls = incl - mine;
-		for (uint32_t i = 0; i < w; ++i) ls += wtot[i];
-#pragma unroll
-		for (uint32_t k = 0; k < PER; ++k)
-		{
-			const uint32_t d = threadIdx.x * PER + k;
-			lstart[d] = ls;
-			if (d == ND - 1) lstart[ND] = ls + tot[k];
-			gdelta[d] = goff[k] - ls;
-			wh[0][d] = ls; wh[1][d] = ls + c[k][0]; wh[2][d] = ls + c[k][0] + c[k][1]; wh[3][d] = ls + c[k][0] + c[k][1] + c[k][2];
-			ls += tot[k];
-		}
-	}
-	__syncthreads();
-#pragma unroll
-	for (uint32_t r = 0; r < SI; ++r)
-	{
-		uint64_t idx = wbase + (uint64_t)r * 64 + lane;
-		if (idx < n)
-		{
-			uint32_t d = (uint32_t)(key[r] >> shift) & dmask;
-			uint32_t lp = wh[w][d] + rank[r];
-			skey[lp] = key[r];
-			if (HAS_V) sval[lp] = val[r];
-		}
-	}
-	__syncthreads();
-	const uint32_t tile_n = lstart[ND];
-	for (uint32_t j = threadIdx.x; j < tile_n; j += ST)
-	{
-		const K k = skey[j];
-		const uint32_t pos = gdelta[(uint32_t)(k >> shift) & dmask] + j;
-		kout[pos] = k;
-		if (HAS_V) vout[pos] = sval[j];
-	}
-}
-
-template<typename K, uint32_t DB>
-cl_status sort_pass(cl_ctx* ctx, const K* kin, const uint32_t* vin, K* kout, uint32_t* vout, uint64_t n, uint32_t shift, uint32_t dmask, uint32_t* hist, uint32_t nb)
-{
-	static const std::string kt = sizeof(K) == 8 ? "unsigned long" : "unsigned int", db = std::to_string(DB) + "u";
-	constexpr uint32_t G = DB == 8 ? 16 : 4; const bool grouped = nb >= 4096;
-	static const std::string n_hist1 = "k_sort_hist<" + kt + ", " + db + ", 1u>", n_histg = "k_sort_hist<" + kt + ", " + db + ", " + std::to_string(G) + "u>", n_sv = "k_sort_scatter<" + kt + ", true, " + db + ">", n_sk = "k_sort_scatter<" + kt + ", false, " + db + ">";
-	if (grouped) LAUNCHB_NAMED(ctx, n_histg.c_str(), n * sizeof(K), (k_sort_hist<K, DB, G>), (nb + G - 1) / G, ST, kin, n, shift, dmask, hist, nb);
-	else LAUNCHB_NAMED(ctx, n_hist1.c_str(), n * sizeof(K), (k_sort_hist<K, DB, 1>), nb, ST, kin, n, shift, dmask, hist, nb);
-	HIP_TRY(ctx, hipGetLastError());
-	CL_TRY(dev_exclusive_scan_u32(ctx, hist, (uint64_t)(1u << DB) * nb, nullptr));
-	if (vin) LAUNCHB_NAMED(ctx, n_sv.c_str(), n * (2 * sizeof(K) + 8), (k_sort_scatter<K, true, DB>), nb, ST, kin, vin, kout, vout, n, shift, dmask, (const uint32_t*)hist, nb);
-	else LAUNCHB_NAMED(ctx, n_sk.c_str(), n * 2 * sizeof(K), (k_sort_scatter<K, false, DB>), nb, ST, kin, (const uint32_t*)nullptr, kout, (uint32_t*)nullptr, n, shift, dmask, (const uint32_t*)hist, nb);
-	HIP_TRY(ctx, hipGetLastError());
-	return CL_OK;
-}
+#include "sort_dev.hpp"
 
 template<typename K>
-cl_status sort_impl(cl_ctx* ctx, K* d_keys, uint32_t* d_vals, uint64_t n, uint32_t begin_bit, uint32_t end_bit, DevBuf<K>* swap_k = nullptr, DevBuf<uint32_t>* swap_v = nullptr)
+cl_status dev_sort_pass_plain(cl_ctx* ctx, uint32_t use, const K* kin, const uint32_t* vin, K* kout, uint32_t* vout, uint64_t n, uint32_t shift, uint32_t dmask, uint32_t* hist, uint32_t nb)
 {
-	if (n <= 1 || end_bit <= begin_bit) return CL_OK;
-	if (n >= (1ULL << 32)) return cl_fail(ctx, CL_E_UNSUPPORTED, "radix sort: n must be < 2^32 per call");
-	const uint32_t nb = grid_for(n, STILE);
-	const uint32_t bits = end_bit - begin_bit;
-	const uint32_t n_pass_real = (bits + 7) / 8 == (bits + 9) / 10 ? (bits + 7) / 8 : (bits + 9) / 10;
-	const uint32_t db_hi = (bits + n_pass_real - 1) / n_pass_real;
-	const bool third = (n_pass_real & 1) && n_pass_real > 1 && n * (sizeof(K) + (d_vals ? 4 : 0)) <= (2ull << 30);
-	const uint32_t n_pass = third ? n_pass_real : (n_pass_real + 1) & ~1u;
-	DevBuf<K> ktmp, ktmp2; DEV_ALLOC(ctx, ktmp, n);
-	DevBuf<uint32_t> vtmp, vtmp2; if (d_vals) DEV_ALLOC(ctx, vtmp, n);
-	if (n_pass & 1) { DEV_ALLOC(ctx, ktmp2, n); if (d_vals) DEV_ALLOC(ctx, vtmp2, n); }
-	DevBuf<uint32_t> hist; DEV_ALLOC(ctx, hist, (uint64_t)(1u << std::max(8u, db_hi)) * nb);
-	K* kin = d_keys; uint32_t* vin = d_vals;
-	uint32_t pass = 0;
-	for (uint32_t shift = begin_bit; shift < end_bit; ++pass)
-	{
-		K* kout; uint32_t* vout;
-		if (n_pass & 1) { kout = pass == 0 ? ktmp2.p : (pass & 1) ? ktmp.p : d_keys; vout = pass == 0 ? vtmp2.p : (pass & 1) ? vtmp.p : d_vals; }
-		else { kout = (pass & 1) ? d_keys : ktmp.p; vout = (pass & 1) ? d_vals : vtmp.p; }
-		const uint32_t left = end_bit - shift, passes_left = n_pass_real - pass;
-		const uint32_t db = std::max(8u, (left + passes_left - 1) / passes_left);
-		const uint32_t use = std::min(db, 10u);
-		const uint32_t dmask = (1u << std::min(use, left)) - 1;
-		if (use == 10) CL_TRY((sort_pass<K, 10>(ctx, kin, vin, kout, vout, n, shift, dmask, hist.p, nb)));
-		else if (use == 9) CL_TRY((sort_pass<K, 9>(ctx, kin, vin, kout, vout, n, shift, dmask, hist.p, nb)));
-		else CL_TRY((sort_pass<K, 8>(ctx, kin, vin, kout, vout, n, shift, dmask, hist.p, nb)));
-		shift += use;
-		kin = kout; vin = vout;
-	}
-	if (kin != d_keys && swap_k && kin == ktmp.p && (!d_vals || (swap_v && vin == vtmp.p)))
-	{
-		std::swap(*swap_k, ktmp);
-		if (d_vals) std::swap(*swap_v, vtmp);
-	}
-	else if (kin != d_keys)
-	{
-		HIP_TRY(ctx, hipMemcpyAsync(d_keys, kin, n * sizeof(K), hipMemcpyDeviceToDevice, cl_launch_stream(ctx)));
-		if (d_vals) HIP_TRY(ctx, hipMemcpyAsync(d_vals, vin, n * 4, hipMemcpyDeviceToDevice, cl_launch_stream(ctx)));
-	}
-	HIP_TRY(ctx, hipStreamSynchronize(cl_launch_stream(ctx)));
-	return CL_OK;
+	return sort_pass_bits<K, PlainSource<K>>(ctx, use, PlainSource<K>{ kin, vin }, vin != nullptr, kout, vout, n, shift, dmask, hist, nb);
 }
-}
+template cl_status dev_sort_pass_plain<uint32_t>(cl_ctx*, uint32_t, const uint32_t*, const uint32_t*, uint32_t*, uint32_t*, uint64_t, uint32_t, uint32_t, uint32_t*, uint32_t);
+template cl_status dev_sort_pass_plain<uint64_t>(cl_ctx*, uint32_t, const uint64_t*, const uint32_t*, uint64_t*, uint32_t*, uint64_t, uint32_t, uint32_t, uint32_t*, uint32_t);
 
 cl_status dev_sort_pairs(cl_ctx* ctx, uint64_t* d_keys, uint32_t* d_vals, uint64_t n, uint32_t begin_bit, uint32_t end_bit)
 {
diff --git a/colord_amd/csrc/sort_dev.hpp b/colord_amd/csrc/sort_dev.hpp
--- /dev/null
+++ b/colord_amd/csrc/sort_dev.hpp
@@ -0,0 +1,228 @@
+#pragma once
+#include "common.hpp"
+#include <string>
+
+namespace {
+constexpr uint32_t ST = 256;
+constexpr uint32_t SI = 16;
+constexpr uint32_t STILE = ST * SI;
+
+template<typename K>
+struct PlainSource {
+	const K* __restrict__ kin; const uint32_t* __restrict__ vin;
+	struct Cursor {};
+	template<bool PAIRS> __device__ Cursor begin(uint64_t, uint64_t) const { return Cursor(); }
+	__device__ K key(Cursor&, uint64_t idx) const { return kin[idx]; }
+	template<bool HAS_V> __device__ void pair(Cursor&, uint64_t idx, K& k, uint32_t& v) const { k = kin[idx]; if (HAS_V) v = vin[idx]; }
+	static const char* suffix() { return ""; }
+	static constexpr bool KEYS_ONLY = true;
+	double hist_bytes() const { return sizeof(K); }
+	double pair_bytes(bool has_v) const { return sizeof(K) + (has_v ? 4 : 0); }
+};
+
+template<typename K, uint32_t DB, uint32_t G, typename Src>
+__global__ __launch_bounds__(ST) void k_sort_hist(const Src src, uint64_t n, uint32_t shift, uint32_t dmask,
+                                                  uint32_t* __restrict__ hist, uint32_t nb)
+{
+	constexpr uint32_t ND = 1u << DB;
+	constexpr uint32_t ROW = G > 1 ? ND + 1 : ND;
+	__shared__ uint32_t h[G * ROW];
+	for (uint32_t i = threadIdx.x; i < G * ROW; i += ST) h[i] = 0;
+	__syncthreads();
+	const uint32_t tile0 = blockIdx.x * G;
+	for (uint32_t g = 0; g < G && tile0 + g < nb; ++g)
+	{
+		const uint64_t base = (uint64_t)(tile0 + g) * STILE;
+		typename Src::Cursor cur = src.template begin<false>(base, base + STILE < n ? base + STILE : n);
+#pragma unroll
+		for (uint32_t i = 0; i < SI; ++i)
+		{
+			uint64_t idx = base + (uint64_t)i * ST + threadIdx.x;
+			if (idx < n) atomicAdd(&h[g * ROW + ((uint32_t)(src.key(cur, idx) >> shift) & dmask)], 1u);
+		}
+	}
+	__syncthreads();
+	for (uint32_t i = threadIdx.x; i < G * ND; i += ST)
+	{
+		const uint32_t g = i % G, d = i / G;
+		if (tile0 + g < nb) hist[(uint64_t)d * nb + tile0 + g] = h[g * ROW + d];
+	}
+}
+
+template<typename K, bool HAS_V, uint32_t DB, typename Src>
+__global__ __launch_bounds__(ST) void k_sort_scatter(const Src src,
+                                                     K* __restrict__ kout, uint32_t* __restrict__ vout,
+                                                     uint64_t n, uint32_t shift, uint32_t dmask, const uint32_t* __restrict__ offs, uint32_t nb)
+{
+	constexpr uint32_t ND = 1u << DB, PER = ND / ST;
+	__shared__ uint32_t wh[4][ND];
+	__shared__ uint32_t lstart[ND + 1];
+	__shared__ uint32_t gdelta[ND];
+	__shared__ uint32_t wtot[4];
+	__shared__ K skey[STILE];
+	__shared__ uint32_t sval[HAS_V ? STILE : 1];
+	const uint32_t w = threadIdx.x >> 6, lane = threadIdx.x & 63;
+	for (uint32_t i = threadIdx.x; i < 4 * ND; i += ST) (&wh[0][0])[i] = 0;
+	__syncthreads();
+
+	const uint64_t tbase = (uint64_t)blockIdx.x * STILE, wbase = tbase + (uint64_t)w * (64 * SI);
+	K key[SI]; uint32_t rank[SI]; uint32_t val[HAS_V ? SI : 1];
+	const uint64_t lt = (1ULL << lane) - 1;
+	uint32_t goff[PER];
+#pragma unroll
+	for (uint32_t k = 0; k < PER; ++k) goff[k] = offs[(uint64_t)(threadIdx.x * PER + k) * nb + blockIdx.x];
+	typename Src::Cursor cur = src.template begin<true>(wbase, wbase + 64 * SI < n ? wbase + 64 * SI : n);
+#pragma unroll
+	for (uint32_t r = 0; r < SI; ++r)
+	{
+		uint64_t idx = wbase + (uint64_t)r * 64 + lane;
+		key[r] = (K)0; if (HAS_V) val[r] = 0u;
+		if (idx < n) src.template pair<HAS_V>(cur, idx, key[r], val[HAS_V ? r : 0]);
+	}
+#pragma unroll
+	for (uint32_t r = 0; r < SI; ++r)
+	{
+		uint64_t idx = wbase + (uint64_t)r * 64 + lane;
+		bool valid = idx < n;
+		uint32_t d = (uint32_t)(key[r] >> shift) & dmask;
+		uint64_t peers = __ballot(valid);
+#pragma unroll
+		for (uint32_t b = 0; b < DB; ++b)
+		{
+			bool bit = (d >> b) & 1u;
+			uint64_t m = __ballot(valid && bit);
+			peers &= bit ? m : ~m;
+		}
+		uint32_t prior = valid ? wh[w][d] : 0u;
+		rank[r] = prior + (uint32_t)__popcll(peers & lt);
+		__builtin_amdgcn_wave_barrier();
+		if (valid && (peers & lt) == 0) wh[w][d] = prior + (uint32_t)__popcll(peers);
+		__builtin_amdgcn_wave_barrier();
+	}
+	__syncthreads();
+	{
+		uint32_t c[PER][4], tot[PER], mine = 0;
+#pragma unroll
+		for (uint32_t k = 0; k < PER; ++k)
+		{
+			const uint32_t d = threadIdx.x * PER + k;
+			c[k][0] = wh[0][d]; c[k][1] = wh[1][d]; c[k][2] = wh[2][d]; c[k][3] = wh[3][d];
+			tot[k] = c[k][0] + c[k][1] + c[k][2] + c[k][3]; mine += tot[k];
+		}
+		uint32_t incl = mine;
+#pragma unroll
+		for (uint32_t o = 1; o < 64; o <<= 1) { const uint32_t t = __shfl_up(incl, o, 64); if (lane >= o) incl += t; }
+		if (lane == 63) wtot[w] = incl;
+		__syncthreads();
+		uint32_t ls = incl - mine;
+		for (uint32_t i = 0; i < w; ++i) ls += wtot[i];
+#pragma unroll
+		for (uint32_t k = 0; k < PER; ++k)
+		{
+			const uint32_t d = threadIdx.x * PER + k;
+			lstart[d] = ls;
+			if (d == ND - 1) lstart[ND] = ls + tot[k];
+			gdelta[d] = goff[k] - ls;
+			wh[0][d] = ls; wh[1][d] = ls + c[k][0]; wh[2][d] = ls + c[k][0] + c[k][1]; wh[3][d] = ls + c[k][0] + c[k][1] + c[k][2];
+			ls += tot[k];
+		}
+	}
+	__syncthreads();
+#pragma unroll
+	for (uint32_t r = 0; r < SI; ++r)
+	{
+		uint64_t idx = wbase + (uint64_t)r * 64 + lane;
+		if (idx < n)
+		{
+			uint32_t d = (uint32_t)(key[r] >> shift) & dmask;
+			uint32_t lp = wh[w][d] + rank[r];
+			skey[lp] = key[r];
+			if (HAS_V) sval[lp] = val[r];
+		}
+	}
+	__syncthreads();
+	const uint32_t tile_n = lstart[ND];
+	for (uint32_t j = threadIdx.x; j < tile_n; j += ST)
+	{
+		const K k = skey[j];
+		const uint32_t pos = gdelta[(uint32_t)(k >> shift) & dmask] + j;
+		kout[pos] = k;
+		if (HAS_V) vout[pos] = sval[j];
+	}
+}
+
+template<typename K, uint32_t DB, typename Src>
+cl_status sort_pass(cl_ctx* ctx, const Src& src, bool has_v, K* kout, uint32_t* vout, uint64_t n, uint32_t shift, uint32_t dmask, uint32_t* hist, uint32_t nb)
+{
+	static const std::string kt = sizeof(K) == 8 ? "unsigned long" : "unsigned int", db = std::to_string(DB) + "u", sfx = Src::suffix()[0] ? std::string(", ") + Src::suffix() : std::string();
+	constexpr uint32_t G = DB == 8 ? 16 : 4; const bool grouped = nb >= 4096;
+	static const std::string n_hist1 = "k_sort_hist<" + kt + ", " + db + ", 1u" + sfx + ">", n_histg = "k_sort_hist<" + kt + ", " + db + ", " + std::to_string(G) + "u" + sfx + ">",
+		n_sv = "k_sort_scatter<" + kt + ", true, " + db + sfx + ">", n_sk = "k_sort_scatter<" + kt + ", false, " + db + sfx + ">";
+	if (grouped) LAUNCHB_NAMED(ctx, n_histg.c_str(), n * src.hist_bytes(), (k_sort_hist<K, DB, G, Src>), (nb + G - 1) / G, ST, src, n, shift, dmask, hist, nb);
+	else LAUNCHB_NAMED(ctx, n_hist1.c_str(), n * src.hist_bytes(), (k_sort_hist<K, DB, 1, Src>), nb, ST, src, n, shift, dmask, hist, nb);
+	HIP_TRY(ctx, hipGetLastError());
+	CL_TRY(dev_exclusive_scan_u32(ctx, hist, (uint64_t)(1u << DB) * nb, nullptr));
+	if (has_v) LAUNCHB_NAMED(ctx, n_sv.c_str(), n * (src.pair_bytes(true) + sizeof(K) + 4), (k_sort_scatter<K, true, DB, Src>), nb, ST, src, kout, vout, n, shift, dmask, (const uint32_t*)hist, nb);
+	else if constexpr (Src::KEYS_ONLY) LAUNCHB_NAMED(ctx, n_sk.c_str(), n * (src.pair_bytes(false) + sizeof(K)), (k_sort_scatter<K, false, DB, Src>), nb, ST, src, kout, (uint32_t*)nullptr, n, shift, dmask, (const uint32_t*)hist, nb);
+	else return cl_fail(ctx, CL_E_INVALID, "radix sort: this source has no keys-only form");
+	HIP_TRY(ctx, hipGetLastError());
+	return CL_OK;
+}
+template<typename K, typename Src>
+cl_status sort_pass_bits(cl_ctx* ctx, uint32_t use, const Src& src, bool has_v, K* kout, uint32_t* vout, uint64_t n, uint32_t shift, uint32_t dmask, uint32_t* hist, uint32_t nb)
+{
+	if (use == 10) return sort_pass<K, 10>(ctx, src, has_v, kout, vout, n, shift, dmask, hist, nb);
+	if (use == 9) return sort_pass<K, 9>(ctx, src, has_v, kout, vout, n, shift, dmask, hist, nb);
+	return sort_pass<K, 8>(ctx, src, has_v, kout, vout, n, shift, dmask, hist, nb);
+}
+}
+
+template<typename K>
+cl_status dev_sort_pass_plain(cl_ctx* ctx, uint32_t use, const K* kin, const uint32_t* vin, K* kout, uint32_t* vout, uint64_t n, uint32_t shift, uint32_t dmask, uint32_t* hist, uint32_t nb);
+
+namespace {
+template<typename K, typename Src0 = PlainSource<K>>
+cl_status sort_impl(cl_ctx* ctx, K* d_keys, uint32_t* d_vals, uint64_t n, uint32_t begin_bit, uint32_t end_bit, DevBuf<K>* swap_k = nullptr, DevBuf<uint32_t>* swap_v = nullptr, const Src0* first = nullptr)
+{
+	if (n <= (first ? 0u : 1u) || end_bit <= begin_bit) return CL_OK;
+	if (n >= (1ULL << 32)) return cl_fail(ctx, CL_E_UNSUPPORTED, "radix sort: n must be < 2^32 per call");
+	const uint32_t nb = grid_for(n, STILE);
+	const uint32_t bits = end_bit - begin_bit;
+	const uint32_t n_pass_real = (bits + 7) / 8 == (bits + 9) / 10 ? (bits + 7) / 8 : (bits + 9) / 10;
+	const uint32_t db_hi = (bits + n_pass_real - 1) / n_pass_real;
+	const bool third = (n_pass_real & 1) && n_pass_real > 1 && n * (sizeof(K) + (d_vals ? 4 : 0)) <= (2ull << 30);
+	const uint32_t n_pass = third ? n_pass_real : (n_pass_real + 1) & ~1u;
+	DevBuf<K> ktmp, ktmp2; DEV_ALLOC(ctx, ktmp, n);
+	DevBuf<uint32_t> vtmp, vtmp2; if (d_vals) DEV_ALLOC(ctx, vtmp, n);
+	if (n_pass & 1) { DEV_ALLOC(ctx, ktmp2, n); if (d_vals) DEV_ALLOC(ctx, vtmp2, n); }
+	DevBuf<uint32_t> hist; DEV_ALLOC(ctx, hist, (uint64_t)(1u << std::max(8u, db_hi)) * nb);
+	K* kin = d_keys; uint32_t* vin = d_vals;
+	uint32_t pass = 0;
+	for (uint32_t shift = begin_bit; shift < end_bit; ++pass)
+	{
+		K* kout; uint32_t* vout;
+		if (n_pass & 1) { kout = pass == 0 ? ktmp2.p : (pass & 1) ? ktmp.p : d_keys; vout = pass == 0 ? vtmp2.p : (pass & 1) ? vtmp.p : d_vals; }
+		else { kout = (pass & 1) ? d_keys : ktmp.p; vout = (pass & 1) ? d_vals : vtmp.p; }
+		const uint32_t left = end_bit - shift, passes_left = n_pass_real - pass;
+		const uint32_t db = std::max(8u, (left + passes_left - 1) / passes_left);
+		const uint32_t use = std::min(db, 10u);
+		const uint32_t dmask = (1u << std::min(use, left)) - 1;
+		if (pass == 0 && first) CL_TRY((sort_pass_bits<K, Src0>(ctx, use, *first, d_vals != nullptr, kout, vout, n, shift, dmask, hist.p, nb)));
+		else CL_TRY(dev_sort_pass_plain<K>(ctx, use, kin, vin, kout, vout, n, shift, dmask, hist.p, nb));
+		shift += use;
+		kin = kout; vin = vout;
+	}
+	if (kin != d_keys && swap_k && kin == ktmp.p && (!d_vals || (swap_v && vin == vtmp.p)))
+	{
+		std::swap(*swap_k, ktmp);
+		if (d_vals) std::swap(*swap_v, vtmp);
+	}
+	else if (kin != d_keys)
+	{
+		HIP_TRY(ctx, hipMemcpyAsync(d_keys, kin, n * sizeof(K), hipMemcpyDeviceToDevice, cl_launch_stream(ctx)));
+		if (d_vals) HIP_TRY(ctx, hipMemcpyAsync(d_vals, vin, n * 4, hipMemcpyDeviceToDevice, cl_launch_stream(ctx)));
+	}
+	HIP_TRY(ctx, hipStreamSynchronize(cl_launch_stream(ctx)));
+	return CL_OK;
+}
+}
```

Result: faster. 3.028, median of 4 (+4.2%).
